# gnosisguild/stylus-zkvm-verifiers

Hardware: AMD Instinct MI355X
Metric: Groth16 proofs verified/sec (BN254) (higher is better)
Workload: dtype u32

## Files before the change

stylus_zkvm_verifiers_amd/csrc/bn254_constants.h:

```cpp
#pragma once
#include <stdint.h>
namespace zkv {
#define ZKV_FP_P_LIMBS {0xd87cfd47u, 0x3c208c16u, 0x6871ca8du, 0x97816a91u, 0x8181585du, 0xb85045b6u, 0xe131a029u, 0x30644e72u}
#define ZKV_FR_R_LIMBS {0xf0000001u, 0x43e1f593u, 0x79b97091u, 0x2833e848u, 0x8181585du, 0xb85045b6u, 0xe131a029u, 0x30644e72u}
#define ZKV_FP_INV32 0xe4866389u
#define ZKV_FP_P29_LIMBS {0x187cfd47u, 0x010460b6u, 0x1c72a34fu, 0x02d522d0u, 0x1585d978u, 0x02db40c0u, 0x00a6e141u, 0x0e5c2634u, 0x0030644eu}
#define ZKV_FP_INV29 0x04866389u
#define ZKV_FP_FAT4P_LIMBS {0x21f3f51cu, 0x241182dau, 0x31ca8d3bu, 0x2b548b42u, 0x361765dfu, 0x2b6d0301u, 0x229b8503u, 0x397098cfu, 0x00c19138u}
#define ZKV_FP_FAT8P_LIMBS {0x23e7ea38u, 0x282305b5u, 0x23951a77u, 0x36a91686u, 0x2c2ecbbfu, 0x36da0604u, 0x25370a07u, 0x32e1319fu, 0x01832272u}
#define ZKV_FP_2P_LIMBS {0xb0f9fa8eu, 0x7841182du, 0xd0e3951au, 0x2f02d522u, 0x0302b0bbu, 0x70a08b6du, 0xc2634053u, 0x60c89ce5u}
#define ZKV_FP_16P2_COLS {0x15d69b10ULL, 0xa2c5113ULL, 0xb0404edULL, 0xe5a13dULL, 0xadca602ULL, 0x4e36cb6ULL, 0x12129406ULL, 0xaf42485ULL, 0x104689e9ULL, 0x1a6359c6ULL, 0x1bb7e970ULL, 0x6eac0c4ULL, 0xb855116ULL, 0x690e580ULL, 0x1bdf00d2ULL, 0x1f38b334ULL, 0xb8763cbULL, 0x492e2ULL}
#define ZKV_FP_ONE {{0x157ccc21u, 0x4e8384ebu, 0x0ce148c3u, 0xfb90a602u, 0x819caa36u, 0x5301fa84u, 0x563d4475u, 0x0dc83629u}}
#define ZKV_FP_R2 {{0x659bac10u, 0xe1a2a074u, 0x5406005au, 0x63985586u, 0x2d3e2632u, 0xff54c580u, 0x34ea65a6u, 0x2a11a68cu}}
#define ZKV_FP_TWO_INV {{0xf6fce4b4u, 0x45520880u, 0xbaa989a8u, 0x49890849u, 0x818f014au, 0x85a9201du, 0x1bb7724fu, 0x1f16424eu}}
#define ZKV_FP_THREE {{0x40766463u, 0xeb8a8ec1u, 0x26a3da49u, 0xf2b1f206u, 0x84d5fea4u, 0xf905ef8du, 0x02b7cd5fu, 0x2958a27cu}}
#define ZKV_TWIST_B {{{0xab489658u, 0xdc19fa4au, 0xfbbf6e69u, 0x0d416744u, 0x0a8a033au, 0x8f7734edu, 0x53ee09bbu, 0x19316b83u}}, {{0x3b9fece0u, 0x1cfd999au, 0x79c1a7c7u, 0xbe166fb2u, 0x5580154cu, 0xe93a1ba4u, 0x4d11a9bau, 0x283739c9u}}}
#define ZKV_TWIST_3B {{{0x295cc5c1u, 0x582d62c9u, 0x8acc80b0u, 0x9042cb3du, 0x9e1cb150u, 0xf6155910u, 0x1a987d08u, 0x1b2ff417u}}, {{0x01e5cc12u, 0xdeb7b4a1u, 0x9c61623au, 0x0b4079f4u, 0xfd7d8f2bu, 0x4b0dc77fu, 0x24d1bcddu, 0x17dd1076u}}}
#define ZKV_FROB1 {{{{0x157ccc21u, 0x4e8384ebu, 0x0ce148c3u, 0xfb90a602u, 0x819caa36u, 0x5301fa84u, 0x563d4475u, 0x0dc83629u}}, {{0x00000000u, 0x00000000u, 0x00000000u, 0x00000000u, 0x00000000u, 0x00000000u, 0x00000000u, 0x00000000u}}}, {{{0x8a0c2399u, 0xb75446afu, 0x8d8526c8u, 0xb5e243dfu, 0x8fc2b89bu, 0x7f6d6627u, 0x62b5af58u, 0x2e056030u}}, {{0x3bc6cc33u, 0xaeefbf6eu, 0x4ed87762u, 0x7f50c04bu, 0xeb6a58d4u, 0x9a8b7572u, 0xc410c870u, 0x009b83e6u}}}, {{{0x24a59190u, 0xecdea09bu, 0xae2fe1c2u, 0x17db8ffeu, 0x6dabac4du, 0xbb09c97cu, 0x1d289af3u, 0x2492b3d4u}}, {{0xf1142ef1u, 0xf1663598u, 0x0bf56062u, 0x77ec057eu, 0xb677a631u, 0xdd0baaecu, 0xd284d463u, 0x135e4e31u}}}, {{{0xdb1f0678u, 0xf46e7f60u, 0x5bcc5c3eu, 0x31fc2ebau, 0x086a2411u, 0xedb3adc3u, 0x837817bcu, 0x1d46bd0fu}}, {{0x79a647d5u, 0x6b3fbdf5u, 0x2ff64974u, 0xcc568fb6u, 0xc4348ac6u, 0xc1bfbf4au, 0x3940b4d3u, 0x15871d4du}}}, {{{0xb081f85eu, 0x227346b0u, 0x30492bb5u, 0x6e51a671u, 0x52b19e16u, 0x7e20162eu, 0x2343bb4bu, 0x1677516fu}}, {{0x2f616a78u, 0x18b28085u, 0xbde06eceu, 0x25433712u, 0x6b9a0e66u, 0xb00a5825u, 0x11971bbdu, 0x06f9f8e1u}}}, {{{0x07461d8cu, 0x5c8694d6u, 0x07d3e2dau, 0x2df58554u, 0x667b18b9u, 0xb41988e2u, 0xc7bd8631u, 0x10a3f03eu}}, {{0xdeb54987u, 0x611aada3u, 0xc03203c7u, 0x4a7a9b79u, 0x9a786b4bu, 0x245c1057u, 0x754fe64du, 0x0817f6bdu}}}}
#define ZKV_FROB3 {{{{0x157ccc21u, 0x4e8384ebu, 0x0ce148c3u, 0xfb90a602u, 0x819caa36u, 0x5301fa84u, 0x563d4475u, 0x0dc83629u}}, {{0x00000000u, 0x00000000u, 0x00000000u, 0x00000000u, 0x00000000u, 0x00000000u, 0x00000000u, 0x00000000u}}}, {{{0x8e6a3d3du, 0x9dc00697u, 0x8ef4bf24u, 0x695b3f03u, 0xba7a7ccdu, 0x1a238968u, 0x0e49839cu, 0x103828f2u}}, {{0x4f4e6b31u, 0x5cbbb0bdu, 0x1b5b282bu, 0xe83ce8beu, 0xf03fbae3u, 0x646d437eu, 0x0031f0c0u, 0x133cf986u}}}, {{{0x136caecdu, 0x4738e103u, 0xc376b8c3u, 0xf491475bu, 0xa97cbee8u, 0x1f4034a3u, 0xef61ccd7u, 0x0cad5f8fu}}, {{0xe6e485d6u, 0x2f41c395u, 0x0242aa46u, 0x997230c7u, 0x84887ab5u, 0xeae16f21u, 0x3bcfc9b2u, 0x266696f7u}}}, {{{0xfd5df6cfu, 0x47b20cb5u, 0x0ca56e4eu, 0x65853bd7u, 0x7917344cu, 0xca9c97f3u, 0x5db9886cu, 0x131d9163u}}, {{0x5ed6b572u, 0xd0e0ce21u, 0x387b8118u, 0xcb2adadbu, 0xbd4ccd96u, 0xf690866bu, 0xa7f0eb55u, 0x1add3125u}}}, {{{0x0af866c4u, 0xa0d04454u, 0x7df631b3u, 0x9cc0145fu, 0xcd752de1u, 0x29dda327u, 0x0a170a74u, 0x14766fdbu}}, {{0xe9d402f7u, 0xdd532940u, 0xbfda559eu, 0x541490c5u, 0xc541b0b8u, 0xd9c9c659u, 0x69cbb3e4u, 0x0baf8cb5u}}}, {{{0xe314d9feu, 0xcdc1bb0eu, 0x7463ae42u, 0xfe0354c4u, 0x3e3cd6b9u, 0xf2cc84b7u, 0xabddad87u, 0x14445b76u}}, {{0x9b3b7638u, 0x0210d593u, 0x9015f128u, 0x2d0dc9e1u, 0xc52a22adu, 0xbe219959u, 0x44050889u, 0x12c9d777u}}}}
#define ZKV_FROB2 {{{0x157ccc21u, 0x4e8384ebu, 0x0ce148c3u, 0xfb90a602u, 0x819caa36u, 0x5301fa84u, 0x563d4475u, 0x0dc83629u}}, {{0x6e4983b2u, 0xd96ee872u, 0x458f581eu, 0xe9b7ed6au, 0x9ea5d262u, 0x5361c2c8u, 0x98a79c6eu, 0x24594fd1u}}, {{0x58ccb791u, 0x8aeb6387u, 0x38ae0f5bu, 0xee274768u, 0x1d09282bu, 0x005fc844u, 0x426a57f9u, 0x169119a8u}}, {{0xc3003126u, 0xed9d072bu, 0x5b9081c9u, 0x9bf0c48fu, 0xffe4ae26u, 0x654e4b31u, 0x8af45bb4u, 0x229c1849u}}, {{0x6a337995u, 0x62b1a3a4u, 0x22e2726eu, 0xadc97d27u, 0xe2db85fau, 0x64ee82edu, 0x488a03bbu, 0x0c0afea1u}}, {{0x7fb045b6u, 0xb135288fu, 0x2fc3bb31u, 0xa95a2329u, 0x64783031u, 0xb7f07d72u, 0x9ec74830u, 0x19d334cau}}}
#define ZKV_BN_U 0x44e992b44a6909f1ULL
#define ZKV_ATE_NAF_LEN 66
#define ZKV_ATE_NAF {0, 0, 0, 1, 0, 1, 0, -1, 0, 0, -1, 0, 0, 0, 1, 0, 0, -1, 0, -1, 0, 0, 0, 1, 0, -1, 0, 0, 0, 0, -1, 0, 0, 1, 0, -1, 0, 0, 1, 0, 0, 0, 0, 0, -1, 0, 0, -1, 0, 1, 0, -1, 0, 0, 0, -1, 0, -1, 0, 0, 0, 1, 0, -1, 0, 1}
#define ZKV_MILLER_STEPS 88
#define ZKV_MILLER_STEP_KIND {0, 0, 2, 0, 0, 1, 0, 0, 0, 0, 2, 0, 0, 2, 0, 0, 0, 0, 2, 0, 0, 1, 0, 0, 2, 0, 0, 0, 2, 0, 0, 0, 0, 0, 0, 1, 0, 0, 0, 2, 0, 0, 1, 0, 0, 0, 2, 0, 0, 0, 0, 0, 2, 0, 0, 1, 0, 0, 0, 0, 2, 0, 0, 2, 0, 0, 0, 1, 0, 0, 0, 0, 2, 0, 0, 0, 2, 0, 0, 1, 0, 0, 1, 0, 0, 0, 3, 4}
#define ZKV_U_NAF_LEN 63
#define ZKV_U_NAF {1, 0, 0, 0, -1, 0, 0, 0, 0, 1, 0, 1, 0, 0, 0, 0, 1, 0, 0, 1, 0, -1, 0, 1, 0, 1, 0, 1, 0, 0, 1, 0, 0, 0, 1, 0, -1, 0, -1, 0, -1, 0, 1, 0, 1, 0, 0, -1, 0, 1, 0, 1, 0, -1, 0, 0, 1, 0, 1, 0, 0, 0, 1}
#define ZKV_U_WNAF3_LEN 63
#define ZKV_U_WNAF3 {1, 0, 0, 0, -1, 0, 0, 0, 0, 5, 0, 0, 0, 0, 0, 0, -7, 0, 0, 0, 7, 0, 0, 0, 0, 5, 0, 0, 0, 0, 1, 0, 0, 0, -3, 0, 0, 0, -5, 0, 0, 0, 5, 0, 0, 0, 0, 3, 0, 0, 0, -3, 0, 0, 0, 0, 5, 0, 0, 0, 0, 0, 1}
#define ZKV_U_DIG_LEN 58
#define ZKV_U_DIG {17, 0, 0, 0, 0, -17, 0, 0, 0, 0, 35, 0, 0, 0, 0, 17, 0, 0, 0, 0, 0, 35, 0, 0, 0, 35, 0, 0, 0, 0, 0, 0, 0, 0, -35, 0, 0, 0, -35, 0, 0, 0, 35, 0, 17, 0, 0, 0, 0, 0, 0, -35, 0, 0, 0, 0, 0, 35}
#define ZKV_FE_PROG_LEN 268
#define ZKV_FE_PROG {0x10000u, 0x1u, 0x10102u, 0x1000003u, 0x800u, 0x2080105u, 0x800u, 0x8010203u, 0x20000u, 0x6u, 0x6u, 0x6u, 0x6u, 0x2000003u, 0x600u, 0x6u, 0x2000003u, 0x700u, 0x6u, 0x6u, 0x6u, 0x6u, 0x6u, 0x6u, 0x7000004u, 0x6u, 0x6u, 0x6u, 0x6u, 0x6u, 0x6u, 0x6u, 0x6000003u, 0x6u, 0x6u, 0x7000003u, 0x6u, 0x6u, 0x6u, 0x6u, 0x7000004u, 0x6u, 0x6u, 0x6u, 0x6u, 0x7000004u, 0x6u, 0x6u, 0x6u, 0x6u, 0x6u, 0x6u, 0x6u, 0x6u, 0x6u, 0x7000003u, 0x6u, 0x6u, 0x6u, 0x6u, 0x7000003u, 0x6u, 0x6u, 0x6u, 0x6u, 0x6u, 0x6u, 0x6000003u, 0x6u, 0x6u, 0x6u, 0x6u, 0x6u, 0x7000003u, 0x6u, 0x6u, 0x6u, 0x6u, 0x6u, 0x6000004u, 0x6u, 0x6u, 0x6u, 0x6u, 0x6u, 0x6000003u, 0x1u, 0x6u, 0x300u, 0x6u, 0x3000003u, 0x400u, 0x6u, 0x6u, 0x6u, 0x6u, 0x4000003u, 0x600u, 0x6u, 0x4000003u, 0x700u, 0x6u, 0x6u, 0x6u, 0x6u, 0x6u, 0x6u, 0x7000004u, 0x6u, 0x6u, 0x6u, 0x6u, 0x6u, 0x6u, 0x6u, 0x6000003u, 0x6u, 0x6u, 0x7000003u, 0x6u, 0x6u, 0x6u, 0x6u, 0x7000004u, 0x6u, 0x6u, 0x6u, 0x6u, 0x7000004u, 0x6u, 0x6u, 0x6u, 0x6u, 0x6u, 0x6u, 0x6u, 0x6u, 0x6u, 0x7000003u, 0x6u, 0x6u, 0x6u, 0x6u, 0x7000003u, 0x6u, 0x6u, 0x6u, 0x6u, 0x6u, 0x6u, 0x6000003u, 0x6u, 0x6u, 0x6u, 0x6u, 0x6u, 0x7000003u, 0x6u, 0x6u, 0x6u, 0x6u, 0x6u, 0x6000004u, 0x6u, 0x6u, 0x6u, 0x6u, 0x6u, 0x6000003u, 0x1u, 0x500u, 0x6u, 0x100u, 0x6u, 0x6u, 0x6u, 0x6u, 0x1000003u, 0x600u, 0x6u, 0x1000003u, 0x700u, 0x6u, 0x6u, 0x6u, 0x6u, 0x6u, 0x6u, 0x7000004u, 0x6u, 0x6u, 0x6u, 0x6u, 0x6u, 0x6u, 0x6u, 0x6000003u, 0x6u, 0x6u, 0x7000003u, 0x6u, 0x6u, 0x6u, 0x6u, 0x7000004u, 0x6u, 0x6u, 0x6u, 0x6u, 0x7000004u, 0x6u, 0x6u, 0x6u, 0x6u, 0x6u, 0x6u, 0x6u, 0x6u, 0x6u, 0x7000003u, 0x6u, 0x6u, 0x6u, 0x6u, 0x7000003u, 0x6u, 0x6u, 0x6u, 0x6u, 0x6u, 0x6u, 0x6000003u, 0x6u, 0x6u, 0x6u, 0x6u, 0x6u, 0x7000003u, 0x6u, 0x6u, 0x6u, 0x6u, 0x6u, 0x6000004u, 0x6u, 0x6u, 0x6u, 0x6u, 0x6u, 0x6000003u, 0x401u, 0x5000003u, 0x4000003u, 0x400u, 0x800u, 0x3080103u, 0x5000003u, 0x2000003u, 0x1010305u, 0x3000003u, 0x2040405u, 0x4000003u, 0x201u, 0x1020203u, 0x3020205u, 0x2000003u, 0x800u, 0x807u}
#define ZKV_FP_M30_LIMBS {0x187cfd47, 0x3082305b, 0x071ca8d3, 0x205aa45a, 0x01585d97, 0x0116da06, 0x1a029b85, 0x139cb84c, 0x00003064}
#define ZKV_FP_MINV30 0x1b799c77u
#define ZKV_FP_R3 {{0x4e2312b2u, 0x26d80b94u, 0x85af210eu, 0xfdde6f98u, 0xad1d1adau, 0xb923065cu, 0xa668ff5au, 0x26c2d286u}}
#define ZKV_FR_M30_LIMBS {0x30000001, 0x0f87d64f, 0x1b970914, 0x0cfa121e, 0x01585d28, 0x0116da06, 0x1a029b85, 0x139cb84c, 0x00003064}
#define ZKV_FR_MINV30 0x10000001u
#define ZKV_FR_R3 {{0x601fddb2u, 0xbafa616cu, 0x23e89803u, 0x29b4a83eu, 0x44d1496bu, 0x917ad601u, 0xfe59ed6du, 0x1baa96fcu}}
#define ZKV_GLV_BETA {{0x58ccb791u, 0x8aeb6387u, 0x38ae0f5bu, 0xee274768u, 0x1d09282bu, 0x005fc844u, 0x426a57f9u, 0x169119a8u}}
#define ZKV_GLV_LAMBDA {0x36636f23u, 0xb8ca0b2du, 0xec2bc5e9u, 0xcc37a73fu, 0x3fd84104u, 0x048b6e19u, 0xe131a029u, 0x30644e72u}
#define ZKV_GLV_G1 {0x00ff6565u, 0x5398fd03u, 0xa773d2d2u, 0x4ccef014u, 0x00000002u}
#define ZKV_GLV_G2 {0xc7e0b3d7u, 0xd91d232eu, 0x00000002u}
#define ZKV_GLV_A1 {0x7d4f1128u, 0x8211bbebu, 0xeeb859fcu, 0x6f4d8248u}
#define ZKV_GLV_N {0x94d213e3u, 0x89d32568u}
#define ZKV_GLV_B2 {0x1221250bu, 0x0be4e154u, 0xeeb859fdu, 0x6f4d8248u}
#define ZKV_FP_INV_SCHED_LEN 76
#define ZKV_FP_INV_SCHED {19, 59, 25, 33, 35, 9, 35, 9, 25, 27, 9, 41, 35, 43, 17, 65, 17, 35, 27, 9, 41, 17, 49, 33, 27, 27, 27, 17, 67, 57, 17, 27, 41, 27, 9, 27, 25, 27, 19, 57, 27, 17, 17, 17, 25, 33, 27, 17, 51, 9, 43, 9, 25, 17, 17, 43, 17, 35, 19, 41, 49, 43, 49, 27, 27, 27, 51, 19, 9, 35, 19, 19, 17, 17, 33, 17}
#define ZKV_FP_PM2_LIMBS {0xd87cfd45u, 0x3c208c16u, 0x6871ca8du, 0x97816a91u, 0x8181585du, 0xb85045b6u, 0xe131a029u, 0x30644e72u}
#define ZKV_FR_R29_LIMBS {0x10000001u, 0x1f0fac9fu, 0x0e5c2450u, 0x07d090f3u, 0x1585d283u, 0x02db40c0u, 0x00a6e141u, 0x0e5c2634u, 0x0030644eu}
#define ZKV_FR_INV29 0x0fffffffu
#define ZKV_FR_ONE {{0x8fffff57u, 0x2fd4e156u, 0xa494b01au, 0x75bba827u, 0x819caa80u, 0x5301fa84u, 0x563d4475u, 0x0dc83629u}}
#define ZKV_FR_R2 {{0x45b69bd4u, 0x38c2e14bu, 0x85883377u, 0x0ffedb18u, 0xabc6e54du, 0x7840f9f0u, 0x848b0f05u, 0x0a054a3eu}}
#define ZKV_FR_RM2_LIMBS {0xefffffffu, 0x43e1f593u, 0x79b97091u, 0x2833e848u, 0x8181585du, 0xb85045b6u, 0xe131a029u, 0x30644e72u}
}
```

stylus_zkvm_verifiers_amd/csrc/gen_constants.py:

```python
#!/usr/bin/env python3
import os

U = 4965661367192848881
P = 36 * U**4 + 36 * U**3 + 24 * U**2 + 6 * U + 1
R = 36 * U**4 + 36 * U**3 + 18 * U**2 + 6 * U + 1
MONT = 1 << 261


def f2mul(a, b): return ((a[0] * b[0] - a[1] * b[1]) % P, (a[0] * b[1] + a[1] * b[0]) % P)
def f2inv(a):
    d = pow(a[0] * a[0] + a[1] * a[1], -1, P)
    return (a[0] * d % P, -a[1] * d % P)
def f2pow(a, e):
    r = (1, 0)
    while e:
        if e & 1:
            r = f2mul(r, a)
        a = f2mul(a, a)
        e >>= 1
    return r


def limbs(x):
    return ', '.join('0x%08xu' % ((x >> (32 * i)) & 0xffffffff) for i in range(8))

def mont(x): return x * MONT % P
def fp(x): return '{{%s}}' % limbs(mont(x))
def fp2(a): return '{%s, %s}' % (fp(a[0]), fp(a[1]))


def naf(n):
    out = []
    while n:
        if n & 1:
            d = 2 - (n % 4)
            n -= d
        else:
            d = 0
        out.append(d)
        n >>= 1
    return out


def main():
    xi = (9, 1)
    twist_b = f2mul((3, 0), f2inv(xi))
    g = f2pow(xi, (P - 1) // 6)
    frob1 = [f2pow(g, k) for k in range(6)]
    g2 = f2pow(xi, (P * P - 1) // 6)
    frob2 = [f2pow(g2, k) for k in range(6)]
    assert all(c[1] == 0 for c in frob2)
    g3 = f2pow(xi, (P**3 - 1) // 6)
    frob3 = [f2pow(g3, k) for k in range(6)]
    ate = 6 * U + 2
    ate_naf = naf(ate)
    assert sum(d * (1 << i) for i, d in enumerate(ate_naf)) == ate
    inv32 = (-pow(P, -1, 1 << 32)) % (1 << 32)
    lines = []
    w = lines.append
    w('// GENERATED by gen_constants.py -- do not edit.  BN254 constants in Montgomery form (R = 2^261),')
    w('// 8 x 32-bit little-endian limbs.')
    w('#pragma once')
    w('#include <stdint.h>')
    w('namespace zkv {')
    w('#define ZKV_FP_P_LIMBS {%s}' % limbs(P))
    w('#define ZKV_FR_R_LIMBS {%s}' % limbs(R))
    w('#define ZKV_FP_INV32 0x%08xu' % inv32)
    w('#define ZKV_FP_P29_LIMBS {%s}' % ', '.join('0x%08xu' % ((P >> (29 * i)) & 0x1fffffff) for i in range(9)))
    w('#define ZKV_FP_INV29 0x%08xu' % ((-pow(P, -1, 1 << 29)) % (1 << 29)))
    d4 = [((4 * P) >> (29 * i)) & 0x1fffffff for i in range(9)]
    fat = [d4[0] + (1 << 29)] + [d4[i] + (1 << 29) - 1 for i in range(1, 8)] + [d4[8] - 1]
    assert sum(v << (29 * i) for i, v in enumerate(fat)) == 4 * P and all(v >= (1 << 29) - 1 for v in fat[:8])
    w('// 4p in borrow-free 29-bit limbs (limbs 0..7 >= 2^29-1): FAT - y is limb-wise non-negative for y < 2p')
    w('#define ZKV_FP_FAT4P_LIMBS {%s}' % ', '.join('0x%08xu' % v for v in fat))
    d8 = [((8 * P) >> (29 * i)) & 0x1fffffff for i in range(9)]
    fat8 = [d8[0] + (1 << 29)] + [d8[i] + (1 << 29) - 1 for i in range(1, 8)] + [d8[8] - 1]
    assert sum(v << (29 * i) for i, v in enumerate(fat8)) == 8 * P and all(v >= (1 << 29) - 1 for v in fat8[:8])
    assert fat8[8] >= ((4 * P) >> 232) and max(fat8) < (1 << 31)
    w('// 8p in borrow-free 29-bit limbs: FAT - y is limb-wise non-negative for every y < 4p (lazy sum of two values < 2p)')
    w('#define ZKV_FP_FAT8P_LIMBS {%s}' % ', '.join('0x%08xu' % v for v in fat8))
    w('#define ZKV_FP_2P_LIMBS {%s}' % limbs(2 * P))
    c16 = 16 * P * P
    w('// 16 p^2 in 29-bit digits (18 columns): offset that keeps T0 - T1 non-negative in the fused Fp2 product')
    w('#define ZKV_FP_16P2_COLS {%s}' % ', '.join('0x%xULL' % ((c16 >> (29 * i)) & 0x1fffffff) for i in range(18)))
    assert c16 >> (29 * 18) == 0
    w('#define ZKV_FP_ONE %s' % fp(1))
    w('#define ZKV_FP_R2 {{%s}}' % limbs(MONT * MONT % P))
    w('#define ZKV_FP_TWO_INV %s' % fp(pow(2, -1, P)))
    w('#define ZKV_FP_THREE %s' % fp(3))
    w('#define ZKV_TWIST_B %s' % fp2(twist_b))
    w('#define ZKV_TWIST_3B %s' % fp2((3 * twist_b[0] % P, 3 * twist_b[1] % P)))
    for name, arr in (('FROB1', frob1), ('FROB3', frob3)):
        w('#define ZKV_%s {%s}' % (name, ', '.join(fp2(c) for c in arr)))
    w('#define ZKV_FROB2 {%s}' % ', '.join(fp(c[0]) for c in frob2))
    w('#define ZKV_BN_U 0x%xULL' % U)
    w('#define ZKV_ATE_NAF_LEN %d' % len(ate_naf))
    w('// NAF digits of 6u+2, least significant first (top digit is 1)')
    w('#define ZKV_ATE_NAF {%s}' % ', '.join(str(d) for d in ate_naf))
    kinds = []
    for i in range(len(ate_naf) - 2, -1, -1):
        kinds.append(0)
        if ate_naf[i]:
            kinds.append(1 if ate_naf[i] > 0 else 2)
    kinds += [3, 4]
    assert len(kinds) == 88
    w('// Miller loop as a flat sequence of line steps: 0 doubling (preceded by f <- f^2 except at step 0), 1 add Q, 2 add -Q, 3 add pi(Q), 4 add -pi^2(Q)')
    w('#define ZKV_MILLER_STEPS %d' % len(kinds))
    w('#define ZKV_MILLER_STEP_KIND {%s}' % ', '.join(str(k) for k in kinds))
    u_naf = naf(U)
    assert sum(d * (1 << i) for i, d in enumerate(u_naf)) == U
    w('// NAF digits of u, least significant first (final exponentiation: x^u with conjugates for the -1 digits)')
    w('#define ZKV_U_NAF_LEN %d' % len(u_naf))
    w('#define ZKV_U_NAF {%s}' % ', '.join(str(d) for d in u_naf))
    def wnaf(n, width):
        out = []
        while n:
            if n & 1:
                d = n % (1 << (width + 1))
                if d >= (1 << width):
                    d -= 1 << (width + 1)
                n -= d
            else:
                d = 0
            out.append(d)
            n >>= 1
        return out
    u_w3 = wnaf(U, 3)
    assert sum(d * (1 << i) for i, d in enumerate(u_w3)) == U and u_w3[-1] == 1 and all(abs(d) in (0, 1, 3, 5, 7) for d in u_w3)
    w('// width-3 NAF digits of u (odd digits up to +-7), least significant first, top digit 1: %d non-zero digits' % sum(1 for d in u_w3 if d))
    w('#define ZKV_U_WNAF3_LEN %d' % len(u_w3))
    w('#define ZKV_U_WNAF3 {%s}' % ', '.join(str(d) for d in u_w3))
    OPS = dict(COPY=0, CONJ=1, INV=2, MUL=3, MULC=4, FROB=5, CSQR=6, ISONE=7)
    ACC, F_, E_, Y1, Y3, Y4, X3, X5, X7 = range(9)
    prog = []
    acc_is = [None]
    def op(name, d=0, a=0, b=0):
        if name == 'COPY' and d == ACC and acc_is[0] == a:
            return
        if name == 'COPY' and a == ACC: acc_is[0] = d
        elif name == 'COPY' and d == ACC: acc_is[0] = a
        elif d == ACC or d == acc_is[0]: acc_is[0] = None
        prog.append(OPS[name] | d << 8 | a << 16 | b << 24)
    import functools, sys
    sys.setrecursionlimit(10000)
    DIG = (1, 17, 35)
    @functools.lru_cache(None)
    def recode(n):
        if n == 0:
            return (0, ())
        if n % 2 == 0:
            c, t = recode(n // 2)
            return (c, (0,) + t)
        best = None
        for d in DIG:
            for sd in (d, -d):
                m = (n - sd) // 2
                if abs(m) < abs(n) or (abs(n) <= max(DIG) and m == 0):
                    c, t = recode(m)
                    if best is None or c + 1 < best[0]:
                        best = (c + 1, (sd,) + t)
        return best
    u_dig = recode(U)[1]
    assert sum(d << i for i, d in enumerate(u_dig)) == U and u_dig[-1] > 0 and sum(1 for d in u_dig if d) == 12
    w('// digits of u from {0, +-1, +-17, +-35}, least significant first, top digit positive: %d non-zero (final exponentiation, x^u)' % sum(1 for d in u_dig if d))
    w('#define ZKV_U_DIG_LEN %d' % len(u_dig))
    w('#define ZKV_U_DIG {%s}' % ', '.join(str(d) for d in u_dig))
    def expu(x):
        X17, X35 = X3, X5
        op('COPY', ACC, x)
        for _ in range(4): op('CSQR', ACC)
        op('MUL', ACC, ACC, x); op('COPY', X17, ACC)
        op('CSQR', ACC)
        op('MUL', ACC, ACC, x); op('COPY', X35, ACC)
        src = {1: x, 17: X17, 35: X35}
        op('COPY', ACC, src[u_dig[-1]])
        for i in range(len(u_dig) - 2, -1, -1):
            op('CSQR', ACC)
            d = u_dig[i]
            if d:
                op('MUL' if d > 0 else 'MULC', ACC, ACC, src[abs(d)])
    op('COPY', ACC, F_); op('CONJ', ACC); op('INV', F_, F_); op('MUL', ACC, ACC, F_)
    op('FROB', F_, ACC, 2); op('MUL', E_, F_, ACC)
    expu(E_); op('CONJ', ACC)
    op('CSQR', ACC); op('COPY', Y1, ACC)
    op('CSQR', ACC)
    op('MUL', ACC, ACC, Y1); op('COPY', Y3, ACC)
    expu(Y3); op('CONJ', ACC); op('COPY', Y4, ACC)
    op('CSQR', ACC); op('COPY', F_, ACC)
    expu(F_)
    op('CONJ', Y3)
    op('MUL', ACC, ACC, Y4)
    op('MUL', ACC, ACC, Y3); op('COPY', Y3, ACC)
    op('MUL', F_, ACC, Y1)
    op('MUL', ACC, ACC, Y4)
    op('MUL', ACC, ACC, E_)
    op('FROB', Y1, F_, 1); op('MUL', ACC, ACC, Y1)
    op('FROB', Y3, Y3, 2); op('MUL', ACC, ACC, Y3)
    op('CONJ', E_); op('MUL', E_, E_, F_); op('FROB', E_, E_, 3)
    op('MUL', ACC, ACC, E_)
    op('ISONE', ACC)
    TMP = 8
    out = []
    for e in prog:
        o, d, a, b = e & 255, (e >> 8) & 255, (e >> 16) & 255, e >> 24
        native = (o == OPS['CSQR'] or o == OPS['COPY'] or (o == OPS['CONJ'] and d == ACC)
                  or (o in (OPS['MUL'], OPS['MULC']) and d == ACC and a == ACC and b != ACC))
        if not native:
            assert d != ACC or o == OPS['ISONE']
            uses = (a == ACC and o in (OPS['INV'], OPS['MUL'], OPS['MULC'], OPS['FROB'])) or (b == ACC and o in (OPS['MUL'], OPS['MULC'])) or (o == OPS['ISONE'] and d == ACC)
            if uses:
                out.append(OPS['COPY'] | TMP << 8 | ACC << 16)
                if o == OPS['ISONE']: d = TMP
                if a == ACC and o != OPS['ISONE']: a = TMP
                if b == ACC and o in (OPS['MUL'], OPS['MULC']): b = TMP
                e = o | d << 8 | a << 16 | b << 24
        out.append(e)
    prog = out
    w('// final exponentiation (easy part, Fuentes-Castaneda hard part, x^u on the signed digit set {1, 17, 35}) as a flat program: op | dst << 8 | a << 16 | b << 24;')
    w('// ops 0 COPY d<-a, 1 CONJ d, 2 INV d<-a, 3 MUL d<-a*b, 4 MULC d<-a*conj(b), 5 FROB d<-pi^b(a), 6 CSQR d (cyclotomic), 7 ISONE; slots 0 ACC 1 F 2 E 3 Y1 4 Y3 5 Y4 6 X17 7 X35 8 TMP')
    w('#define ZKV_FE_PROG_LEN %d' % len(prog))
    w('#define ZKV_FE_PROG {%s}' % ', '.join('0x%xu' % v for v in prog))
    e = P - 2
    bits = bin(e)[2:]
    sched = []
    i = 0
    nsq = 0
    while i < len(bits):
        if bits[i] == '0':
            nsq += 1; i += 1
            continue
        l = min(2, len(bits) - i)
        while bits[i + l - 1] == '0':
            l -= 1
        v = int(bits[i:i + l], 2)
        sched.append((nsq + l, v))
        nsq = 0
        i += l
    if nsq:
        sched.append((nsq, 0))
    first = sched[0]
    acc = first[1]
    for n_, v in sched[1:]:
        acc = acc * (1 << n_) + v
    assert acc == e and first[0] == len(bin(first[1])) - 2
    assert all(n_ < 32 and v in (0, 1, 3) for n_, v in sched)
    w('// a^(p-2): sliding window (width 2) schedule, entries = squarings << 3 | odd power (0 = none); entry 0 = start power.')
    w('// %d squarings and %d multiplications instead of 253 and %d' % (sum(n_ for n_, v in sched[1:]), sum(1 for n_, v in sched[1:] if v) + 2, bin(e).count('1') - 1))
    def limbs30(x): return ', '.join('0x%08x' % ((x >> (30 * i)) & ((1 << 30) - 1)) for i in range(9))
    w('// safegcd inversion (zkv_modinv.h): the modulus as nine 30-bit limbs, its inverse mod 2^30, and R^3 mod p (Montgomery factor that')
    w('// turns (aR)^-1 into a^-1 R with one multiplication)')
    w('#define ZKV_FP_M30_LIMBS {%s}' % limbs30(P))
    w('#define ZKV_FP_MINV30 0x%08xu' % pow(P, -1, 1 << 30))
    w('#define ZKV_FP_R3 {{%s}}' % limbs(MONT ** 3 % P))
    w('#define ZKV_FR_M30_LIMBS {%s}' % limbs30(R))
    w('#define ZKV_FR_MINV30 0x%08xu' % pow(R, -1, 1 << 30))
    w('#define ZKV_FR_R3 {{%s}}' % limbs((1 << (3 * 261)) % R))
    lam = 0x30644e72e131a029048b6e193fd84104cc37a73fec2bc5e9b8ca0b2d36636f23
    beta = 0x30644e72e131a0295e6dd9e7e0acccb0c28f069fbb966e3de4bd44e5607cfd48
    assert (lam * lam + lam + 1) % R == 0 and pow(beta, 3, P) == 1 and beta != 1
    a1, nb1, a2, b2 = 6 * U * U + 2 * U, 2 * U + 1, 2 * U + 1, 6 * U * U + 4 * U + 1
    assert (a1 - nb1 * lam) % R == 0 and (a2 + b2 * lam) % R == 0
    def nl(x, n): return ', '.join('0x%08xu' % ((x >> (32 * i)) & 0xffffffff) for i in range(n))
    w('// GLV: beta (Montgomery form), lambda, floor(2^256 b2 / r) (5 words), floor(2^256 (2u+1) / r) (3 words), a1 = 6u^2+2u (4), 2u+1 (2), b2 = 6u^2+4u+1 (4)')
    w('#define ZKV_GLV_BETA %s' % fp(beta))
    w('#define ZKV_GLV_LAMBDA {%s}' % limbs(lam))
    w('#define ZKV_GLV_G1 {%s}' % nl((b2 << 256) // R, 5))
    w('#define ZKV_GLV_G2 {%s}' % nl((nb1 << 256) // R, 3))
    w('#define ZKV_GLV_A1 {%s}' % nl(a1, 4))
    w('#define ZKV_GLV_N {%s}' % nl(nb1, 2))
    w('#define ZKV_GLV_B2 {%s}' % nl(b2, 4))
    assert ((b2 << 256) // R).bit_length() <= 160 and ((nb1 << 256) // R).bit_length() <= 96
    w('#define ZKV_FP_INV_SCHED_LEN %d' % len(sched))
    w('#define ZKV_FP_INV_SCHED {%s}' % ', '.join(str((n_ << 3) | v) for n_, v in sched))
    w('// p-2 for Fermat inversion, little-endian 32-bit words')
    w('#define ZKV_FP_PM2_LIMBS {%s}' % limbs(P - 2))
    w('// scalar field: r as nine 29-bit limbs, -r^-1 mod 2^29, 2^261 mod r, 2^522 mod r, r - 2 (Fermat inversion)')
    w('#define ZKV_FR_R29_LIMBS {%s}' % ', '.join('0x%08xu' % ((R >> (29 * i)) & 0x1fffffff) for i in range(9)))
    w('#define ZKV_FR_INV29 0x%08xu' % ((-pow(R, -1, 1 << 29)) % (1 << 29)))
    w('#define ZKV_FR_ONE {{%s}}' % limbs((1 << 261) % R))
    w('#define ZKV_FR_R2 {{%s}}' % limbs((1 << 522) % R))
    w('#define ZKV_FR_RM2_LIMBS {%s}' % limbs(R - 2))
    w('}  // namespace zkv')
    out = os.path.join(os.path.dirname(os.path.abspath(__file__)), 'bn254_constants.h')
    with open(out, 'w') as f:
        f.write('\n'.join(lines) + '\n')
    print('wrote', out, 'naf len', len(ate_naf), 'weight', sum(1 for d in ate_naf if d))


if __name__ == '__main__':
    main()
```

stylus_zkvm_verifiers_amd/csrc/k_pair.hip:

```cpp
#define ZKV_PAIRED 1
#include "zkv_internal.h"
#include "zkv_agg.h"

namespace zkv {

#ifndef ZKV_PAIR_WAVES
#define ZKV_PAIR_WAVES 1
#endif
constexpr int PAIR_BLOCK = ZKV_BLOCK * ZKV_PAIR_WAVES;

__device__ __forceinline__ Fp2 ld_b(const Workspace& ws, int word0, size_t i) {
    Fp2 r; r.h = ws_ld(ws.prep, ws.cap, word0 + 8 * (int)(threadIdx.x & 1u), i);
    return r;
}

__global__ __launch_bounds__(ZKV_BLOCK, 2) void k_g2chk2(size_t n, Workspace ws, uint8_t* __restrict__ status) {
    size_t i = ((size_t)blockIdx.x * ZKV_BLOCK + threadIdx.x) >> 1;
    if (i >= n) return;
    uint32_t flags = ws.flags[i];
    if (!(flags & FL_ALIVE) || (flags & FL_B_INF)) return;
    Fp2 bx = ld_b(ws, 32, i), by = ld_b(ws, 48, i);
    bool ok = g2_in_subgroup(bx, by);
    if (!ok && !(threadIdx.x & 1u)) { ws.g2bad[i] = 1; status[i] = ST_VERIFICATION_FAILED; }
}

#if defined(ZKV_STAMPS)
__device__ unsigned long long* g_zkv_stamps = nullptr;
extern "C" __attribute__((visibility("default"))) int zkv_diag_set_stamps(void* dev_ptr) {
    return (int)hipMemcpyToSymbol(HIP_SYMBOL(g_zkv_stamps), &dev_ptr, sizeof(dev_ptr));
}
__device__ __forceinline__ void zkv_stamp(unsigned kernel, unsigned slot) {
    if ((threadIdx.x & 63u) != 0 || !g_zkv_stamps) return;
    unsigned long long* row = g_zkv_stamps + ((size_t)kernel * gridDim.x * (blockDim.x >> 6) + (size_t)blockIdx.x * (blockDim.x >> 6) + (threadIdx.x >> 6)) * 8;
    row[slot] = __builtin_amdgcn_s_memrealtime();
    row[4 + slot] = __builtin_amdgcn_s_memtime();
    if (slot == 0) { row[2] = __builtin_amdgcn_s_getreg((31 << 11) | 4); row[3] = __builtin_amdgcn_s_getreg((31 << 11) | 20); }
}
#define ZKV_STAMP(k, s) zkv_stamp(k, s)
#else
#define ZKV_STAMP(k, s) ((void)0)
#endif

__global__ __launch_bounds__(PAIR_BLOCK, 2) void k_miller2(size_t n, const VkTables* __restrict__ vk, Workspace ws, uint8_t* __restrict__ status) {
    __shared__ uint32_t lds[(48 + 24) * PAIR_BLOCK];
    ZKV_STAMP(0, 0);
    size_t i = ((size_t)blockIdx.x * PAIR_BLOCK + threadIdx.x) >> 1;
    if (i >= n) return;
    uint32_t flags = ws.flags[i];
    if (!(flags & FL_ALIVE)) return;
    const uint32_t par = threadIdx.x & 1u;
    uint32_t* wl = lds + (threadIdx.x >> 6) * ((48 + 24) * ZKV_BLOCK) + (threadIdx.x & 63u);
    LRef fm = l_ref(wl);
    LRef tm = l_ref(wl + 48 * ZKV_BLOCK);
    SoaRef norm = {ws.norm, ws.cap, (uint32_t)i * 4u};
    SoaRef bsrc = {ws.prep + 32 * ws.cap, ws.cap, (uint32_t)(8 * par * ws.cap + i) * 4u};
    if (!miller_loop_p(vk, flags, norm, bsrc, fm, tm, true)) {
        if (!par) { ws.g2bad[i] = 1; status[i] = ST_VERIFICATION_FAILED; }
        return;
    }
    MRef ab = m_ref((uint32_t*)(vk->f_alpha_beta) + 8 * par, 1, 16);
    MRef out = m_ref(ws.f + (size_t)(8 * par) * ws.cap + i, (uint32_t)ws.cap, 16);
    f12m_mul_body(out, fm, ab, false);
    ZKV_STAMP(0, 1);
}

__global__ __launch_bounds__(PAIR_BLOCK, 2) void k_finalexp2(size_t n, Workspace ws, uint8_t* __restrict__ status) {
    __shared__ uint32_t lds[54 * PAIR_BLOCK];
    ZKV_STAMP(1, 0);
    size_t i = ((size_t)blockIdx.x * PAIR_BLOCK + threadIdx.x) >> 1;
    if (i >= n) return;
    uint32_t flags = ws.flags[i];
    if (!(flags & FL_ALIVE) || ws.g2bad[i]) return;
    const uint32_t par = threadIdx.x & 1u;
    uint32_t* wl = lds + (threadIdx.x >> 6) * (54 * ZKV_BLOCK) + (threadIdx.x & 63u);
    L9Ref acc = l9_ref(wl);
    bool one = final_exp_prog_p(ws.f, ws.fe, ws.cap, (uint32_t)(8 * par * ws.cap + i) * 4u, acc);
    if (!par) status[i] = one ? ST_OK : ST_VERIFICATION_FAILED;
    ZKV_STAMP(1, 1);
}

ZKV_HD bool pair_all(bool mine) {
    uint32_t v = mine ? 0u : 1u;
    v |= zkv_partner_u32(v);
    return v == 0;
}
__global__ __launch_bounds__(ZKV_BLOCK, 2) void k_pairing_check(size_t n, uint32_t k, uint32_t j, size_t slot_off, const uint8_t* __restrict__ in, Workspace ws,
                                                                uint8_t* __restrict__ ok) {
    const size_t call = ((size_t)blockIdx.x * ZKV_BLOCK + threadIdx.x) >> 1;
    if (call >= n) return;
    const size_t i = call + slot_off;
    const uint32_t par = threadIdx.x & 1u;
    if (j == 0) {
        f12m_set_one(m_ref(ws.f + (size_t)(8 * par) * ws.cap + call, (uint32_t)ws.cap, 16));
        if (!par) ok[call] = 1;
    } else if (!ok[call]) { if (!par) ws.flags[i] = 0; return; }
    const uint8_t* p = in + (size_t)192 * ((size_t)k * call + j);
    uint32_t gx[8], gy[8], qxw[8], qyw[8];
    load_be256(gx, p); load_be256(gy, p + 32);
    load_be256(qxw, p + 64 + 32 * (1 - par));
    load_be256(qyw, p + 128 + 32 * (1 - par));
    bool okj = raw_lt_p(gx) && raw_lt_p(gy);
    okj = pair_all(okj && raw_lt_p(qxw) && raw_lt_p(qyw));
    const bool pinf = raw_is_zero(gx) && raw_is_zero(gy);
    const bool qinf = pair_all(raw_is_zero(qxw) && raw_is_zero(qyw));
    Fp px = fp_zero(), py = fp_zero();
    if (okj && !pinf) { px = fp_from_raw(gx); py = fp_from_raw(gy); okj = g1_on_curve(px, py); }
    uint32_t run = 0;
    if (okj && !qinf) {
        Fp2 qx, qy; qx.h = fp_from_raw(qxw); qy.h = fp_from_raw(qyw);
        okj = g2_on_twist(qx, qy);
        if (okj) {
            const Fp iy = pinf ? fp_zero() : fp_inv(py);
            ws_st(ws.norm, ws.cap, 0, i, fp_mul(px, iy)); ws_st(ws.norm, ws.cap, 8, i, iy);
            ws_st(ws.prep, ws.cap, 32 + 8 * (int)par, i, qx.h); ws_st(ws.prep, ws.cap, 48 + 8 * (int)par, i, qy.h);
            run = pinf ? 2u : 1u;
        }
    }
    if (!par) { ws.flags[i] = run; if (!okj) ok[call] = 0; }
}
template <int G>
__global__ __launch_bounds__(PAIR_BLOCK, 2) void k_pairing_miller_g(size_t n, uint32_t k, Workspace ws, uint8_t* __restrict__ ok) {
    __shared__ uint32_t lds[48 * PAIR_BLOCK];
    const size_t i = ((size_t)blockIdx.x * PAIR_BLOCK + threadIdx.x) >> 1;
    if (i >= n) return;
    if (!ok[i]) return;
    uint32_t mask = 0, abmask = 0;
#pragma unroll
    for (uint32_t p = 0; p < (uint32_t)G; p++) {
        const uint32_t run = p < k ? ws.flags[i + p * n] : 0u;
        if (run) { mask |= 1u << p; if (run == 1u) abmask |= 1u << p; }
    }
    const uint32_t par = threadIdx.x & 1u;
    MRef P = m_ref(ws.f + (size_t)(8 * par) * ws.cap + i, (uint32_t)ws.cap, 16);
    if (!mask) return;
    uint32_t* wl = lds + (threadIdx.x >> 6) * (48 * ZKV_BLOCK) + (threadIdx.x & 63u);
    LRef fm = l_ref(wl);
    SoaRef norm = {ws.norm, ws.cap, (uint32_t)i * 4u};
    SoaRef bsrc = {ws.prep + 32 * ws.cap, ws.cap, (uint32_t)(8 * par * ws.cap + i) * 4u};
    SoaRW tq = {ws.fe, ws.cap, (uint32_t)(8 * par * ws.cap + i) * 4u};
    const uint32_t fine = miller_loop_pg<G>(mask, abmask, norm, bsrc, tq, (uint32_t)n * 4u, fm);
    if ((fine & mask) != mask) { if (!par) ok[i] = 0; return; }
    f12m_copy(P, fm);
}
__global__ __launch_bounds__(ZKV_BLOCK, 2) void k_pairing_miller(size_t n, Workspace ws, uint8_t* __restrict__ ok) {
    __shared__ uint32_t lds[(48 + 24) * ZKV_BLOCK];
    size_t i = ((size_t)blockIdx.x * ZKV_BLOCK + threadIdx.x) >> 1;
    if (i >= n) return;
    const uint32_t run = ws.flags[i];
    if (!run) return;
    const uint32_t par = threadIdx.x & 1u;
    LRef fm = l_ref(lds + threadIdx.x);
    LRef tm = l_ref(lds + 48 * ZKV_BLOCK + threadIdx.x);
    MRef P = m_ref(ws.f + (size_t)(8 * par) * ws.cap + i, (uint32_t)ws.cap, 16);
    SoaRef norm = {ws.norm, ws.cap, (uint32_t)i * 4u};
    SoaRef bsrc = {ws.prep + 32 * ws.cap, ws.cap, (uint32_t)(8 * par * ws.cap + i) * 4u};
    const bool fine = miller_loop_p((const VkTables*)nullptr, run == 2 ? (uint32_t)FL_A_INF : 0u, norm, bsrc, fm, tm, true);
    if (fine && run == 1) f12m_mul(P, fm, P);
    if (!fine && !par) ok[i] = 0;
}
__global__ __launch_bounds__(ZKV_BLOCK, 2) void k_pairing_finalexp(size_t n, Workspace ws, const uint8_t* __restrict__ ok, uint8_t* __restrict__ result,
                                                                   uint32_t empty) {
    __shared__ uint32_t lds[54 * ZKV_BLOCK];
    size_t i = ((size_t)blockIdx.x * ZKV_BLOCK + threadIdx.x) >> 1;
    if (i >= n) return;
    const uint32_t par = threadIdx.x & 1u;
    uint8_t res = empty ? 1 : 0;
    if (ok[i] && !empty) {
        L9Ref acc = l9_ref(lds + threadIdx.x);
        res = final_exp_prog_p(ws.f, ws.fe, ws.cap, (uint32_t)(8 * par * ws.cap + i) * 4u, acc) ? 1 : 0;
    }
    if (!par) result[i] = res;
}
uint32_t pairing_group(uint32_t k) { return k < 2 ? 0u : k <= 2 ? 2u : k <= 4 ? 4u : k <= 8 ? 8u : 0u; }
void launch_pairing(size_t n, uint32_t k, const uint8_t* in, const Workspace& ws, uint8_t* result, uint8_t* ok, hipStream_t s) {
    if (!n) return;
    const unsigned grid = (unsigned)((2 * n + ZKV_BLOCK - 1) / ZKV_BLOCK);
    if (k == 0) (void)hipMemsetAsync(ok, 1, n, s);
    const uint32_t g = pairing_group(k);
    if (g && (size_t)k * n <= ws.cap) {
        for (uint32_t j = 0; j < k; j++) hipLaunchKernelGGL(k_pairing_check, dim3(grid), dim3(ZKV_BLOCK), 0, s, n, k, j, (size_t)j * n, in, ws, ok);
        const dim3 hg((unsigned)((2 * n + PAIR_BLOCK - 1) / PAIR_BLOCK)), hb(PAIR_BLOCK);
        if (g == 2) hipLaunchKernelGGL(k_pairing_miller_g<2>, hg, hb, 0, s, n, k, ws, ok);
        else if (g == 4) hipLaunchKernelGGL(k_pairing_miller_g<4>, hg, hb, 0, s, n, k, ws, ok);
        else hipLaunchKernelGGL(k_pairing_miller_g<8>, hg, hb, 0, s, n, k, ws, ok);
    } else for (uint32_t j = 0; j < k; j++) {
        hipLaunchKernelGGL(k_pairing_check, dim3(grid), dim3(ZKV_BLOCK), 0, s, n, k, j, (size_t)0, in, ws, ok);
        hipLaunchKernelGGL(k_pairing_miller, dim3(grid), dim3(ZKV_BLOCK), 0, s, n, ws, ok);
    }
    hipLaunchKernelGGL(k_pairing_finalexp, dim3(grid), dim3(ZKV_BLOCK), 0, s, n, ws, ok, result, k == 0 ? 1u : 0u);
}

template <int G>
__global__ __launch_bounds__(PAIR_BLOCK, 2) void k_agg_miller(size_t n, const VkTables* __restrict__ vk, Workspace ws, uint8_t* __restrict__ status) {
    __shared__ uint32_t lds[48 * PAIR_BLOCK];
    constexpr uint32_t L = 64u / G;
    const size_t gp = ((size_t)blockIdx.x * PAIR_BLOCK + threadIdx.x) >> 1;
    const size_t i0 = (gp / L) * 64 + (gp % L);
    if (i0 >= n) return;
    uint32_t alive = 0, mask = 0, abmask = 0;
#pragma unroll
    for (uint32_t p = 0; p < (uint32_t)G; p++) {
        const size_t i = i0 + p * L;
        const uint32_t f = i < n ? ws.flags[i] : 0u;
        if (f & FL_ALIVE) {
            alive |= 1u << p;
            if (!(f & FL_B_INF)) { mask |= 1u << p; if (!(f & FL_A_INF)) abmask |= 1u << p; }
        }
    }
    if (!alive) return;
    const uint32_t par = threadIdx.x & 1u;
    uint32_t* wl = lds + (threadIdx.x >> 6) * (48 * ZKV_BLOCK) + (threadIdx.x & 63u);
    LRef fm = l_ref(wl);
    SoaRef norm = {ws.norm, ws.cap, (uint32_t)i0 * 4u};
    SoaRef bsrc = {ws.prep + 32 * ws.cap, ws.cap, (uint32_t)(8 * par * ws.cap + i0) * 4u};
    SoaRW tq = {ws.fe, ws.cap, (uint32_t)(8 * par * ws.cap + i0) * 4u};
    const uint32_t fine = miller_loop_pg<G>(mask, abmask, norm, bsrc, tq, L * 4u, fm);
    if ((fine & mask) != mask) {
        if (!par) {
#pragma unroll 1
            for (uint32_t p = 0; p < (uint32_t)G; p++) {
                if (!((alive >> p) & 1u)) continue;
                const bool bad = ((mask & ~fine) >> p) & 1u;
                ws.g2bad[i0 + p * L] = bad ? 1u : 2u;
                if (bad) status[i0 + p * L] = ST_VERIFICATION_FAILED;
            }
        }
        return;
    }
    MRef ab = m_ref((uint32_t*)(vk->f_alpha_beta) + 8 * par, 1, 16);
    MRef out = m_ref(ws.f + (size_t)(8 * par) * ws.cap + i0, (uint32_t)ws.cap, 16);
    f12m_mul_body(out, fm, ab, false);
}
void launch_agg_miller(size_t n, uint32_t g, const VkTables* d_tab, const Workspace& ws, uint8_t* status, hipStream_t s) {
    if (!n) return;
    const size_t pairs = ((n + 63) / 64) * (64 / g);
    const dim3 grid((unsigned)((2 * pairs + PAIR_BLOCK - 1) / PAIR_BLOCK)), block(PAIR_BLOCK);
    if (g == 8) hipLaunchKernelGGL(k_agg_miller<8>, grid, block, 0, s, n, d_tab, ws, status);
    else if (g == 4) hipLaunchKernelGGL(k_agg_miller<4>, grid, block, 0, s, n, d_tab, ws, status);
    else hipLaunchKernelGGL(k_agg_miller<2>, grid, block, 0, s, n, d_tab, ws, status);
}
__global__ __launch_bounds__(ZKV_BLOCK, 2) void k_agg_fprod(size_t n, size_t n2, uint32_t sub, uint32_t g, Workspace ws, const uint32_t* __restrict__ agg, Workspace ws2) {
    __shared__ uint32_t lds[48 * ZKV_BLOCK];
    const size_t sb = ((size_t)blockIdx.x * ZKV_BLOCK + threadIdx.x) >> 1;
    if (sb >= n2) return;
    if (!(ws2.flags[sb] & FL_ALIVE)) return;
    const uint32_t par = threadIdx.x & 1u;
    LRef acc = l_ref(lds + threadIdx.x);
    MRef P2 = m_ref(ws2.f + (size_t)(8 * par) * ws2.cap + sb, (uint32_t)ws2.cap, 16);
    f12m_copy(acc, P2);
    const uint32_t L = 64u / g, w = (sub < 64u ? sub : 64u) / g, nblk = sub > 64u ? sub / 64u : 1u, per = sub > 64u ? 1u : 64u / sub;
#pragma unroll 1
    for (uint32_t b = 0; b < nblk; b++) {
        const size_t i0 = sub > 64u ? sb * sub + (size_t)b * 64 : (sb / per) * 64 + (sb % per) * w;
#pragma unroll 1
        for (uint32_t k = 0; k < w; k++) {
            bool in = false;
#pragma unroll 1
            for (uint32_t p = 0; p < g && !in; p++) {
                const size_t i = i0 + k + p * L;
                if (i < n) in = (agg[(size_t)AGG_W_FLAGS * ws.cap + i] & FL_ALIVE) && !ws.g2bad[i];
            }
            if (!in) continue;
            MRef Pi = m_ref(ws.f + (size_t)(8 * par) * ws.cap + i0 + k, (uint32_t)ws.cap, 16);
            f12m_mul(acc, acc, Pi);
        }
    }
    f12m_copy(P2, acc);
}
void launch_agg_fprod(size_t n, size_t n2, uint32_t sub, uint32_t g, const Workspace& ws, const uint32_t* agg, const Workspace& ws2, hipStream_t s) {
    if (!n2) return;
    hipLaunchKernelGGL(k_agg_fprod, dim3((unsigned)((2 * n2 + ZKV_BLOCK - 1) / ZKV_BLOCK)), dim3(ZKV_BLOCK), 0, s, n, n2, sub, g, ws, agg, ws2);
}

static inline unsigned pair_grid(size_t n) { return (unsigned)((2 * n + ZKV_BLOCK - 1) / ZKV_BLOCK); }
static inline unsigned hot_grid(size_t n) { return (unsigned)((2 * n + PAIR_BLOCK - 1) / PAIR_BLOCK); }

void launch_g2chk2(size_t n, const Workspace& ws, uint8_t* status, hipStream_t s) {
    if (!n) return;
    hipLaunchKernelGGL(k_g2chk2, dim3(pair_grid(n)), dim3(ZKV_BLOCK), 0, s, n, ws, status);
}
void launch_miller2(size_t n, const VkTables* d_tab, const Workspace& ws, uint8_t* status, hipStream_t s) {
    if (!n) return;
    hipLaunchKernelGGL(k_miller2, dim3(hot_grid(n)), dim3(PAIR_BLOCK), 0, s, n, d_tab, ws, status);
}
void launch_finalexp2(size_t n, const Workspace& ws, uint8_t* status, hipStream_t s) {
    if (!n) return;
    hipLaunchKernelGGL(k_finalexp2, dim3(hot_grid(n)), dim3(PAIR_BLOCK), 0, s, n, ws, status);
}

}
```

stylus_zkvm_verifiers_amd/csrc/zkv_field.h:

```cpp
#pragma once
#include <stdint.h>
#include "bn254_constants.h"

#if defined(__HIPCC__)
#define ZKV_HD __host__ __device__ __forceinline__
#define ZKV_HD_NI __host__ __device__ __noinline__ inline
#else
#define ZKV_HD inline
#define ZKV_HD_NI inline
#endif

#if defined(ZKV_COUNT_FP_MUL)
static thread_local unsigned long long zkv_fp_mul_counter = 0;
static thread_local unsigned long long zkv_mad_counter = 0;
#define ZKV_COUNT_MADS(n) (zkv_mad_counter += (n))
#else
#define ZKV_COUNT_MADS(n) ((void)0)
#endif

#if defined(__HIP_DEVICE_COMPILE__)
#define ZKV_TABLE static __device__ const
#else
#define ZKV_TABLE static const
#endif

#if defined(ZKV_ASM_MARKS) && defined(__HIP_DEVICE_COMPILE__)
#define ZKV_MARK(name) asm volatile("; ZKVMARK " name)
#else
#define ZKV_MARK(name) ((void)0)
#endif

#ifndef ZKV_FAIR_SLICE_SHIFT
#define ZKV_FAIR_SLICE_SHIFT 17
#endif
ZKV_HD uint32_t zkv_wave_slot_parity() {
#if defined(__HIP_DEVICE_COMPILE__) && !defined(ZKV_NO_FAIR_SHARE)
    return __builtin_amdgcn_s_getreg((3 << 11) | 4) & 1u;
#else
    return 0;
#endif
}
ZKV_HD void zkv_fair_share(uint32_t slot_parity) {
#if defined(__HIP_DEVICE_COMPILE__) && !defined(ZKV_NO_FAIR_SHARE)
    const uint32_t t = (uint32_t)(__builtin_amdgcn_s_memrealtime() >> ZKV_FAIR_SLICE_SHIFT);
    if ((t ^ slot_parity) & 1u) __builtin_amdgcn_s_setprio(1);
    else __builtin_amdgcn_s_setprio(0);
#else
    (void)slot_parity;
#endif
}

#include "zkv_modinv.h"

namespace zkv {

struct Fp { uint32_t v[8]; };
struct Fp2C { Fp c0, c1; };
#if defined(ZKV_PAIRED)
struct Fp2 { Fp h; };
#else
struct Fp2 { Fp c0, c1; };
#endif
struct Fp6 { Fp2 c0, c1, c2; };

#if defined(__has_builtin)
#if __has_builtin(__builtin_addc) && __has_builtin(__builtin_subc)
#define ZKV_HAVE_CARRY_BUILTINS 1
#endif
#endif
ZKV_HD uint32_t addc(uint32_t a, uint32_t b, uint32_t& carry) {
#if defined(ZKV_HAVE_CARRY_BUILTINS)
    unsigned co; uint32_t r = __builtin_addc(a, b, carry, &co); carry = co; return r;
#else
    uint64_t t = (uint64_t)a + b + carry;
    carry = (uint32_t)(t >> 32);
    return (uint32_t)t;
#endif
}
ZKV_HD uint32_t subb(uint32_t a, uint32_t b, uint32_t& borrow) {
#if defined(ZKV_HAVE_CARRY_BUILTINS)
    unsigned bo; uint32_t r = __builtin_subc(a, b, borrow, &bo); borrow = bo; return r;
#else
    uint64_t t = (uint64_t)a - b - borrow;
    borrow = (uint32_t)(t >> 32) & 1u;
    return (uint32_t)t;
#endif
}

ZKV_HD Fp fp_zero() { Fp r; for (int i = 0; i < 8; i++) r.v[i] = 0; return r; }
ZKV_HD Fp fp_one() { Fp r = ZKV_FP_ONE; return r; }
ZKV_HD bool fp_is_zero(const Fp& a) {
    const uint32_t P[8] = ZKV_FP_P_LIMBS;
    uint32_t o = 0, q = 0;
    for (int i = 0; i < 8; i++) { o |= a.v[i]; q |= a.v[i] ^ P[i]; }
    return o == 0 || q == 0;
}
ZKV_HD bool u256_geq(const uint32_t* a, const uint32_t* m) {
    uint32_t br = 0;
    for (int i = 0; i < 8; i++) (void)subb(a[i], m[i], br);
    return br == 0;
}
ZKV_HD Fp fp_add(const Fp& a, const Fp& b) {
    const uint32_t P[8] = ZKV_FP_2P_LIMBS;
    Fp t, s; uint32_t c = 0, br = 0;
#pragma unroll
    for (int i = 0; i < 8; i++) t.v[i] = addc(a.v[i], b.v[i], c);
#pragma unroll
    for (int i = 0; i < 8; i++) s.v[i] = subb(t.v[i], P[i], br);
#pragma unroll
    for (int i = 0; i < 8; i++) t.v[i] = br ? t.v[i] : s.v[i];
    return t;
}
ZKV_HD Fp fp_sub(const Fp& a, const Fp& b) {
    const uint32_t P[8] = ZKV_FP_2P_LIMBS;
    Fp t; uint32_t br = 0, c = 0;
#pragma unroll
    for (int i = 0; i < 8; i++) t.v[i] = subb(a.v[i], b.v[i], br);
    uint32_t mask = 0u - br;
#pragma unroll
    for (int i = 0; i < 8; i++) t.v[i] = addc(t.v[i], P[i] & mask, c);
    return t;
}
ZKV_HD bool fp_eq(const Fp& a, const Fp& b) { return fp_is_zero(fp_sub(a, b)); }
ZKV_HD Fp fp_neg(const Fp& a) { return fp_sub(fp_zero(), a); }
ZKV_HD Fp fp_dbl(const Fp& a) { return fp_add(a, a); }
ZKV_HD Fp fp_half(const Fp& a) {
    const uint32_t P[8] = ZKV_FP_P_LIMBS;
    const uint32_t m = 0u - (a.v[0] & 1u);
    Fp t; uint32_t c = 0;
#pragma unroll
    for (int i = 0; i < 8; i++) t.v[i] = addc(a.v[i], P[i] & m, c);
    Fp r;
#pragma unroll
    for (int i = 0; i < 7; i++) r.v[i] = (t.v[i] >> 1) | (t.v[i + 1] << 31);
    r.v[7] = t.v[7] >> 1;
    return r;
}
ZKV_HD Fp fp_add_nr(const Fp& a, const Fp& b) {
    Fp t; uint32_t c = 0;
#pragma unroll
    for (int i = 0; i < 8; i++) t.v[i] = addc(a.v[i], b.v[i], c);
    return t;
}
ZKV_HD void fp_add_x2(const Fp& a0, const Fp& b0, const Fp& a1, const Fp& b1, Fp& r0, Fp& r1) {
    const uint32_t P[8] = ZKV_FP_2P_LIMBS;
    Fp t0, t1, s0, s1; uint32_t c0 = 0, c1 = 0, w0 = 0, w1 = 0;
#pragma unroll
    for (int i = 0; i < 8; i++) { t0.v[i] = addc(a0.v[i], b0.v[i], c0); t1.v[i] = addc(a1.v[i], b1.v[i], c1); }
#pragma unroll
    for (int i = 0; i < 8; i++) { s0.v[i] = subb(t0.v[i], P[i], w0); s1.v[i] = subb(t1.v[i], P[i], w1); }
#pragma unroll
    for (int i = 0; i < 8; i++) { r0.v[i] = w0 ? t0.v[i] : s0.v[i]; r1.v[i] = w1 ? t1.v[i] : s1.v[i]; }
}
ZKV_HD void fp_sub_x2(const Fp& a0, const Fp& b0, const Fp& a1, const Fp& b1, Fp& r0, Fp& r1) {
    const uint32_t P[8] = ZKV_FP_2P_LIMBS;
    Fp t0, t1; uint32_t w0 = 0, w1 = 0, c0 = 0, c1 = 0;
#pragma unroll
    for (int i = 0; i < 8; i++) { t0.v[i] = subb(a0.v[i], b0.v[i], w0); t1.v[i] = subb(a1.v[i], b1.v[i], w1); }
    uint32_t m0 = 0u - w0, m1 = 0u - w1;
#pragma unroll
    for (int i = 0; i < 8; i++) { r0.v[i] = addc(t0.v[i], P[i] & m0, c0); r1.v[i] = addc(t1.v[i], P[i] & m1, c1); }
}

ZKV_HD void fp_unpack29(const Fp& a, uint32_t x[9]) {
#pragma unroll
    for (int k = 0; k < 9; k++) {
        const int bit = 29 * k, w = bit >> 5, s = bit & 31;
        uint32_t v = a.v[w] >> s;
        if (s > 3 && w < 7) v |= a.v[w + 1] << (32 - s);
        x[k] = v & 0x1fffffffu;
    }
}
template <typename COL>
ZKV_HD void fp_mac81(COL col[18], const uint32_t x[9], const uint32_t y[9]) {
    ZKV_COUNT_MADS(81);
#pragma unroll
    for (int i = 0; i < 9; i++) {
#pragma unroll
        for (int j = 0; j < 9; j++) col[i + j] = (COL)((uint64_t)col[i + j] + (uint64_t)x[i] * y[j]);
    }
}
template <typename COL>
ZKV_HD void fp_reduce_cols_limbs(COL col[18], uint32_t (&r)[9]) {
    ZKV_COUNT_MADS(81);
    const uint32_t P29[9] = ZKV_FP_P29_LIMBS;
    const uint32_t M29 = 0x1fffffffu;
#pragma unroll
    for (int i = 0; i < 9; i++) {
        uint32_t m = ((uint32_t)col[i] * ZKV_FP_INV29) & M29;
#pragma unroll
        for (int j = 0; j < 9; j++) col[i + j] = (COL)((uint64_t)col[i + j] + (uint64_t)m * P29[j]);
        col[i + 1] += col[i] >> 29;
    }
#pragma unroll
    for (int k = 9; k < 17; k++) {
        r[k - 9] = (uint32_t)col[k] & M29;
        col[k + 1] += col[k] >> 29;
    }
    r[8] = (uint32_t)col[17];
}
ZKV_HD Fp fp_pack29(const uint32_t (&r)[9]) {
    Fp o;
#pragma unroll
    for (int w = 0; w < 8; w++) {
        const int bit = 32 * w, k = bit / 29, s = bit - 29 * k, got = 29 - s;
        uint32_t v = r[k] >> s;
        if (k + 1 < 9) v |= r[k + 1] << got;
        if (got + 29 < 32 && k + 2 < 9) v |= r[k + 2] << (got + 29);
        o.v[w] = v;
    }
    return o;
}
template <typename COL>
ZKV_HD Fp fp_reduce_cols(COL col[18]) {
    uint32_t r[9];
    fp_reduce_cols_limbs(col, r);
    return fp_pack29(r);
}
#if defined(ZKV_FP_MUL_NOINLINE)
ZKV_HD_NI
#else
ZKV_HD
#endif
Fp fp_mul(Fp a, Fp b) {
#if defined(ZKV_COUNT_FP_MUL)
    zkv_fp_mul_counter++;
#endif
    uint32_t x[9], y[9];
    fp_unpack29(a, x); fp_unpack29(b, y);
    int64_t col[18];
#pragma unroll
    for (int k = 0; k < 18; k++) col[k] = 0;
    fp_mac81(col, x, y);
    return fp_reduce_cols(col);
}
#if defined(ZKV_FP_MUL_NOINLINE)
ZKV_HD_NI
#else
ZKV_HD
#endif
Fp fp_sqr(Fp a) {
#if defined(ZKV_COUNT_FP_MUL)
    zkv_fp_mul_counter++;
#endif
    uint32_t x[9], d[9];
    fp_unpack29(a, x);
#pragma unroll
    for (int i = 0; i < 9; i++) d[i] = x[i] << 1;
    uint64_t col[18];
    ZKV_COUNT_MADS(45);
#pragma unroll
    for (int k = 0; k < 18; k++) col[k] = 0;
#pragma unroll
    for (int i = 0; i < 9; i++) {
        col[2 * i] += (uint64_t)x[i] * x[i];
#pragma unroll
        for (int j = i + 1; j < 9; j++) col[i + j] += (uint64_t)d[i] * x[j];
    }
    return fp_reduce_cols(col);
}

ZKV_HD Fp fp_from_raw(const uint32_t* limbs) {
    Fp t, r2 = ZKV_FP_R2;
    for (int i = 0; i < 8; i++) t.v[i] = limbs[i];
    return fp_mul(t, r2);
}
ZKV_HD void fp_to_raw(uint32_t* limbs, const Fp& a) {
    const uint32_t P[8] = ZKV_FP_P_LIMBS;
    Fp one = fp_zero(); one.v[0] = 1;
    Fp t = fp_mul(a, one), s; uint32_t br = 0;
    for (int i = 0; i < 8; i++) s.v[i] = subb(t.v[i], P[i], br);
    for (int i = 0; i < 8; i++) limbs[i] = br ? t.v[i] : s.v[i];
}
ZKV_HD Fp fp_inv_fermat(const Fp& a) {
    const uint8_t S[ZKV_FP_INV_SCHED_LEN] = ZKV_FP_INV_SCHED;
    const Fp a3 = fp_mul(fp_sqr(a), a);
    Fp acc = (S[0] & 7) == 3 ? a3 : a;
#pragma unroll 1
    for (int i = 1; i < ZKV_FP_INV_SCHED_LEN; i++) {
        const int nsq = S[i] >> 3, v = S[i] & 7;
#pragma unroll 1
        for (int k = 0; k < nsq; k++) acc = fp_sqr(acc);
        if (v) {
            Fp m;
#pragma unroll
            for (int k = 0; k < 8; k++) m.v[k] = v == 3 ? a3.v[k] : a.v[k];
            acc = fp_mul(acc, m);
        }
    }
    return acc;
}

ZKV_HD Fp fp_inv(const Fp& a) {
    const int32_t M[9] = ZKV_FP_M30_LIMBS;
    const Fp r3 = ZKV_FP_R3;
    Fp t = a;
    modinv30(t.v, M, ZKV_FP_MINV30);
    return fp_mul(t, r3);
}

template <int N>
ZKV_HD void fp_add_n(const Fp (&a)[N], const Fp (&b)[N], Fp (&r)[N]) {
    const uint32_t P[8] = ZKV_FP_2P_LIMBS;
    Fp t[N], s[N]; uint32_t c[N], w[N];
#pragma unroll
    for (int k = 0; k < N; k++) { c[k] = 0; w[k] = 0; }
#pragma unroll
    for (int i = 0; i < 8; i++) {
#pragma unroll
        for (int k = 0; k < N; k++) t[k].v[i] = addc(a[k].v[i], b[k].v[i], c[k]);
    }
#pragma unroll
    for (int i = 0; i < 8; i++) {
#pragma unroll
        for (int k = 0; k < N; k++) s[k].v[i] = subb(t[k].v[i], P[i], w[k]);
    }
#pragma unroll
    for (int i = 0; i < 8; i++) {
#pragma unroll
        for (int k = 0; k < N; k++) r[k].v[i] = w[k] ? t[k].v[i] : s[k].v[i];
    }
}
template <int N>
ZKV_HD void fp_sub_n(const Fp (&a)[N], const Fp (&b)[N], Fp (&r)[N]) {
    const uint32_t P[8] = ZKV_FP_2P_LIMBS;
    Fp t[N]; uint32_t w[N], c[N], m[N];
#pragma unroll
    for (int k = 0; k < N; k++) { c[k] = 0; w[k] = 0; }
#pragma unroll
    for (int i = 0; i < 8; i++) {
#pragma unroll
        for (int k = 0; k < N; k++) t[k].v[i] = subb(a[k].v[i], b[k].v[i], w[k]);
    }
#pragma unroll
    for (int k = 0; k < N; k++) m[k] = 0u - w[k];
#pragma unroll
    for (int i = 0; i < 8; i++) {
#pragma unroll
        for (int k = 0; k < N; k++) r[k].v[i] = addc(t[k].v[i], P[i] & m[k], c[k]);
    }
}

#if !defined(ZKV_PAIRED)
ZKV_HD Fp2 f2_const(const Fp2C& c) { Fp2 r; r.c0 = c.c0; r.c1 = c.c1; return r; }
ZKV_HD Fp2 f2_zero() { Fp2 r; r.c0 = fp_zero(); r.c1 = fp_zero(); return r; }
ZKV_HD Fp2 f2_one() { Fp2 r; r.c0 = fp_one(); r.c1 = fp_zero(); return r; }
ZKV_HD bool f2_is_zero(const Fp2& a) { return fp_is_zero(a.c0) && fp_is_zero(a.c1); }
ZKV_HD bool f2_eq(const Fp2& a, const Fp2& b) { return fp_eq(a.c0, b.c0) && fp_eq(a.c1, b.c1); }
ZKV_HD Fp2 f2_add(const Fp2& a, const Fp2& b) { Fp2 r; fp_add_x2(a.c0, b.c0, a.c1, b.c1, r.c0, r.c1); return r; }
ZKV_HD Fp2 f2_sub(const Fp2& a, const Fp2& b) { Fp2 r; fp_sub_x2(a.c0, b.c0, a.c1, b.c1, r.c0, r.c1); return r; }
ZKV_HD Fp2 f2_neg(const Fp2& a) { Fp2 r; Fp z = fp_zero(); fp_sub_x2(z, a.c0, z, a.c1, r.c0, r.c1); return r; }
ZKV_HD Fp2 f2_add_nr(const Fp2& a, const Fp2& b) { Fp2 r; r.c0 = fp_add_nr(a.c0, b.c0); r.c1 = fp_add_nr(a.c1, b.c1); return r; }
ZKV_HD Fp2 f2_dbl(const Fp2& a) { return f2_add(a, a); }
ZKV_HD Fp2 f2_half(const Fp2& a) { Fp2 r; r.c0 = fp_half(a.c0); r.c1 = fp_half(a.c1); return r; }
ZKV_HD Fp2 f2_conj(const Fp2& a) { Fp2 r; r.c0 = a.c0; r.c1 = fp_neg(a.c1); return r; }
ZKV_HD void f2_mul_core(const Fp& a0, const Fp& a1, const Fp& b0, const Fp& b1, Fp& c0, Fp& c1) {
#if defined(ZKV_COUNT_FP_MUL)
    zkv_fp_mul_counter += 3;
#endif
    const uint64_t C16P2[18] = ZKV_FP_16P2_COLS;
    uint32_t x0[9], x1[9], y0[9], y1[9], sx[9], sy[9];
    fp_unpack29(a0, x0); fp_unpack29(a1, x1); fp_unpack29(b0, y0); fp_unpack29(b1, y1);
#pragma unroll
    for (int i = 0; i < 9; i++) { sx[i] = x0[i] + x1[i]; sy[i] = y0[i] + y1[i]; }
    int64_t t0[18], t1[18], m[18];
#pragma unroll
    for (int k = 0; k < 18; k++) { t0[k] = 0; t1[k] = 0; m[k] = 0; }
    fp_mac81(t0, x0, y0); fp_mac81(t1, x1, y1); fp_mac81(m, sx, sy);
#pragma unroll
    for (int k = 0; k < 18; k++) {
        m[k] = (int64_t)((uint64_t)m[k] - (uint64_t)t0[k] - (uint64_t)t1[k]);
        t0[k] = (int64_t)((uint64_t)t0[k] - (uint64_t)t1[k] + C16P2[k]);
    }
    c0 = fp_reduce_cols(t0);
    c1 = fp_reduce_cols(m);
}
#if defined(__HIP_DEVICE_COMPILE__) && defined(ZKV_FP_MUL_NOINLINE)
#define ZKV_L8(p) uint32_t p##0, uint32_t p##1, uint32_t p##2, uint32_t p##3, uint32_t p##4, uint32_t p##5, uint32_t p##6, uint32_t p##7
#define ZKV_A8(f) f.v[0], f.v[1], f.v[2], f.v[3], f.v[4], f.v[5], f.v[6], f.v[7]
#define ZKV_MK(f, p) Fp f; f.v[0] = p##0; f.v[1] = p##1; f.v[2] = p##2; f.v[3] = p##3; f.v[4] = p##4; f.v[5] = p##5; f.v[6] = p##6; f.v[7] = p##7
__device__ __noinline__ inline Fp2 f2_mul_ni(ZKV_L8(pa), ZKV_L8(pb), ZKV_L8(pc), ZKV_L8(pd)) {
    ZKV_MK(a0, pa); ZKV_MK(a1, pb); ZKV_MK(b0, pc); ZKV_MK(b1, pd);
    Fp2 r; f2_mul_core(a0, a1, b0, b1, r.c0, r.c1);
    return r;
}
ZKV_HD Fp2 f2_mul(const Fp2& a, const Fp2& b) { return f2_mul_ni(ZKV_A8(a.c0), ZKV_A8(a.c1), ZKV_A8(b.c0), ZKV_A8(b.c1)); }
#else
ZKV_HD Fp2 f2_mul(const Fp2& a, const Fp2& b) { Fp2 r; f2_mul_core(a.c0, a.c1, b.c0, b.c1, r.c0, r.c1); return r; }
#endif
ZKV_HD Fp2 f2_sqr(const Fp2& a) {
    Fp2 r;
    r.c0 = fp_mul(fp_add_nr(a.c0, a.c1), fp_sub(a.c0, a.c1));
    r.c1 = fp_mul(fp_add_nr(a.c0, a.c0), a.c1);
    return r;
}
ZKV_HD Fp2 f2_mul_fp(const Fp2& a, const Fp& k) { Fp2 r; r.c0 = fp_mul(a.c0, k); r.c1 = fp_mul(a.c1, k); return r; }
ZKV_HD Fp2 f2_mul_xi(const Fp2& a) {
    Fp t0 = fp_dbl(fp_dbl(fp_dbl(a.c0))), t1 = fp_dbl(fp_dbl(fp_dbl(a.c1)));
    Fp2 r; r.c0 = fp_sub(fp_add(t0, a.c0), a.c1); r.c1 = fp_add(fp_add(t1, a.c1), a.c0);
    return r;
}
ZKV_HD Fp2 f2_inv(const Fp2& a) {
    Fp n = fp_add(fp_sqr(a.c0), fp_sqr(a.c1));
    Fp i = fp_inv(n);
    Fp2 r; r.c0 = fp_mul(a.c0, i); r.c1 = fp_neg(fp_mul(a.c1, i));
    return r;
}

#else
#if defined(__HIP_DEVICE_COMPILE__)
ZKV_HD uint32_t zkv_parity() { return __builtin_amdgcn_mbcnt_hi(~0u, __builtin_amdgcn_mbcnt_lo(~0u, 0u)) & 1u; }
ZKV_HD uint32_t zkv_partner_u32(uint32_t x) { return (uint32_t)__builtin_amdgcn_mov_dpp((int)x, 0xB1, 0xF, 0xF, true); }
ZKV_HD uint32_t zkv_pair_even_u32(uint32_t x) { return (uint32_t)__builtin_amdgcn_mov_dpp((int)x, 0xA0, 0xF, 0xF, true); }
ZKV_HD uint32_t zkv_pair_odd_u32(uint32_t x) { return (uint32_t)__builtin_amdgcn_mov_dpp((int)x, 0xF5, 0xF, 0xF, true); }
#else
uint32_t zkv_parity();
uint32_t zkv_partner_u32(uint32_t x);
inline uint32_t zkv_pair_even_u32(uint32_t x) { const uint32_t o = zkv_partner_u32(x); return zkv_parity() ? o : x; }
inline uint32_t zkv_pair_odd_u32(uint32_t x) { const uint32_t o = zkv_partner_u32(x); return zkv_parity() ? x : o; }
#endif
ZKV_HD Fp zkv_partner(const Fp& a) {
    Fp r;
#pragma unroll
    for (int i = 0; i < 8; i++) r.v[i] = zkv_partner_u32(a.v[i]);
    return r;
}
ZKV_HD Fp fp_sel(bool odd, const Fp& if_odd, const Fp& if_even) {
    Fp r;
#pragma unroll
    for (int i = 0; i < 8; i++) r.v[i] = odd ? if_odd.v[i] : if_even.v[i];
    return r;
}
ZKV_HD Fp2 f2_const(const Fp2C& c) { Fp2 r; r.h = fp_sel(zkv_parity() != 0, c.c1, c.c0); return r; }
ZKV_HD Fp2 f2_zero() { Fp2 r; r.h = fp_zero(); return r; }
ZKV_HD Fp2 f2_one() { Fp2 r; r.h = fp_sel(zkv_parity() != 0, fp_zero(), fp_one()); return r; }
ZKV_HD bool f2_is_zero(const Fp2& a) {
    uint32_t o = fp_is_zero(a.h) ? 0u : 1u;
    o |= zkv_partner_u32(o);
    return o == 0;
}
ZKV_HD bool f2_eq(const Fp2& a, const Fp2& b) {
    uint32_t o = fp_eq(a.h, b.h) ? 0u : 1u;
    o |= zkv_partner_u32(o);
    return o == 0;
}
ZKV_HD Fp2 f2_add(const Fp2& a, const Fp2& b) { Fp2 r; r.h = fp_add(a.h, b.h); return r; }
ZKV_HD Fp2 f2_sub(const Fp2& a, const Fp2& b) { Fp2 r; r.h = fp_sub(a.h, b.h); return r; }
ZKV_HD Fp2 f2_neg(const Fp2& a) { Fp2 r; r.h = fp_neg(a.h); return r; }
ZKV_HD Fp2 f2_add_nr(const Fp2& a, const Fp2& b) { Fp2 r; r.h = fp_add_nr(a.h, b.h); return r; }
ZKV_HD Fp2 f2_dbl(const Fp2& a) { return f2_add(a, a); }
ZKV_HD Fp2 f2_half(const Fp2& a) { Fp2 r; r.h = fp_half(a.h); return r; }
ZKV_HD Fp2 f2_conj(const Fp2& a) { Fp2 r; r.h = fp_sel(zkv_parity() != 0, fp_neg(a.h), a.h); return r; }
#if defined(ZKV_FP_MUL_NOINLINE)
ZKV_HD_NI
#else
ZKV_HD
#endif
Fp f2_mul_lane(Fp my_a, Fp my_b) {
#if defined(ZKV_COUNT_FP_MUL)
    zkv_fp_mul_counter += 2;
#endif
    const uint32_t FAT[9] = ZKV_FP_FAT8P_LIMBS;
    const bool odd = zkv_parity() != 0;
    uint32_t xa[9], xo[9], yb[9], U[9], V[9];
    fp_unpack29(my_a, xa); fp_unpack29(my_b, yb);
#pragma unroll
    for (int i = 0; i < 9; i++) { xo[i] = zkv_partner_u32(xa[i]); U[i] = zkv_pair_even_u32(yb[i]); V[i] = zkv_pair_odd_u32(yb[i]); }
    if (!odd) {
#pragma unroll
        for (int i = 0; i < 9; i++) V[i] = FAT[i] - V[i];
    }
    uint64_t col[18];
#pragma unroll
    for (int k = 0; k < 18; k++) col[k] = 0;
    fp_mac81(col, xa, U); fp_mac81(col, xo, V);
    return fp_reduce_cols(col);
}
ZKV_HD Fp2 f2_mul(const Fp2& a, const Fp2& b) { Fp2 r; r.h = f2_mul_lane(a.h, b.h); return r; }
ZKV_HD void f2_limbs_x(const Fp& v, uint32_t (&own)[9], uint32_t (&par)[9]) {
    fp_unpack29(v, own);
#pragma unroll
    for (int i = 0; i < 9; i++) par[i] = zkv_partner_u32(own[i]);
}
ZKV_HD void f2_limbs_y(const Fp& v, uint32_t (&U)[9], uint32_t (&V)[9]) {
    const uint32_t FAT[9] = ZKV_FP_FAT8P_LIMBS;
    uint32_t y[9];
    fp_unpack29(v, y);
#pragma unroll
    for (int i = 0; i < 9; i++) { U[i] = zkv_pair_even_u32(y[i]); V[i] = zkv_pair_odd_u32(y[i]); }
    if (zkv_parity() == 0) {
#pragma unroll
        for (int i = 0; i < 9; i++) V[i] = FAT[i] - V[i];
    }
}
ZKV_HD Fp f2_dot2_limbs(const uint32_t (&ao)[9], const uint32_t (&ap)[9], const uint32_t (&bU)[9], const uint32_t (&bV)[9],
                        const uint32_t (&co)[9], const uint32_t (&cp)[9], const uint32_t (&dU)[9], const uint32_t (&dV)[9]) {
#if defined(ZKV_COUNT_FP_MUL)
    zkv_fp_mul_counter += 4;
#endif
    uint64_t col[18];
#pragma unroll
    for (int k = 0; k < 18; k++) col[k] = 0;
    fp_mac81(col, ao, bU); fp_mac81(col, ap, bV); fp_mac81(col, co, dU); fp_mac81(col, cp, dV);
    return fp_reduce_cols(col);
}
ZKV_HD Fp f2_mul_limbs(const uint32_t (&ao)[9], const uint32_t (&ap)[9], const uint32_t (&bU)[9], const uint32_t (&bV)[9]) {
#if defined(ZKV_COUNT_FP_MUL)
    zkv_fp_mul_counter += 2;
#endif
    uint64_t col[18];
#pragma unroll
    for (int k = 0; k < 18; k++) col[k] = 0;
    fp_mac81(col, ao, bU); fp_mac81(col, ap, bV);
    return fp_reduce_cols(col);
}
struct L9 { uint32_t l[9]; };
ZKV_HD L9 l9_from_fp(const Fp& a) { L9 r; fp_unpack29(a, r.l); return r; }
ZKV_HD Fp l9_to_fp(const L9& a) { return fp_pack29(a.l); }
ZKV_HD L9 l9_partner(const L9& a) {
    L9 r;
#pragma unroll
    for (int i = 0; i < 9; i++) r.l[i] = zkv_partner_u32(a.l[i]);
    return r;
}
ZKV_HD L9 l9_mul_core(const L9& a, const L9& b) {
#if defined(ZKV_COUNT_FP_MUL)
    zkv_fp_mul_counter += 2;
#endif
    const uint32_t FAT[9] = ZKV_FP_FAT8P_LIMBS;
    uint32_t xo[9], U[9], V[9];
    uint64_t col[18];
#pragma unroll
    for (int k = 0; k < 18; k++) col[k] = 0;
#pragma unroll
    for (int i = 0; i < 9; i++) U[i] = zkv_pair_even_u32(b.l[i]);
    fp_mac81(col, a.l, U);
#pragma unroll
    for (int i = 0; i < 9; i++) { xo[i] = zkv_partner_u32(a.l[i]); V[i] = zkv_pair_odd_u32(b.l[i]); }
    if (zkv_parity() == 0) {
#pragma unroll
        for (int i = 0; i < 9; i++) V[i] = FAT[i] - V[i];
    }
    fp_mac81(col, xo, V);
    L9 r; fp_reduce_cols_limbs(col, r.l);
    return r;
}
#if defined(__HIP_DEVICE_COMPILE__) && defined(ZKV_FP_MUL_NOINLINE)
#define ZKV_L9P(p) uint32_t p##0, uint32_t p##1, uint32_t p##2, uint32_t p##3, uint32_t p##4, uint32_t p##5, uint32_t p##6, uint32_t p##7, uint32_t p##8
#define ZKV_L9A(f) f.l[0], f.l[1], f.l[2], f.l[3], f.l[4], f.l[5], f.l[6], f.l[7], f.l[8]
#define ZKV_L9MK(f, p) L9 f; f.l[0] = p##0; f.l[1] = p##1; f.l[2] = p##2; f.l[3] = p##3; f.l[4] = p##4; f.l[5] = p##5; f.l[6] = p##6; f.l[7] = p##7; f.l[8] = p##8
__device__ __noinline__ inline L9 l9_mul_ni(ZKV_L9P(pa), ZKV_L9P(pb)) {
    ZKV_L9MK(a, pa); ZKV_L9MK(b, pb);
    return l9_mul_core(a, b);
}
ZKV_HD L9 l9_mul(const L9& a, const L9& b) { return l9_mul_ni(ZKV_L9A(a), ZKV_L9A(b)); }
#else
ZKV_HD L9 l9_mul(const L9& a, const L9& b) { return l9_mul_core(a, b); }
#endif
struct LTerm { const uint32_t* x; int32_t k; };
#define ZKV_L9_G 256
template <int N> ZKV_HD L9 l9_lincomb(const LTerm (&t)[N], const int c) {
    const uint32_t P29[9] = ZKV_FP_P29_LIMBS;
    const int32_t D = (int32_t)P29[8] + 1;
    const uint32_t M = (uint32_t)(((1ull << 53) + (uint64_t)D - 1) / (uint64_t)D);
    int32_t top = 0;
#pragma unroll
    for (int j = 0; j < N; j++) top += t[j].k * (int32_t)t[j].x[8];
    const uint32_t tt = (uint32_t)(top + c * D - c - ZKV_L9_G);
    const int32_t nq = c - (int32_t)(uint32_t)(((uint64_t)tt * M) >> 53);
    L9 y; int64_t carry = 0;
#pragma unroll
    for (int i = 0; i < 9; i++) {
        int64_t s = carry;
#pragma unroll
        for (int j = 0; j < N; j++) s += (int64_t)t[j].k * (int64_t)(int32_t)t[j].x[i];
        s += (int64_t)nq * (int64_t)(int32_t)P29[i];
        if (i < 8) { y.l[i] = (uint32_t)s & 0x1fffffffu; carry = s >> 29; }
        else y.l[i] = (uint32_t)s;
    }
    return y;
}
ZKV_HD Fp2 f2_sqr(const Fp2& a) {
    const bool odd = zkv_parity() != 0;
    Fp o = zkv_partner(a.h);
    Fp x = fp_add_nr(a.h, fp_sel(odd, a.h, o));
    Fp y = fp_sel(odd, o, fp_sub(a.h, o));
    Fp2 r; r.h = fp_mul(x, y);
    return r;
}
ZKV_HD Fp2 f2_mul_fp(const Fp2& a, const Fp& k) { Fp2 r; r.h = fp_mul(a.h, k); return r; }
ZKV_HD Fp2 f2_mul_xi(const Fp2& a) {
    const uint32_t P2[8] = ZKV_FP_2P_LIMBS;
    const bool odd = zkv_parity() != 0;
    Fp n; uint32_t br = 0;
#pragma unroll
    for (int i = 0; i < 8; i++) n.v[i] = subb(P2[i], a.h.v[i], br);
    const Fp o = zkv_partner(fp_sel(odd, n, a.h));
    uint32_t t[9], c = 0;
#pragma unroll
    for (int i = 0; i < 8; i++) t[i] = addc(a.h.v[i], o.v[i], c);
    t[8] = c;
    uint32_t sh[9];
    sh[0] = a.h.v[0] << 3;
#pragma unroll
    for (int i = 1; i < 8; i++) sh[i] = (a.h.v[i] << 3) | (a.h.v[i - 1] >> 29);
    sh[8] = a.h.v[7] >> 29;
    c = 0;
#pragma unroll
    for (int i = 0; i < 9; i++) t[i] = addc(t[i], sh[i], c);
    const uint32_t x = (t[8] << 12) | (t[7] >> 20);
    const uint32_t q = (uint32_t)(((uint64_t)x * 0x2a4effu) >> 32);
    uint64_t carry = 0;
    Fp r, s2; br = 0;
#pragma unroll
    for (int i = 0; i < 8; i++) { carry += (uint64_t)q * P2[i]; r.v[i] = subb(t[i], (uint32_t)carry, br); carry >>= 32; }
    br = 0;
#pragma unroll
    for (int i = 0; i < 8; i++) s2.v[i] = subb(r.v[i], P2[i], br);
    Fp2 out;
#pragma unroll
    for (int i = 0; i < 8; i++) out.h.v[i] = br ? r.v[i] : s2.v[i];
    return out;
}
ZKV_HD Fp2 f2_inv(const Fp2& a) {
    Fp sq = fp_sqr(a.h);
    Fp n = fp_add(sq, zkv_partner(sq));
    Fp i = fp_inv(n);
    Fp m = fp_mul(a.h, i);
    Fp2 r; r.h = fp_sel(zkv_parity() != 0, fp_neg(m), m);
    return r;
}
#endif

ZKV_HD Fp6 f6_zero() { Fp6 r; r.c0 = f2_zero(); r.c1 = f2_zero(); r.c2 = f2_zero(); return r; }
#if defined(ZKV_PAIRED)
constexpr int F6N = 3;
ZKV_HD void f6_flat(const Fp6& a, Fp (&o)[3]) { o[0] = a.c0.h; o[1] = a.c1.h; o[2] = a.c2.h; }
ZKV_HD Fp6 f6_unflat(const Fp (&o)[3]) { Fp6 r; r.c0.h = o[0]; r.c1.h = o[1]; r.c2.h = o[2]; return r; }
#else
constexpr int F6N = 6;
ZKV_HD void f6_flat(const Fp6& a, Fp (&o)[6]) { o[0] = a.c0.c0; o[1] = a.c0.c1; o[2] = a.c1.c0; o[3] = a.c1.c1; o[4] = a.c2.c0; o[5] = a.c2.c1; }
ZKV_HD Fp6 f6_unflat(const Fp (&o)[6]) { Fp6 r; r.c0.c0 = o[0]; r.c0.c1 = o[1]; r.c1.c0 = o[2]; r.c1.c1 = o[3]; r.c2.c0 = o[4]; r.c2.c1 = o[5]; return r; }
#endif
ZKV_HD Fp6 f6_add(const Fp6& a, const Fp6& b) { Fp x[F6N], y[F6N], r[F6N]; f6_flat(a, x); f6_flat(b, y); fp_add_n<F6N>(x, y, r); return f6_unflat(r); }
ZKV_HD Fp6 f6_sub(const Fp6& a, const Fp6& b) { Fp x[F6N], y[F6N], r[F6N]; f6_flat(a, x); f6_flat(b, y); fp_sub_n<F6N>(x, y, r); return f6_unflat(r); }
ZKV_HD Fp6 f6_neg(const Fp6& a) { Fp x[F6N], z[F6N], r[F6N]; f6_flat(a, x); for (int k = 0; k < F6N; k++) z[k] = fp_zero(); fp_sub_n<F6N>(z, x, r); return f6_unflat(r); }
ZKV_HD Fp6 f6_mul_v(const Fp6& a) { Fp6 r; r.c0 = f2_mul_xi(a.c2); r.c1 = a.c0; r.c2 = a.c1; return r; }
ZKV_HD Fp6 f6_mul(const Fp6& a, const Fp6& b) {
    Fp2 v0 = f2_mul(a.c0, b.c0), v1 = f2_mul(a.c1, b.c1), v2 = f2_mul(a.c2, b.c2);
    Fp6 t, u, w;
    t.c0 = f2_mul(f2_add_nr(a.c1, a.c2), f2_add_nr(b.c1, b.c2));
    t.c1 = f2_mul(f2_add_nr(a.c0, a.c1), f2_add_nr(b.c0, b.c1));
    t.c2 = f2_mul(f2_add_nr(a.c0, a.c2), f2_add_nr(b.c0, b.c2));
    u.c0 = v1; u.c1 = v0; u.c2 = v0;
    w.c0 = v2; w.c1 = v1; w.c2 = v2;
    t = f6_sub(f6_sub(t, u), w);
    u.c0 = v0; u.c1 = t.c1; u.c2 = t.c2;
    w.c0 = f2_mul_xi(t.c0); w.c1 = f2_mul_xi(v2); w.c2 = v1;
    return f6_add(u, w);
}
ZKV_HD Fp6 f6_mul_by_01(const Fp6& a, const Fp2& b0, const Fp2& b1) {
    Fp2 v0 = f2_mul(a.c0, b0), v1 = f2_mul(a.c1, b1);
    Fp6 r;
    r.c1 = f2_sub(f2_sub(f2_mul(f2_add_nr(a.c0, a.c1), f2_add_nr(b0, b1)), v0), v1);
    r.c0 = f2_add(v0, f2_mul_xi(f2_mul(a.c2, b1)));
    r.c2 = f2_add(v1, f2_mul(a.c2, b0));
    return r;
}
ZKV_HD Fp6 f6_mul_fp2(const Fp6& a, const Fp2& k) { Fp6 r; r.c0 = f2_mul(a.c0, k); r.c1 = f2_mul(a.c1, k); r.c2 = f2_mul(a.c2, k); return r; }
ZKV_HD Fp6 f6_inv(const Fp6& a) {
    Fp2 A = f2_sub(f2_sqr(a.c0), f2_mul_xi(f2_mul(a.c1, a.c2)));
    Fp2 B = f2_sub(f2_mul_xi(f2_sqr(a.c2)), f2_mul(a.c0, a.c1));
    Fp2 C = f2_sub(f2_sqr(a.c1), f2_mul(a.c0, a.c2));
    Fp2 F = f2_add(f2_mul_xi(f2_add(f2_mul(a.c2, B), f2_mul(a.c1, C))), f2_mul(a.c0, A));
    F = f2_inv(F);
    Fp6 r; r.c0 = f2_mul(A, F); r.c1 = f2_mul(B, F); r.c2 = f2_mul(C, F);
    return r;
}

}
```

stylus_zkvm_verifiers_amd/csrc/zkv_internal.h:

```cpp
#pragma once
#include <hip/hip_runtime.h>
#include "zkv_verify.h"

namespace zkv {

constexpr int WS_PREP_WORDS = 64 + 8 * MAX_VAR;
constexpr int WS_NORM_WORDS = 48;
constexpr int WS_F_WORDS = 96;
constexpr int WS_FE_WORDS = 7 * 96;
struct Workspace {
    uint32_t* prep; uint32_t* norm; uint32_t* f; uint32_t* fe; uint32_t* flags;
    uint32_t* g2bad;
    size_t cap;
};

constexpr int ZKV_BLOCK = 64;

__device__ __forceinline__ Fp ws_ld(const uint32_t* base, size_t cap, int word0, size_t i) {
    Fp r;
#pragma unroll
    for (int k = 0; k < 8; k++) r.v[k] = base[(size_t)(word0 + k) * cap + i];
    return r;
}
__device__ __forceinline__ void ws_st(uint32_t* base, size_t cap, int word0, size_t i, const Fp& a) {
#pragma unroll
    for (int k = 0; k < 8; k++) base[(size_t)(word0 + k) * cap + i] = a.v[k];
}

struct PrepArgs {
    size_t n;
    const uint8_t* blob;
    const uint64_t* off;
    uint32_t stride;
    const uint8_t* in32_a;
    const uint8_t* in32_b;
    const uint8_t* pv_blob;
    const uint64_t* pv_off;
    uint32_t pv_stride;
    uint32_t selector_be;
    uint32_t force_fail;
    uint32_t n_sig;
    uint32_t negate_a;
    const uint32_t* len;
    const uint8_t* kind;
    const uint32_t* pv_len;
    const uint32_t* inst; const InstTab* inst_tab; uint32_t n_inst;
    uint32_t* plonk_tab;
    uint32_t not_initialized;
    uint8_t* status; uint8_t* recv;
};

struct WireArgs {
    size_t n;
    const uint8_t* cd;
    const uint64_t* off;
    uint64_t cd_bytes;
    uint32_t sel_a_be, sel_b_be;
    uint8_t* seals;
    uint32_t* seal_len;
    uint8_t* in_a; uint8_t* in_b;
    uint8_t* kind;
    uint8_t* pv; uint64_t* pv_off; uint32_t* pv_len;
};
void launch_wire_risc0(const WireArgs& a, hipStream_t s);
void launch_wire_sp1(const WireArgs& a, hipStream_t s);

void launch_setup(const VkRaw* d_raw, VkTables* d_tab, hipStream_t s);
void launch_prep_risc0(const PrepArgs& a, const Risc0Consts& k, const Workspace& ws, hipStream_t s);
void launch_prep_sp1(const PrepArgs& a, const Workspace& ws, hipStream_t s);
void launch_prep_groth16(const PrepArgs& a, const Workspace& ws, hipStream_t s);
void launch_setup_msm16(const VkTables* d_tab, const Msm16& m, G1A* tab, uint32_t rows, hipStream_t s);
void launch_msm(size_t n, const VkTables* d_tab, const Msm16& m16, const InstTab* inst_tab, const Workspace& ws, hipStream_t s);
void launch_msm_w(size_t n, const VkTables* d_tab, const InstTab* inst_tab, const Workspace& ws, hipStream_t s);
void launch_setup_long(const uint32_t* d_ic, uint32_t n_sig, VkTables* d_tab, G1A* tab, uint32_t* win, hipStream_t s);
void launch_prep_groth16_long(const PrepArgs& a, const Workspace& ws, uint32_t* sig, size_t stride, hipStream_t s);
void launch_msm_long(size_t n, uint32_t lanes, const VkTables* d_tab, const LongKey& lk, const Workspace& ws, hipStream_t s);
void launch_vk_x_long(size_t n, uint32_t lanes, const VkTables* d_tab, const LongKey& lk, const uint8_t* sig, uint8_t* out, hipStream_t s);
void launch_status_to_bool(size_t n, uint8_t* status, hipStream_t s);
void launch_setup_instances(const VkRaw* d_raw, const InstConsts& k, const InstRaw* d_in, InstTab* d_out, uint32_t n_inst, hipStream_t s);
void launch_vk_x(size_t n, const VkTables* d_tab, const Msm16& m16, const InstTab* inst_tab, const uint32_t* inst, const uint8_t* sig, uint8_t* out, hipStream_t s);
void launch_g2chk2(size_t n, const Workspace& ws, uint8_t* status, hipStream_t s);
void launch_miller2(size_t n, const VkTables* d_tab, const Workspace& ws, uint8_t* status, hipStream_t s);
void launch_finalexp2(size_t n, const Workspace& ws, uint8_t* status, hipStream_t s);
void launch_miller_w(size_t n, const VkTables* d_tab, const Workspace& ws, hipStream_t s);
void launch_finalexp_w(size_t n, const Workspace& ws, uint8_t* status, hipStream_t s);
void launch_miller_w64(size_t n, const VkTables* d_tab, const Workspace& ws, hipStream_t s);
void launch_finalexp_w64(size_t n, const Workspace& ws, uint8_t* status, hipStream_t s);
void launch_miller_w64d(size_t n, const VkTables* d_tab, const Workspace& ws, uint8_t* status, hipStream_t s);

struct MixedArgs {
    size_t n;
    const uint8_t* vm;
    const uint8_t* method;
    const uint8_t* seals; const uint64_t* seal_off; uint32_t seal_stride;
    const uint8_t* in_a;
    const uint8_t* in_b; const uint64_t* b_off; uint32_t b_stride, pv_len;
    const uint32_t* cnt; const uint32_t* totals;
    uint32_t* pos; uint32_t* idx;
    uint8_t* c_seals; uint32_t* c_len; uint8_t* c_a; uint8_t* c_b; uint64_t* c_pvoff; uint32_t* c_pvlen;
    uint8_t* c_kind;
    uint8_t* status; uint8_t* recv;
};
void launch_mixed_partition(const MixedArgs& a, uint32_t* cnt, uint32_t* totals, hipStream_t s);
void launch_mixed_return(size_t m, const uint32_t* idx, const uint8_t* c_status, const uint8_t* c_recv, uint8_t* status, uint8_t* recv, hipStream_t s);

constexpr int GW_MAX_ROUTES = 8, GW_COL_NOT_FOUND = 8, GW_COL_SHORT = 9, GW_COLS = 10;
constexpr uint32_t GW_NONE = 0xFFFFFFFFu;
struct GatewayArgs {
    size_t n;
    const uint8_t* proofs; const uint64_t* proof_off; uint64_t proof_bytes;
    const uint8_t* vkeys;
    const uint64_t* pv_off; uint64_t pv_stride;
    uint32_t n_routes;
    uint32_t sel[GW_MAX_ROUTES];
    uint32_t rec[GW_MAX_ROUTES];
    uint32_t start[GW_MAX_ROUTES]; uint64_t base[GW_MAX_ROUTES];
    uint32_t* cnt; uint32_t* totals;
    uint32_t* pos; uint32_t* idx;
    uint8_t* c_proofs; uint32_t* c_len; uint8_t* c_a; uint64_t* c_pvoff; uint32_t* c_pvlen;
    uint8_t* status; uint8_t* recv;
};
void launch_gateway_count(const GatewayArgs& a, hipStream_t s);
void launch_gateway_place(const GatewayArgs& a, hipStream_t s);

struct GsetKey { const VkTables* tab; uint32_t sig0, n_sig, negate, pad; };
constexpr uint32_t GSET_NONE = 0xFFFFFFFFu;
struct GsetPart {
    size_t n; uint32_t n_keys, blocks, per_block;
    const uint32_t* key;
    uint32_t* cnt;
    uint32_t* totals;
    uint32_t* off;
    uint32_t* idx; uint32_t* skey;
    uint32_t* pos;
};
struct GsetChunk {
    size_t m, slot0;
    const uint32_t* idx; const uint32_t* skey;
    const GsetKey* keys; const G1A* rows; const uint32_t* win;
    const uint8_t* proofs; const uint8_t* signals; uint32_t sig_stride;
    uint32_t* sig; size_t sig_cap;
    uint8_t* status;
};
void launch_gset_setup(uint32_t n_keys, const VkRaw* d_raw, VkTables* d_tabs, uint32_t n_sig_all, const uint32_t* d_ic, const uint32_t* d_sig_key,
                       G1A* rows, uint32_t* win, hipStream_t s);
void launch_gset_count(const GsetPart& p, hipStream_t s);
void launch_gset_place(const GsetPart& p, const uint64_t* d_start, hipStream_t s);
void launch_gset_prep(const GsetChunk& c, const Workspace& ws, hipStream_t s);
void launch_gset_msm(const GsetChunk& c, uint32_t lanes, const Workspace& ws, hipStream_t s);
void launch_gset_vk_x(size_t n, uint32_t lanes, const uint32_t* key, const GsetKey* keys, const G1A* rows, const uint32_t* win, const uint8_t* sig,
                      uint32_t sig_stride, uint8_t* out, hipStream_t s);
void launch_gset_return(size_t n, const uint32_t* pos, const uint8_t* status, uint8_t* verified, hipStream_t s);
void launch_gset_miller(int lanes, size_t m, const uint32_t* skey, const GsetKey* keys, const Workspace& ws, uint8_t* status, hipStream_t s);
int read_gset_wait_faults(unsigned long long* out);
struct AggTables;
void launch_gset_setup_agg(uint32_t n_keys, const VkRaw* d_raw, const VkTables* d_tabs, AggTables* d_agg, hipStream_t s);
__global__ void k_gset_scan(GsetPart p, const uint64_t* __restrict__ start);
void launch_gset_agg_place(const GsetPart& p, const uint64_t* d_zero, const uint64_t* d_map, hipStream_t s);
void launch_gset_agg_miller(size_t n, uint32_t g, const uint32_t* skey, const GsetKey* keys, const Workspace& ws, uint8_t* status, hipStream_t s);
void launch_gset_agg_reduce(const GsetChunk& c, uint32_t sub, uint32_t g, const Workspace& ws, const uint32_t* agg, const AggTables* tabs,
                            const Workspace& ws2, uint8_t* status2, const uint32_t* psl, bool park, hipStream_t s);
void launch_gset_agg_combine(const GsetChunk& c, size_t n2, uint32_t wide, const AggTables* tabs, const Workspace& ws2, uint8_t* status2, const uint32_t* psl,
                             hipStream_t s);
void launch_gset_agg_fprod(size_t n, size_t n2, uint32_t sub, uint32_t g, const Workspace& ws, const uint32_t* agg, const Workspace& ws2, const uint32_t* psl,
                           hipStream_t s);
void launch_gset_agg_mark(size_t n, uint32_t sub, uint32_t g, const Workspace& ws, const uint32_t* agg, const uint8_t* status2, const uint32_t* psl,
                          uint8_t* status, unsigned long long* counters, hipStream_t s);

#ifndef ZKV_PLONK_PROOF_BYTES
#define ZKV_PLONK_PROOF_BYTES 868
#endif
struct PlonkKeyRaw; struct PlonkKey;
void launch_plonk_setup(const PlonkKeyRaw* d_raw, PlonkKey* d_key, hipStream_t s);
void launch_plonk_setup_keys(const PlonkKeyRaw* d_raw, PlonkKey* d_key, hipStream_t s);
void launch_plonk_prep(const PrepArgs& a, const PlonkKey* d_key, const Workspace& ws, hipStream_t s);
void launch_plonk_prep_keys(const PrepArgs& a, const PlonkKey* d_key, const Workspace& ws, hipStream_t s);
struct PsetChunk {
    size_t m, slot0;
    const uint32_t* idx; const uint32_t* skey;
    const PlonkKey* keys; const uint32_t* ok;
    const uint8_t* proofs; uint32_t proof_stride;
    const uint8_t* inputs; uint32_t input_stride;
    uint32_t* plonk_tab;
    uint8_t* status;
};
void launch_pset_setup(uint32_t n_keys, const PlonkKeyRaw* d_raw, PlonkKey* d_keys, const VkTables* d_tabs, uint32_t* d_ok, hipStream_t s);
void launch_pset_prep(const PsetChunk& c, const Workspace& ws, hipStream_t s);
void launch_pset_agg_reduce(size_t m, uint32_t sub, const Workspace& ws, const uint32_t* agg, const Workspace& ws2, uint8_t* status2, const uint32_t* psl,
                            bool park, hipStream_t s);
void launch_pset_agg_combine(size_t n2, uint32_t wide, const Workspace& ws2, uint8_t* status2, const uint32_t* psl, hipStream_t s);

int read_wait_faults(unsigned long long* out);
void launch_diag_mulmod(int kind, unsigned blocks, uint32_t iters, uint32_t* out, unsigned long long* clk, hipStream_t s);
void launch_diag_issue(int kind, unsigned blocks, uint32_t iters, uint32_t* out, unsigned long long* clk, hipStream_t s);
void launch_selftest_lane(int op, unsigned waves, const uint32_t* in, uint32_t* out, hipStream_t s);
void launch_selftest_pair(int mapping, int op, unsigned waves, const uint32_t* in, uint32_t* out, hipStream_t s);

struct AggTables; struct AggSeed;
void launch_setup_agg(const VkRaw* d_raw, const VkTables* d_tab, AggTables* d_agg, hipStream_t s);
void launch_agg_g1(size_t n, const VkTables* d_tab, const InstTab* inst_tab, const Workspace& ws, uint32_t* agg, const AggSeed& seed, bool sums, hipStream_t s);
void launch_agg_reduce(size_t n, uint32_t sub, bool sums, uint32_t g, const VkTables* d_tab, const Workspace& ws, const uint32_t* agg, const AggTables* tab,
                       const Workspace& ws2, uint8_t* status2, bool park, hipStream_t s);
void launch_agg_combine(size_t n64, size_t n2, uint32_t wide, const AggTables* tab, const Workspace& ws2, uint8_t* status2, hipStream_t s);
void launch_agg_miller(size_t n, uint32_t g, const VkTables* d_tab, const Workspace& ws, uint8_t* status, hipStream_t s);
void launch_agg_fprod(size_t n, size_t n2, uint32_t sub, uint32_t g, const Workspace& ws, const uint32_t* agg, const Workspace& ws2, hipStream_t s);
void launch_agg_mark(size_t n, uint32_t sub, uint32_t g, const Workspace& ws, const uint32_t* agg, const uint8_t* status2, uint8_t* status, unsigned long long* counters,
                     uint32_t* idx, hipStream_t s);
void launch_agg_gather(size_t n, const Workspace& ws, const uint32_t* agg, const unsigned long long* counters, const uint32_t* idx, const Workspace& ws3,
                       uint8_t* status3, hipStream_t s);
void launch_agg_plonk_g1(size_t n, const Workspace& ws, uint32_t* agg, const AggSeed& seed, hipStream_t s);
void launch_agg_plonk_norm(size_t n, const Workspace& ws, const uint32_t* agg, const unsigned long long* counters, const uint32_t* idx, const Workspace& ws3,
                           uint8_t* status3, hipStream_t s);
void launch_agg_scatter(size_t n, const unsigned long long* counters, const uint32_t* idx, const uint8_t* status3, uint8_t* status, hipStream_t s);

void launch_ecadd(size_t n, const uint8_t* in, uint8_t* out, uint8_t* ok, hipStream_t s);
void launch_ecmul(size_t n, const uint8_t* in, uint8_t* out, uint8_t* ok, hipStream_t s);
void launch_pairing(size_t n, uint32_t k, const uint8_t* in, const Workspace& ws, uint8_t* result, uint8_t* ok, hipStream_t s);
uint32_t pairing_group(uint32_t k);
void launch_pairing_w(size_t n, uint32_t k, const uint8_t* in, const Workspace& ws, uint8_t* result, uint8_t* ok, hipStream_t s);

}
```

stylus_zkvm_verifiers_amd/csrc/zkv_tower_mem.h:

```cpp
#pragma once
#include "zkv_curve.h"

namespace zkv {

struct MRef {
    uint32_t* p; uint32_t stride; uint32_t f2w;
    ZKV_HD uint32_t ld(int k) const { return p[(size_t)k * stride]; }
    ZKV_HD void st(int k, uint32_t v) const { p[(size_t)k * stride] = v; }
    ZKV_HD int fw() const { return (int)f2w; }
};
ZKV_HD MRef m_ref(uint32_t* p, uint32_t stride, uint32_t f2w = 16) { MRef r; r.p = p; r.stride = stride; r.f2w = f2w; return r; }
ZKV_HD MRef m_off(MRef m, int words) { MRef r = m; r.p = m.p + (size_t)words * m.stride; return r; }

struct SoaRW {
    uint32_t* p; size_t stride; uint32_t off;
    ZKV_HD uint32_t ld(int k) const { return *(const uint32_t*)((const char*)(p + (size_t)k * stride) + off); }
    ZKV_HD void st(int k, uint32_t v) const { *(uint32_t*)((char*)(p + (size_t)k * stride) + off) = v; }
    ZKV_HD int fw() const { return 16; }
};
template <class R> ZKV_HD R m_fresh(R r) { return r; }
ZKV_HD SoaRW m_fresh(SoaRW r) {
#if defined(__HIP_DEVICE_COMPILE__)
    asm volatile("" : "+v"(r.off));
#endif
    return r;
}

#if defined(__HIP_DEVICE_COMPILE__)
typedef __attribute__((address_space(3))) uint32_t zkv_lds_u32;
#else
typedef uint32_t zkv_lds_u32;
#endif
struct LRef {
    zkv_lds_u32* p;
    ZKV_HD uint32_t ld(int k) const { return p[k * 64]; }
    ZKV_HD void st(int k, uint32_t v) const { p[k * 64] = v; }
#if defined(ZKV_PAIRED)
    ZKV_HD int fw() const { return 8; }
#else
    ZKV_HD int fw() const { return 16; }
#endif
};
ZKV_HD LRef l_ref(uint32_t* lds_base_plus_lane) { LRef r; r.p = (zkv_lds_u32*)lds_base_plus_lane; return r; }

template <class R> ZKV_HD Fp m_ld_fp(R m, int word0) {
    Fp r;
#pragma unroll
    for (int k = 0; k < 8; k++) r.v[k] = m.ld(word0 + k);
    return r;
}
template <class R> ZKV_HD void m_st_fp(R m, int word0, const Fp& a) {
#pragma unroll
    for (int k = 0; k < 8; k++) m.st(word0 + k, a.v[k]);
}
#if defined(ZKV_PAIRED)
template <class R> ZKV_HD Fp2 m_ld_f2(R m, int idx) { Fp2 r; r.h = m_ld_fp(m, m.fw() * idx); return r; }
template <class R> ZKV_HD void m_st_f2(R m, int idx, const Fp2& a) { m_st_fp(m, m.fw() * idx, a.h); }
#else
template <class R> ZKV_HD Fp2 m_ld_f2(R m, int idx) { Fp2 r; r.c0 = m_ld_fp(m, 16 * idx); r.c1 = m_ld_fp(m, 16 * idx + 8); return r; }
template <class R> ZKV_HD void m_st_f2(R m, int idx, const Fp2& a) { m_st_fp(m, 16 * idx, a.c0); m_st_fp(m, 16 * idx + 8, a.c1); }
#endif
template <class R> ZKV_HD Fp6 m_ld_f6(R m, int idx) { Fp6 r; r.c0 = m_ld_f2(m, idx); r.c1 = m_ld_f2(m, idx + 1); r.c2 = m_ld_f2(m, idx + 2); return r; }
template <class R> ZKV_HD void m_st_f6(R m, int idx, const Fp6& a) { m_st_f2(m, idx, a.c0); m_st_f2(m, idx + 1, a.c1); m_st_f2(m, idx + 2, a.c2); }
template <class RD, class RA> ZKV_HD void f12m_copy(RD d, RA a) {
#pragma unroll 1
    for (int k = 0; k < 6; k++) m_st_f2(d, k, m_ld_f2(a, k));
}
template <class RD> ZKV_HD void f12m_set_one(RD d) {
    m_st_f2(d, 0, f2_one());
#pragma unroll 1
    for (int k = 1; k < 6; k++) m_st_f2(d, k, f2_zero());
}
template <class RD> ZKV_HD void f12m_conj(RD d) {
#pragma unroll 1
    for (int k = 3; k < 6; k++) m_st_f2(d, k, f2_neg(m_ld_f2(d, k)));
}
template <class RA> ZKV_HD bool f12m_is_one(RA a) {
    bool ok = f2_eq(m_ld_f2(a, 0), f2_one());
#pragma unroll 1
    for (int k = 1; k < 6; k++) ok = f2_is_zero(m_ld_f2(a, k)) && ok;
    return ok;
}

template <class RF> ZKV_HD void f12m_sqr_body(RF f) {
    Fp6 g = m_ld_f6(f, 0), h = m_ld_f6(f, 3);
    Fp6 t = f6_mul(g, h);
    Fp6 s = f6_mul(f6_add(g, h), f6_add(g, f6_mul_v(h)));
    m_st_f6(f, 0, f6_sub(f6_sub(s, t), f6_mul_v(t)));
    m_st_f6(f, 3, f6_add(t, t));
}
template <class RF> ZKV_HD_NI void f12m_sqr(RF f) { f12m_sqr_body(f); }
ZKV_HD void fp4_sqr(const Fp2& a, const Fp2& b, Fp2& t0, Fp2& t1) {
    Fp2 tmp = f2_mul(a, b);
    t0 = f2_sub(f2_sub(f2_mul(f2_add(a, b), f2_add(f2_mul_xi(b), a)), tmp), f2_mul_xi(tmp));
    t1 = f2_dbl(tmp);
}
template <class RF> ZKV_HD void f12m_cyclo_sqr_body(RF f) {
    Fp2 z0 = m_ld_f2(f, 0), z1 = m_ld_f2(f, 4), t0, t1;
    fp4_sqr(z0, z1, t0, t1);
    z0 = f2_sub(t0, z0); z0 = f2_add(f2_dbl(z0), t0);
    z1 = f2_add(t1, z1); z1 = f2_add(f2_dbl(z1), t1);
    m_st_f2(f, 0, z0); m_st_f2(f, 4, z1);
    Fp2 z2 = m_ld_f2(f, 3), z3 = m_ld_f2(f, 2), t2, t3;
    fp4_sqr(z2, z3, t2, t3);
    Fp2 z4 = m_ld_f2(f, 1), z5 = m_ld_f2(f, 5), t4, t5;
    fp4_sqr(z4, z5, t4, t5);
    Fp2 x = f2_mul_xi(t5);
    z2 = f2_add(x, z2); z2 = f2_add(f2_dbl(z2), x);
    z3 = f2_sub(t4, z3); z3 = f2_add(f2_dbl(z3), t4);
    z4 = f2_sub(t2, z4); z4 = f2_add(f2_dbl(z4), t2);
    z5 = f2_add(t3, z5); z5 = f2_add(f2_dbl(z5), t3);
    m_st_f2(f, 3, z2); m_st_f2(f, 2, z3); m_st_f2(f, 1, z4); m_st_f2(f, 5, z5);
}
template <class RF> ZKV_HD_NI void f12m_cyclo_sqr(RF f) { f12m_cyclo_sqr_body(f); }
#if defined(ZKV_PAIRED)
struct L9Ref {
    zkv_lds_u32* p;
    ZKV_HD int fw() const { return 8; }
};
ZKV_HD L9Ref l9_ref(uint32_t* lds_base_plus_lane) { L9Ref r; r.p = (zkv_lds_u32*)lds_base_plus_lane; return r; }
ZKV_HD L9 l9_ld(L9Ref m, int idx) {
    L9 r;
#pragma unroll
    for (int k = 0; k < 9; k++) r.l[k] = m.p[(9 * idx + k) * 64];
    return r;
}
ZKV_HD void l9_st(L9Ref m, int idx, const L9& a) {
#pragma unroll
    for (int k = 0; k < 9; k++) m.p[(9 * idx + k) * 64] = a.l[k];
}
ZKV_HD Fp m_ld_fp(L9Ref m, int word0) { return l9_to_fp(l9_ld(m, word0 >> 3)); }
ZKV_HD void m_st_fp(L9Ref m, int word0, const Fp& a) { l9_st(m, word0 >> 3, l9_from_fp(a)); }

ZKV_HD void l9_fp4_sqr_update(const L9& a, const L9& b, const L9& za, const L9& zb, const bool xi_t1, L9& o0, L9& o1) {
    const bool odd = zkv_parity() != 0;
    const int32_t k1 = odd ? 1 : -1, k3 = odd ? -3 : 3;
    const L9 tmp = l9_mul(a, b);
    L9 s1, s2;
#pragma unroll
    for (int i = 0; i < 9; i++) s1.l[i] = a.l[i] + b.l[i];
    {
        const L9 pb = l9_partner(b);
        const LTerm t[3] = {{a.l, 1}, {b.l, 9}, {pb.l, k1}};
        s2 = l9_lincomb(t, 4);
    }
    const L9 S = l9_mul(s1, s2);
    const L9 tp = l9_partner(tmp);
    {
        const LTerm t[4] = {{S.l, 3}, {tmp.l, -30}, {tp.l, k3}, {za.l, -2}};
        o0 = l9_lincomb(t, 72);
    }
    if (!xi_t1) {
        const LTerm t[2] = {{tmp.l, 6}, {zb.l, 2}};
        o1 = l9_lincomb(t, 1);
    } else {
        const LTerm t[3] = {{tmp.l, 54}, {tp.l, -2 * k3}, {zb.l, 2}};
        o1 = l9_lincomb(t, 14);
    }
}
ZKV_HD void f12l9_cyclo_sqr(L9Ref f) {
    {
        const L9 a = l9_ld(f, 0), b = l9_ld(f, 4);
        L9 o0, o1;
        l9_fp4_sqr_update(a, b, a, b, false, o0, o1);
        l9_st(f, 0, o0); l9_st(f, 4, o1);
    }
    L9 n1, n5;
    {
        const L9 a = l9_ld(f, 3), b = l9_ld(f, 2), za = l9_ld(f, 1), zb = l9_ld(f, 5);
        l9_fp4_sqr_update(a, b, za, zb, false, n1, n5);
    }
    {
        const L9 a = l9_ld(f, 1), b = l9_ld(f, 5), za = l9_ld(f, 2), zb = l9_ld(f, 3);
        L9 o0, o1;
        l9_fp4_sqr_update(a, b, za, zb, true, o0, o1);
        l9_st(f, 2, o0); l9_st(f, 3, o1);
    }
    l9_st(f, 1, n1); l9_st(f, 5, n5);
}
ZKV_HD void l9_carry(uint32_t (&x)[9]) {
#pragma unroll
    for (int k = 0; k < 8; k++) { x[k + 1] += x[k] >> 29; x[k] &= 0x1fffffffu; }
}
struct L9F6Raw { L9 v0, v2; int32_t wa[9], wb[9], wc[9]; };
template <class LDA, class LDB> ZKV_HD void l9_f6_mul_raw(LDA lda, LDB ldb, L9F6Raw& r) {
    const L9 b0 = ldb(0), b1 = ldb(1), b2 = ldb(2);
    r.v0 = l9_mul(lda(0), b0);
    const L9 v1 = l9_mul(lda(1), b1);
    r.v2 = l9_mul(lda(2), b2);
    L9 sa, sb, m;
    { const L9 a1 = lda(1), a2 = lda(2);
#pragma unroll
      for (int i = 0; i < 9; i++) { sa.l[i] = a1.l[i] + a2.l[i]; sb.l[i] = b1.l[i] + b2.l[i]; } }
    l9_carry(sb.l); m = l9_mul(sa, sb);
#pragma unroll
    for (int i = 0; i < 9; i++) r.wa[i] = (int32_t)m.l[i] - (int32_t)v1.l[i] - (int32_t)r.v2.l[i];
    { const L9 a0 = lda(0), a1 = lda(1);
#pragma unroll
      for (int i = 0; i < 9; i++) { sa.l[i] = a0.l[i] + a1.l[i]; sb.l[i] = b0.l[i] + b1.l[i]; } }
    l9_carry(sb.l); m = l9_mul(sa, sb);
#pragma unroll
    for (int i = 0; i < 9; i++) r.wb[i] = (int32_t)m.l[i] - (int32_t)r.v0.l[i] - (int32_t)v1.l[i];
    { const L9 a0 = lda(0), a2 = lda(2);
#pragma unroll
      for (int i = 0; i < 9; i++) { sa.l[i] = a0.l[i] + a2.l[i]; sb.l[i] = b0.l[i] + b2.l[i]; } }
    l9_carry(sb.l); m = l9_mul(sa, sb);
#pragma unroll
    for (int i = 0; i < 9; i++) r.wc[i] = (int32_t)m.l[i] - (int32_t)r.v0.l[i] - (int32_t)r.v2.l[i] + (int32_t)v1.l[i];
}
ZKV_HD void l9_partner_i32(const int32_t (&a)[9], int32_t (&o)[9]) {
#pragma unroll
    for (int i = 0; i < 9; i++) o[i] = (int32_t)zkv_partner_u32((uint32_t)a[i]);
}
template <class RB> ZKV_HD void f12l9_mul(L9Ref acc, RB S0, const bool conj_b) {
    const int32_t k1 = zkv_parity() != 0 ? 1 : -1;
    L9F6Raw raw;
    int32_t pw[9];
    L9 xc0, xc1, xc2;
    {
        const RB S = m_fresh(S0);
        l9_f6_mul_raw([&](int i) { return l9_ld(acc, i); }, [&](int i) { return l9_from_fp(m_ld_f2(S, i).h); }, raw);
        l9_partner_i32(raw.wa, pw);
        { const LTerm t[3] = {{raw.v0.l, 1}, {(const uint32_t*)raw.wa, 9}, {(const uint32_t*)pw, k1}}; xc0 = l9_lincomb(t, 48); }
        const L9 pv2 = l9_partner(raw.v2);
        { const LTerm t[3] = {{(const uint32_t*)raw.wb, 1}, {raw.v2.l, 9}, {pv2.l, k1}}; xc1 = l9_lincomb(t, 8); }
        { const LTerm t[1] = {{(const uint32_t*)raw.wc, 1}}; xc2 = l9_lincomb(t, 8); }
    }
    uint32_t xy0[9], xy1[9], xy2[9];
    {
        L9 g0, g1, g2;
        const RB S = m_fresh(S0);
        l9_f6_mul_raw([&](int i) { return l9_ld(acc, 3 + i); }, [&](int i) {
            Fp2 b = m_ld_f2(S, 3 + i);
            if (conj_b) b = f2_neg(b);
            return l9_from_fp(b.h);
        }, raw);
        L9 yc0, yc1, yc2;
        l9_partner_i32(raw.wa, pw);
        { const LTerm t[3] = {{raw.v0.l, 1}, {(const uint32_t*)raw.wa, 9}, {(const uint32_t*)pw, k1}}; yc0 = l9_lincomb(t, 48); }
        const L9 pv2 = l9_partner(raw.v2);
        { const LTerm t[3] = {{(const uint32_t*)raw.wb, 1}, {raw.v2.l, 9}, {pv2.l, k1}}; yc1 = l9_lincomb(t, 8); }
        { const LTerm t[1] = {{(const uint32_t*)raw.wc, 1}}; yc2 = l9_lincomb(t, 8); }
        const L9 pyc2 = l9_partner(yc2);
        { const LTerm t[3] = {{xc0.l, 1}, {yc2.l, 9}, {pyc2.l, k1}}; g0 = l9_lincomb(t, 4); }
        { const LTerm t[2] = {{xc1.l, 1}, {yc0.l, 1}}; g1 = l9_lincomb(t, 1); }
        { const LTerm t[2] = {{xc2.l, 1}, {yc1.l, 1}}; g2 = l9_lincomb(t, 1); }
#pragma unroll
        for (int i = 0; i < 9; i++) { xy0[i] = xc0.l[i] + yc0.l[i]; xy1[i] = xc1.l[i] + yc1.l[i]; xy2[i] = xc2.l[i] + yc2.l[i]; }
#pragma unroll
        for (int i = 0; i < 3; i++) {
            const L9 g = l9_ld(acc, i), h = l9_ld(acc, 3 + i);
            L9 sum;
#pragma unroll
            for (int k = 0; k < 9; k++) sum.l[k] = g.l[k] + h.l[k];
            l9_carry(sum.l);
            l9_st(acc, 3 + i, sum);
        }
        l9_st(acc, 0, g0); l9_st(acc, 1, g1); l9_st(acc, 2, g2);
    }
    L9 h0, h1, h2;
    {
        const RB S = m_fresh(S0);
        l9_f6_mul_raw([&](int i) { return l9_ld(acc, 3 + i); }, [&](int i) {
            Fp2 b = m_ld_f2(S, 3 + i);
            if (conj_b) b = f2_neg(b);
            return l9_from_fp(f2_add(m_ld_f2(S, i), b).h);
        }, raw);
        l9_partner_i32(raw.wa, pw);
        { const LTerm t[4] = {{raw.v0.l, 1}, {(const uint32_t*)raw.wa, 9}, {(const uint32_t*)pw, k1}, {xy0, -1}}; h0 = l9_lincomb(t, 52); }
        const L9 pv2 = l9_partner(raw.v2);
        { const LTerm t[4] = {{(const uint32_t*)raw.wb, 1}, {raw.v2.l, 9}, {pv2.l, k1}, {xy1, -1}}; h1 = l9_lincomb(t, 12); }
        { const LTerm t[2] = {{(const uint32_t*)raw.wc, 1}, {xy2, -1}}; h2 = l9_lincomb(t, 12); }
    }
    l9_st(acc, 3, h0); l9_st(acc, 4, h1); l9_st(acc, 5, h2);
}
#endif

template <class RD, class RA, class RB> ZKV_HD void f12m_mul_body(RD d, RA a, RB b, bool conj_b) {
    Fp6 ag = m_ld_f6(a, 0), bg = m_ld_f6(b, 0);
    Fp6 t0 = f6_mul(ag, bg);
    Fp6 ah = m_ld_f6(a, 3), bh = m_ld_f6(b, 3);
    if (conj_b) bh = f6_neg(bh);
    Fp6 t1 = f6_mul(ah, bh);
    Fp6 m = f6_mul(f6_add(ag, ah), f6_add(bg, bh));
    d = m_fresh(d);
    m_st_f6(d, 3, f6_sub(f6_sub(m, t0), t1));
    m_st_f6(d, 0, f6_add(t0, f6_mul_v(t1)));
}
template <class RD, class RA, class RB> ZKV_HD_NI void f12m_mul(RD d, RA a, RB b) { f12m_mul_body(d, a, b, false); }
template <class RD, class RA, class RB> ZKV_HD_NI void f12m_mul_conj(RD d, RA a, RB b) { f12m_mul_body(d, a, b, true); }
#if defined(ZKV_PAIRED)
template <class RF> ZKV_HD void f12m_mul_by_034_body(RF f, const Fp2& c0, const Fp2& c3, const Fp2& c4) {
    uint32_t c0U[9], c0V[9], c4U[9], c4V[9], tU[9], tV[9], xo[9], xp[9];
    f2_limbs_y(c0.h, c0U, c0V); f2_limbs_y(c4.h, c4U, c4V);
    Fp2 t0c0, t0c1, t0c2, t1c0, t1c1, t1c2;
    {
        const Fp2 h0 = m_ld_f2(f, 3), h1 = m_ld_f2(f, 4), h2 = m_ld_f2(f, 5);
        Fp2 p4, p5, p6, p7, p8;
        f2_limbs_y(c3.h, tU, tV);
        f2_limbs_x(h0.h, xo, xp); p4.h = f2_mul_limbs(xo, xp, tU, tV);
        f2_limbs_x(h2.h, xo, xp); p8.h = f2_mul_limbs(xo, xp, tU, tV); p7.h = f2_mul_limbs(xo, xp, c4U, c4V);
        f2_limbs_x(h1.h, xo, xp); p5.h = f2_mul_limbs(xo, xp, c4U, c4V);
        f2_limbs_y(f2_add_nr(c3, c4).h, tU, tV);
        f2_limbs_x(f2_add_nr(h0, h1).h, xo, xp); p6.h = f2_mul_limbs(xo, xp, tU, tV);
        t1c0 = f2_add(p4, f2_mul_xi(p7)); t1c1 = f2_sub(f2_sub(p6, p4), p5); t1c2 = f2_add(p5, p8);
    }
    Fp2 s0, s1, s2;
    {
        const Fp2 g0 = m_ld_f2(f, 0), g1 = m_ld_f2(f, 1), g2 = m_ld_f2(f, 2);
        f2_limbs_x(g0.h, xo, xp); t0c0.h = f2_mul_limbs(xo, xp, c0U, c0V);
        f2_limbs_x(g1.h, xo, xp); t0c1.h = f2_mul_limbs(xo, xp, c0U, c0V);
        f2_limbs_x(g2.h, xo, xp); t0c2.h = f2_mul_limbs(xo, xp, c0U, c0V);
        s0 = f2_add(g0, m_ld_f2(f, 3)); s1 = f2_add(g1, m_ld_f2(f, 4)); s2 = f2_add(g2, m_ld_f2(f, 5));
    }
    m_st_f2(f, 0, f2_add(t0c0, f2_mul_xi(t1c2))); m_st_f2(f, 1, f2_add(t0c1, t1c0)); m_st_f2(f, 2, f2_add(t0c2, t1c1));
    const Fp2 b0 = f2_add(c0, c3);
    Fp2 w0, w1, n, q;
    f2_limbs_y(b0.h, tU, tV);
    f2_limbs_x(s0.h, xo, xp); w0.h = f2_mul_limbs(xo, xp, tU, tV);
    f2_limbs_x(s2.h, xo, xp); q.h = f2_mul_limbs(xo, xp, tU, tV);
    Fp2 q2; q2.h = f2_mul_limbs(xo, xp, c4U, c4V);
    f2_limbs_x(s1.h, xo, xp); w1.h = f2_mul_limbs(xo, xp, c4U, c4V);
    f2_limbs_y(f2_add_nr(b0, c4).h, tU, tV);
    f2_limbs_x(f2_add_nr(s0, s1).h, xo, xp); n.h = f2_mul_limbs(xo, xp, tU, tV);
    m_st_f2(f, 3, f2_sub(f2_sub(f2_add(w0, f2_mul_xi(q2)), t0c0), t1c0));
    m_st_f2(f, 4, f2_sub(f2_sub(f2_sub(f2_sub(n, w0), w1), t0c1), t1c1));
    m_st_f2(f, 5, f2_sub(f2_sub(f2_add(w1, q), t0c2), t1c2));
}
#else
template <class RF> ZKV_HD void f12m_mul_by_034_body(RF f, const Fp2& c0, const Fp2& c3, const Fp2& c4) {
    Fp6 g = m_ld_f6(f, 0), h = m_ld_f6(f, 3);
    Fp6 t0 = f6_mul_fp2(g, c0);
    Fp6 t1 = f6_mul_by_01(h, c3, c4);
    Fp6 t2 = f6_mul_by_01(f6_add(g, h), f2_add(c0, c3), c4);
    m_st_f6(f, 3, f6_sub(f6_sub(t2, t0), t1));
    m_st_f6(f, 0, f6_add(t0, f6_mul_v(t1)));
}
#endif
template <class RF> ZKV_HD_NI void f12m_mul_by_034(RF f, const Fp2* c0, const Fp2* c3, const Fp2* c4) { f12m_mul_by_034_body(f, *c0, *c3, *c4); }
#if defined(ZKV_PAIRED)
template <class RF> ZKV_HD void f12m_mul_by_134_body(RF f, const Fp2& c3, const Fp2& c4) {
    uint32_t c3U[9], c3V[9], c4U[9], c4V[9], x3U[9], x3V[9], x4U[9], x4V[9];
    f2_limbs_y(c3.h, c3U, c3V); f2_limbs_y(c4.h, c4U, c4V);
    { const Fp2 x3 = f2_mul_xi(c3), x4 = f2_mul_xi(c4); f2_limbs_y(x3.h, x3U, x3V); f2_limbs_y(x4.h, x4U, x4V); }
    Fp ng0, ng1, ng2, nh0, nh1, nh2;
    {
        uint32_t h0o[9], h0p[9], h1o[9], h1p[9], h2o[9], h2p[9];
        f2_limbs_x(m_ld_f2(f, 3).h, h0o, h0p); f2_limbs_x(m_ld_f2(f, 4).h, h1o, h1p); f2_limbs_x(m_ld_f2(f, 5).h, h2o, h2p);
        ng0 = fp_add(m_ld_f2(f, 0).h, f2_dot2_limbs(h1o, h1p, x4U, x4V, h2o, h2p, x3U, x3V));
        ng1 = fp_add(m_ld_f2(f, 1).h, f2_dot2_limbs(h0o, h0p, c3U, c3V, h2o, h2p, x4U, x4V));
        ng2 = fp_add(m_ld_f2(f, 2).h, f2_dot2_limbs(h0o, h0p, c4U, c4V, h1o, h1p, c3U, c3V));
    }
    {
        uint32_t g0o[9], g0p[9], g1o[9], g1p[9], g2o[9], g2p[9];
        f2_limbs_x(m_ld_f2(f, 0).h, g0o, g0p); f2_limbs_x(m_ld_f2(f, 1).h, g1o, g1p); f2_limbs_x(m_ld_f2(f, 2).h, g2o, g2p);
        nh0 = fp_add(m_ld_f2(f, 3).h, f2_dot2_limbs(g0o, g0p, c3U, c3V, g2o, g2p, x4U, x4V));
        nh1 = fp_add(m_ld_f2(f, 4).h, f2_dot2_limbs(g0o, g0p, c4U, c4V, g1o, g1p, c3U, c3V));
        nh2 = fp_add(m_ld_f2(f, 5).h, f2_dot2_limbs(g1o, g1p, c4U, c4V, g2o, g2p, c3U, c3V));
    }
    Fp2 o;
    o.h = ng0; m_st_f2(f, 0, o); o.h = ng1; m_st_f2(f, 1, o); o.h = ng2; m_st_f2(f, 2, o);
    o.h = nh0; m_st_f2(f, 3, o); o.h = nh1; m_st_f2(f, 4, o); o.h = nh2; m_st_f2(f, 5, o);
}
#else
template <class RF> ZKV_HD void f12m_mul_by_134_body(RF f, const Fp2& c3, const Fp2& c4) {
    Fp6 g = m_ld_f6(f, 0), h = m_ld_f6(f, 3);
    Fp6 hs = f6_mul_by_01(h, c3, c4);
    Fp6 gs = f6_mul_by_01(g, c3, c4);
    m_st_f6(f, 0, f6_add(g, f6_mul_v(hs)));
    m_st_f6(f, 3, f6_add(h, gs));
}
#endif
template <class RF> ZKV_HD_NI void f12m_mul_by_134(RF f, const Fp2* c3, const Fp2* c4) { f12m_mul_by_134_body(f, *c3, *c4); }
template <class RD, class RA> ZKV_HD void f12m_inv_body(RD d, RA a) {
    Fp6 g = m_ld_f6(a, 0), h = m_ld_f6(a, 3);
    Fp6 t = f6_sub(f6_mul(g, g), f6_mul_v(f6_mul(h, h)));
    t = f6_inv(t);
    d = m_fresh(d);
    m_st_f6(d, 0, f6_mul(g, t));
    m_st_f6(d, 3, f6_neg(f6_mul(h, t)));
}
template <class RD, class RA> ZKV_HD_NI void f12m_inv(RD d, RA a) { f12m_inv_body(d, a); }
ZKV_TABLE Fp2C ZKV_FROB1_TAB[6] = ZKV_FROB1;
ZKV_TABLE Fp ZKV_FROB2_TAB[6] = ZKV_FROB2;
ZKV_TABLE Fp2C ZKV_FROB3_TAB[6] = ZKV_FROB3;
template <class RD, class RA> ZKV_HD void f12m_frob_body(RD d, RA a, int k) {
    const Fp2C* G1 = ZKV_FROB1_TAB; const Fp* G2 = ZKV_FROB2_TAB; const Fp2C* G3 = ZKV_FROB3_TAB;
    const int wp[6] = {0, 2, 4, 1, 3, 5};
#pragma unroll 1
    for (int i = 0; i < 6; i++) {
        Fp2 c = m_ld_f2(a, i);
        int e = wp[i];
        if (k == 2) c = f2_mul_fp(c, G2[e]);
        else {
            c = f2_conj(c);
            if (e) c = f2_mul(c, f2_const(k == 1 ? G1[e] : G3[e]));
        }
        m_st_f2(d, i, c);
    }
}
template <class RD, class RA> ZKV_HD_NI void f12m_frob(RD d, RA a, int k) { f12m_frob_body(d, a, k); }

template <class RT> ZKV_HD_NI void g2m_line_dbl(RT Tm, Fp2* l0, Fp2* l1, Fp2* l3) {
    G2H T; T.x = m_ld_f2(Tm, 0); T.y = m_ld_f2(Tm, 1); T.z = m_ld_f2(Tm, 2);
    line_dbl(T, *l0, *l1, *l3);
    m_st_f2(Tm, 0, T.x); m_st_f2(Tm, 1, T.y); m_st_f2(Tm, 2, T.z);
}
template <class RT> ZKV_HD_NI void g2m_line_add(RT Tm, const Fp2* qx, const Fp2* qy, Fp2* l0, Fp2* l1, Fp2* l3) {
    G2H T; T.x = m_ld_f2(Tm, 0); T.y = m_ld_f2(Tm, 1); T.z = m_ld_f2(Tm, 2);
    line_add(T, *qx, *qy, *l0, *l1, *l3);
    m_st_f2(Tm, 0, T.x); m_st_f2(Tm, 1, T.y); m_st_f2(Tm, 2, T.z);
}

}
```

stylus_zkvm_verifiers_amd/csrc/zkv_verify.h:

```cpp
#pragma once
#include "zkv_tower_mem.h"
#include "zkv_sha256.h"

namespace zkv {

enum : uint8_t {
    ST_OK = 0, ST_VERIFICATION_FAILED = 1, ST_INVALID_INITIALIZATION = 2, ST_ALREADY_INITIALIZED = 3,
    ST_INVALID_PROOF_DATA = 4, ST_SELECTOR_MISMATCH = 5,
    ST_BAD_CALLDATA = 6
};
enum : uint32_t { FL_ALIVE = 1u, FL_A_INF = 2u, FL_B_INF = 4u, FL_C_INF = 8u, FL_L_INF = 16u };

constexpr int N_LINES = 88;
constexpr int MSM_MAX_WINDOWS = 32;
constexpr int MSM_DIGITS = 256;
constexpr int MAX_IC = 6;
constexpr int MAX_VAR = 5;

struct VkRaw {
    uint32_t alpha[2][8];
    uint32_t beta[4][8], gamma[4][8], delta[4][8];
    uint32_t ic[MAX_IC][2][8];
    uint32_t n_ic;
    uint32_t fixed_scalar[MAX_IC][8];
    uint32_t is_fixed[MAX_IC];
    uint32_t n_var;
    uint32_t var_ic[MAX_VAR];
    uint32_t var_windows[MAX_VAR];
};

struct VkTables {
    G1A base; uint32_t base_inf; uint32_t n_var; uint32_t var_windows[MAX_VAR];
    uint32_t vk_valid;
    uint32_t skip_fixed[2];
    G1A msm[MAX_VAR][MSM_MAX_WINDOWS][MSM_DIGITS];
    LineAffC lines[2][N_LINES];
    uint32_t f_alpha_beta[96];
};

constexpr uint32_t MSM16_MAX_ROWS = 32;
struct Msm16 { const G1A* tab; uint32_t row0[MAX_VAR]; };
struct LongKey {
    const G1A* tab; const uint32_t* win;
    const uint32_t* sig; size_t stride;
    uint32_t n_sig;
};
constexpr uint32_t LONG_ROW_ENTRIES = MSM_MAX_WINDOWS * MSM_DIGITS;

struct InstRaw { uint8_t control_root[32]; uint8_t control_id[32]; };
struct InstConsts { uint8_t tag[32]; uint8_t vk_digest[32]; };
struct InstTab { G1A base; uint32_t base_inf, selector_be, fail, pad; };

struct PrepOut {
    Fp ax, ay, cx, cy; Fp2 bx, by;
    uint32_t s[MAX_VAR][8];
    uint32_t flags;
};
struct G1Norm { Fp axs, ays, lxs, lys, cxs, cys; };

ZKV_HD int8_t ate_naf(int i) {
    const int8_t NAF[ZKV_ATE_NAF_LEN] = ZKV_ATE_NAF;
    return NAF[i];
}

ZKV_HD void load_be256(uint32_t limbs[8], const uint8_t* p) {
#pragma unroll 1
    for (int i = 0; i < 8; i++) limbs[7 - i] = load_be32(p + 4 * i);
}
ZKV_HD bool raw_is_zero(const uint32_t* a) {
    uint32_t o = 0;
    for (int i = 0; i < 8; i++) o |= a[i];
    return o == 0;
}
ZKV_HD bool raw_lt_p(const uint32_t* a) { const uint32_t P[8] = ZKV_FP_P_LIMBS; return !u256_geq(a, P); }
ZKV_HD bool raw_lt_r(const uint32_t* a) { const uint32_t R[8] = ZKV_FR_R_LIMBS; return !u256_geq(a, R); }

struct Risc0Consts { uint32_t tag_output[8]; uint32_t claim_mid[8]; uint32_t post[8]; };

#if !defined(ZKV_PAIRED)
ZKV_HD bool prep_points(uint32_t w[8][8], bool negate_a, PrepOut& o) {
    const uint32_t P[8] = ZKV_FP_P_LIMBS;
    if (negate_a && !(raw_is_zero(w[0]) && raw_is_zero(w[1]))) {
        uint32_t br = 0;
        for (int i = 0; i < 8; i++) w[1][i] = subb(P[i], w[1][i], br);
    }
    bool ok = true;
    for (int k = 0; k < 8; k++) ok = ok && raw_lt_p(w[k]);
    if (!ok) return false;
    uint32_t fl = 0;
    if (raw_is_zero(w[0]) && raw_is_zero(w[1])) {
        fl |= FL_A_INF; o.ax = fp_zero(); o.ay = fp_zero();
    } else {
        o.ax = fp_from_raw(w[0]); o.ay = fp_from_raw(w[1]);
        if (!g1_on_curve(o.ax, o.ay)) return false;
    }
    if (raw_is_zero(w[6]) && raw_is_zero(w[7])) {
        fl |= FL_C_INF; o.cx = fp_zero(); o.cy = fp_zero();
    } else {
        o.cx = fp_from_raw(w[6]); o.cy = fp_from_raw(w[7]);
        if (!g1_on_curve(o.cx, o.cy)) return false;
    }
    if (raw_is_zero(w[2]) && raw_is_zero(w[3]) && raw_is_zero(w[4]) && raw_is_zero(w[5])) {
        fl |= FL_B_INF; o.bx = f2_zero(); o.by = f2_zero();
    } else {
        o.bx.c1 = fp_from_raw(w[2]); o.bx.c0 = fp_from_raw(w[3]);
        o.by.c1 = fp_from_raw(w[4]); o.by.c0 = fp_from_raw(w[5]);
        if (!g2_on_twist(o.bx, o.by)) return false;
    }
    o.flags = fl | FL_ALIVE;
    return true;
}


ZKV_HD void risc0_claim_digest(const Risc0Consts& k, const uint8_t* image_id, const uint8_t* journal, uint32_t h[8]) {
    uint32_t w[16], out[8];
    sha256_init(out);
    for (int i = 0; i < 8; i++) { w[i] = k.tag_output[i]; w[8 + i] = load_be32(journal + 4 * i); }
    sha256_compress(out, w);
    for (int i = 0; i < 8; i++) w[i] = 0;
    w[8] = 0x02008000u;
    for (int i = 9; i < 15; i++) w[i] = 0;
    w[15] = 98u * 8u;
    sha256_compress(out, w);
    for (int i = 0; i < 8; i++) h[i] = k.claim_mid[i];
    for (int i = 0; i < 8; i++) { w[i] = load_be32(image_id + 4 * i); w[8 + i] = k.post[i]; }
    sha256_compress(h, w);
    for (int i = 0; i < 8; i++) w[i] = out[i];
    w[8] = 0; w[9] = 0;
    w[10] = 0x04008000u;
    for (int i = 11; i < 15; i++) w[i] = 0;
    w[15] = 170u * 8u;
    sha256_compress(h, w);
}
ZKV_HD void risc0_split_digest(const uint32_t h[8], uint32_t lo[8], uint32_t hi[8]) {
    for (int i = 0; i < 4; i++) {
        lo[i] = __builtin_bswap32(h[i]); hi[i] = __builtin_bswap32(h[4 + i]);
        lo[4 + i] = 0; hi[4 + i] = 0;
    }
}

template <class WORD> ZKV_HD G1J msm_accumulate_w(const VkTables& vk, WORD word, const G1A& base, uint32_t base_inf) {
    G1J acc;
    if (base_inf) acc = g1j_infinity();
    else { acc.x = base.x; acc.y = base.y; acc.z = fp_one(); }
#pragma unroll 1
    for (uint32_t b = 0; b < vk.n_var; b++) {
#pragma unroll 1
        for (uint32_t w = 0; w < vk.var_windows[b]; w++) {
            uint32_t d = (word(b, w >> 2) >> ((w & 3) * 8)) & 255u;
            if (d) {
                const G1A& e = vk.msm[b][w][d];
                acc = g1j_add_affine(acc, e.x, e.y);
            }
        }
    }
    return acc;
}
template <class WORD> ZKV_HD G1J msm_accumulate_w16(const VkTables& vk, const Msm16& m, WORD word, const G1A& base, uint32_t base_inf) {
    G1J acc;
    if (base_inf) acc = g1j_infinity();
    else { acc.x = base.x; acc.y = base.y; acc.z = fp_one(); }
#pragma unroll 1
    for (uint32_t b = 0; b < vk.n_var; b++) {
        const uint32_t nw = vk.var_windows[b];
#pragma unroll 1
        for (uint32_t w = 0; 2 * w < nw; w++) {
            uint32_t d = (word(b, w >> 1) >> ((w & 1) * 16)) & 0xffffu;
            if (2 * w + 1 >= nw) d &= 0xffu;
            if (d) {
                const G1A e = m.tab[((size_t)(m.row0[b] + w) << 16) + d];
                acc = g1j_add_affine(acc, e.x, e.y);
            }
        }
    }
    return acc;
}
ZKV_HD G1J msm_accumulate(const VkTables& vk, const PrepOut& in, const G1A& base, uint32_t base_inf) {
    return msm_accumulate_w(vk, [&](uint32_t b, uint32_t k) { return in.s[b][k]; }, base, base_inf);
}
ZKV_HD G1J msm_accumulate(const VkTables& vk, const PrepOut& in) { return msm_accumulate(vk, in, vk.base, vk.base_inf); }
ZKV_HD void msm_normalize_acc(const G1J& acc, const PrepOut& in, uint32_t& flags, G1Norm& out);
ZKV_HD void msm_normalize(const VkTables& vk, const PrepOut& in, uint32_t& flags, G1Norm& out, const G1A& base, uint32_t base_inf) {
    msm_normalize_acc(msm_accumulate(vk, in, base, base_inf), in, flags, out);
}
ZKV_HD void msm_normalize_acc(const G1J& acc, const PrepOut& in, uint32_t& flags, G1Norm& out) {
    Fp one = fp_one();
    bool linf = fp_is_zero(acc.z), ainf = (flags & FL_A_INF) != 0, cinf = (flags & FL_C_INF) != 0;
    if (linf) flags |= FL_L_INF;
    Fp ya = ainf ? one : in.ay, yl = linf ? one : acc.y, yc = cinf ? one : in.cy;
    Fp t = fp_mul(ya, yl);
    Fp inv = fp_inv(fp_mul(t, yc));
    Fp iyc = fp_mul(inv, t);
    Fp u = fp_mul(inv, yc);
    Fp iyl = fp_mul(u, ya), iya = fp_mul(u, yl);
    out.axs = fp_mul(in.ax, iya); out.ays = iya;
    out.cxs = fp_mul(in.cx, iyc); out.cys = iyc;
    Fp z2 = fp_sqr(acc.z);
    out.lxs = fp_mul(fp_mul(acc.x, acc.z), iyl);
    out.lys = fp_mul(fp_mul(z2, acc.z), iyl);
}
ZKV_HD void msm_normalize(const VkTables& vk, const PrepOut& in, uint32_t& flags, G1Norm& out) { msm_normalize(vk, in, flags, out, vk.base, vk.base_inf); }

template <class DIGIT> ZKV_HD G1J long_msm_slice(uint32_t n_sig, const uint32_t* win, const G1A* tab, DIGIT digit, uint32_t lane, uint32_t lanes) {
    G1J acc = g1j_infinity();
#pragma unroll 1
    for (uint32_t q = lane; q < (uint32_t)MSM_MAX_WINDOWS * n_sig; q += lanes) {
        const uint32_t b = q / MSM_MAX_WINDOWS, w = q % MSM_MAX_WINDOWS;
        if (w >= win[b]) continue;
        const uint32_t d = digit(b, w);
        if (d) { const G1A e = tab[(size_t)q * MSM_DIGITS + d]; acc = g1j_add_affine(acc, e.x, e.y); }
    }
    return acc;
}

#endif

template <class RF> ZKV_HD void fixed_line_mul(RF fm, const LineAffC& L, const Fp& xs, const Fp& ys) {
    Fp2 c3 = f2_mul_fp(f2_const(L.nl), xs), c4 = f2_mul_fp(f2_const(L.c), ys);
    f12m_mul_by_134(fm, &c3, &c4);
}
template <class RF> ZKV_HD void var_line_mul(RF fm, const Fp2& l0, const Fp2& l1, const Fp2& l3, const Fp& xs, const Fp& ys) {
    Fp2 c3 = f2_mul_fp(l1, xs), c4 = f2_mul_fp(l3, ys);
    f12m_mul_by_034(fm, &l0, &c3, &c4);
}
template <class RT> ZKV_HD bool miller_point_closes(RT tm, const Fp2& bx, const Fp2& by) {
    const Fp2C G3[6] = ZKV_FROB3;
    const Fp2 tz = m_ld_f2(tm, 2);
    const Fp2 x3 = f2_mul(f2_mul(f2_conj(bx), f2_const(G3[2])), tz);
    const Fp2 y3 = f2_mul(f2_mul(f2_conj(by), f2_const(G3[3])), tz);
    return !f2_is_zero(tz) && f2_eq(m_ld_f2(tm, 0), x3) && f2_is_zero(f2_add(m_ld_f2(tm, 1), y3));
}
template <class RF, class RT>
ZKV_HD bool miller_loop_m(const VkTables* vkp, uint32_t flags, const G1Norm& n, const Fp2& bx, const Fp2& by, RF fm, RT tm, bool check_b = false) {
    const bool with_fixed = vkp != nullptr;
    const VkTables* vkq = with_fixed ? vkp : nullptr;
    const bool do_ab = !(flags & (FL_A_INF | FL_B_INF));
    const bool do_t = do_ab || (check_b && !(flags & FL_B_INF));
    bool do_l = with_fixed && !(flags & FL_L_INF) && !vkq->skip_fixed[0], do_c = with_fixed && !(flags & FL_C_INF) && !vkq->skip_fixed[1];
    const LineAffC* lines0 = with_fixed ? vkq->lines[0] : nullptr;
    const LineAffC* lines1 = with_fixed ? vkq->lines[1] : nullptr;
    f12m_set_one(fm);
    m_st_f2(tm, 0, bx); m_st_f2(tm, 1, by); m_st_f2(tm, 2, f2_one());
    Fp2 nby = f2_neg(by);
    Fp2 l0, l1, l3;
    int li = 0;
#pragma unroll 1
    for (int i = ZKV_ATE_NAF_LEN - 2; i >= 0; i--) {
        if (i != ZKV_ATE_NAF_LEN - 2) f12m_sqr(fm);
        if (do_t) {
            g2m_line_dbl(tm, &l0, &l1, &l3);
            if (do_ab) var_line_mul(fm, l0, l1, l3, n.axs, n.ays);
        }
        if (do_l) fixed_line_mul(fm, lines0[li], n.lxs, n.lys);
        if (do_c) fixed_line_mul(fm, lines1[li], n.cxs, n.cys);
        li++;
        int d = ate_naf(i);
        if (d != 0) {
            if (do_t) {
                Fp2 qy = d > 0 ? by : nby;
                g2m_line_add(tm, &bx, &qy, &l0, &l1, &l3);
                if (do_ab) var_line_mul(fm, l0, l1, l3, n.axs, n.ays);
            }
            if (do_l) fixed_line_mul(fm, lines0[li], n.lxs, n.lys);
            if (do_c) fixed_line_mul(fm, lines1[li], n.cxs, n.cys);
            li++;
        }
    }
    Fp2 qx[2], qy[2];
    g2_frob_affine(qx[0], qy[0], bx, by);
    g2_frob2_affine(qx[1], qy[1], bx, by);
    qy[1] = f2_neg(qy[1]);
#pragma unroll 1
    for (int s = 0; s < 2; s++) {
        if (do_t) {
            g2m_line_add(tm, &qx[s], &qy[s], &l0, &l1, &l3);
            if (do_ab) var_line_mul(fm, l0, l1, l3, n.axs, n.ays);
        }
        if (do_l) fixed_line_mul(fm, lines0[li], n.lxs, n.lys);
        if (do_c) fixed_line_mul(fm, lines1[li], n.cxs, n.cys);
        li++;
    }
    return !(check_b && do_t) || miller_point_closes(tm, bx, by);
}

#if defined(ZKV_PAIRED)
struct SoaRef {
    const uint32_t* p; size_t stride; uint32_t off;
    ZKV_HD Fp fp(int word0) const {
        Fp r;
#pragma unroll
        for (int k = 0; k < 8; k++) r.v[k] = *(const uint32_t*)((const char*)(p + (size_t)(word0 + k) * stride) + off);
        return r;
    }
};
template <class RF, class RT>
ZKV_HD bool miller_loop_p(const VkTables* vkp, uint32_t flags, SoaRef norm, SoaRef bsrc, RF fm, RT tm, bool check_b = false) {
    const uint8_t KIND[ZKV_MILLER_STEPS] = ZKV_MILLER_STEP_KIND;
    const bool with_fixed = vkp != nullptr;
    const bool do_ab = !(flags & (FL_A_INF | FL_B_INF));
    const bool do_t = do_ab || (check_b && !(flags & FL_B_INF));
    const bool do_l = with_fixed && !(flags & FL_L_INF) && !vkp->skip_fixed[0], do_c = with_fixed && !(flags & FL_C_INF) && !vkp->skip_fixed[1];
    f12m_set_one(fm);
    { Fp2 bx, by; bx.h = bsrc.fp(0); by.h = bsrc.fp(16); m_st_f2(tm, 0, bx); m_st_f2(tm, 1, by); m_st_f2(tm, 2, f2_one()); }
    const uint32_t slot = zkv_wave_slot_parity();
#pragma unroll 1
    for (int li = 0; li < ZKV_MILLER_STEPS; li++) {
        const int kind = KIND[li];
        zkv_fair_share(slot);
#if defined(__HIP_DEVICE_COMPILE__)
        asm volatile("" : "+v"(norm.off), "+v"(bsrc.off));
#endif
        if (kind == 0 && li != 0) { ZKV_MARK("begin sqr"); f12m_sqr_body(fm); ZKV_MARK("end sqr"); }
        if (do_t) {
            Fp2 l0, l1, l3;
            G2H T; T.x = m_ld_f2(tm, 0); T.y = m_ld_f2(tm, 1); T.z = m_ld_f2(tm, 2);
            if (kind == 0) { ZKV_MARK("begin linedbl"); line_dbl(T, l0, l1, l3); ZKV_MARK("end linedbl"); }
            else {
                Fp2 qx, qy; qx.h = bsrc.fp(0); qy.h = bsrc.fp(16);
                if (kind == 2) qy = f2_neg(qy);
                else if (kind == 3) { Fp2 x, y; g2_frob_affine(x, y, qx, qy); qx = x; qy = y; }
                else if (kind == 4) { Fp2 x, y; g2_frob2_affine(x, y, qx, qy); qx = x; qy = f2_neg(y); }
                ZKV_MARK("begin lineadd"); line_add(T, qx, qy, l0, l1, l3); ZKV_MARK("end lineadd");
            }
            m_st_f2(tm, 0, T.x); m_st_f2(tm, 1, T.y); m_st_f2(tm, 2, T.z);
            if (do_ab) {
                ZKV_MARK("begin mul034");
                const Fp2 c3 = f2_mul_fp(l1, norm.fp(0)), c4 = f2_mul_fp(l3, norm.fp(8));
                f12m_mul_by_034_body(fm, l0, c3, c4);
                ZKV_MARK("end mul034");
            }
        }
#pragma unroll 1
        for (int j = 0; j < 2; j++) {
            if (j == 0 ? !do_l : !do_c) continue;
            ZKV_MARK("begin mul134");
            const LineAffC& L = vkp->lines[j][li];
            const Fp2 c3 = f2_mul_fp(f2_const(L.nl), norm.fp(16 + 16 * j)), c4 = f2_mul_fp(f2_const(L.c), norm.fp(24 + 16 * j));
            f12m_mul_by_134_body(fm, c3, c4);
            ZKV_MARK("end mul134");
        }
    }
    if (!check_b || !do_t) return true;
    Fp2 qx, qy; qx.h = bsrc.fp(0); qy.h = bsrc.fp(16);
    return miller_point_closes(tm, qx, qy);
}
template <int G, class RF>
ZKV_HD uint32_t miller_loop_pg(uint32_t mask, uint32_t abmask, SoaRef norm, SoaRef bsrc, SoaRW tq, uint32_t step, RF fm) {
    const uint8_t KIND[ZKV_MILLER_STEPS] = ZKV_MILLER_STEP_KIND;
    f12m_set_one(fm);
#pragma unroll 1
    for (uint32_t p = 0; p < (uint32_t)G; p++) {
        if (!((mask >> p) & 1u)) continue;
        SoaRef b = bsrc; b.off += p * step;
        SoaRW t = tq; t.off += p * step;
        Fp2 bx, by; bx.h = b.fp(0); by.h = b.fp(16);
        m_st_f2(t, 0, bx); m_st_f2(t, 1, by); m_st_f2(t, 2, f2_one());
    }
#pragma unroll 1
    for (int li = 0; li < ZKV_MILLER_STEPS; li++) {
        const int kind = KIND[li];
#if defined(__HIP_DEVICE_COMPILE__)
        asm volatile("" : "+v"(norm.off), "+v"(bsrc.off), "+v"(tq.off));
#endif
        if (kind == 0 && li != 0) f12m_sqr_body(fm);
#pragma unroll 1
        for (uint32_t p = 0; p < (uint32_t)G; p++) {
            if (!((mask >> p) & 1u)) continue;
            SoaRef n = norm; n.off += p * step;
            SoaRef b = bsrc; b.off += p * step;
            SoaRW t = tq; t.off += p * step;
            Fp2 l0, l1, l3;
            G2H T; T.x = m_ld_f2(t, 0); T.y = m_ld_f2(t, 1); T.z = m_ld_f2(t, 2);
            if (kind == 0) line_dbl(T, l0, l1, l3);
            else {
                Fp2 qx, qy; qx.h = b.fp(0); qy.h = b.fp(16);
                if (kind == 2) qy = f2_neg(qy);
                else if (kind == 3) { Fp2 x, y; g2_frob_affine(x, y, qx, qy); qx = x; qy = y; }
                else if (kind == 4) { Fp2 x, y; g2_frob2_affine(x, y, qx, qy); qx = x; qy = f2_neg(y); }
                line_add(T, qx, qy, l0, l1, l3);
            }
            m_st_f2(t, 0, T.x); m_st_f2(t, 1, T.y); m_st_f2(t, 2, T.z);
            if ((abmask >> p) & 1u) {
                const Fp2 c3 = f2_mul_fp(l1, n.fp(0)), c4 = f2_mul_fp(l3, n.fp(8));
                f12m_mul_by_034_body(fm, l0, c3, c4);
            }
        }
    }
    uint32_t fine = (1u << G) - 1u;
#pragma unroll 1
    for (uint32_t p = 0; p < (uint32_t)G; p++) {
        if (!((mask >> p) & 1u)) continue;
        SoaRef b = bsrc; b.off += p * step;
        SoaRW t = tq; t.off += p * step;
        Fp2 qx, qy; qx.h = b.fp(0); qy.h = b.fp(16);
        if (!miller_point_closes(t, qx, qy)) fine &= ~(1u << p);
    }
    return fine;
}
#endif

ZKV_HD int8_t u_digit(int i) {
    const int8_t D[ZKV_U_DIG_LEN] = ZKV_U_DIG;
    return D[i];
}
template <class RA> ZKV_HD void exp_u_m(RA acc, MRef x, MRef W) {
    const MRef X17 = W, X35 = m_off(W, 96);
    f12m_copy(acc, x);
#pragma unroll 1
    for (int k = 0; k < 4; k++) f12m_cyclo_sqr(acc);
    f12m_mul(X17, acc, x);
    f12m_copy(acc, X17); f12m_cyclo_sqr(acc);
    f12m_mul(X35, acc, x);
    { const int t = u_digit(ZKV_U_DIG_LEN - 1); f12m_copy(acc, t == 1 ? x : t == 17 ? X17 : X35); }
#pragma unroll 1
    for (int i = ZKV_U_DIG_LEN - 2; i >= 0; i--) {
        f12m_cyclo_sqr(acc);
        const int d = u_digit(i);
        if (d == 0) continue;
        const int m = d < 0 ? -d : d;
        const MRef S = m == 1 ? x : m == 17 ? X17 : X35;
        if (d > 0) f12m_mul(acc, acc, S);
        else f12m_mul_conj(acc, acc, S);
    }
}
template <class RA> ZKV_HD bool final_exp_is_one_m(MRef F, MRef E, MRef Y1, MRef Y3, MRef Y4, MRef W, RA acc) {
    f12m_copy(acc, F); f12m_conj(acc);
    f12m_inv(F, F);
    f12m_mul(acc, acc, F);
    f12m_frob(F, acc, 2);
    f12m_mul(E, F, acc);
    exp_u_m(acc, E, W); f12m_conj(acc);
    f12m_cyclo_sqr(acc); f12m_copy(Y1, acc);
    f12m_cyclo_sqr(acc);
    f12m_mul(acc, acc, Y1); f12m_copy(Y3, acc);
    exp_u_m(acc, Y3, W); f12m_conj(acc); f12m_copy(Y4, acc);
    f12m_cyclo_sqr(acc); f12m_copy(F, acc);
    exp_u_m(acc, F, W);
    f12m_conj(Y3);
    f12m_mul(acc, acc, Y4);
    f12m_mul(acc, acc, Y3); f12m_copy(Y3, acc);
    f12m_mul(F, acc, Y1);
    f12m_mul(acc, acc, Y4);
    f12m_mul(acc, acc, E);
    f12m_frob(Y1, F, 1);
    f12m_mul(acc, Y1, acc);
    f12m_frob(Y3, Y3, 2);
    f12m_mul(acc, Y3, acc);
    f12m_conj(E);
    f12m_mul(E, E, F);
    f12m_frob(E, E, 3);
    f12m_mul(acc, E, acc);
    return f12m_is_one(acc);
}

#if defined(ZKV_PAIRED)
ZKV_HD SoaRW fe_slot(int s, uint32_t* fbase, uint32_t* ebase, size_t cap, uint32_t off) {
    SoaRW r; r.p = s == 1 ? fbase : ebase + (size_t)(96 * (s - 2)) * cap; r.stride = cap; r.off = off;
    return r;
}
ZKV_HD bool final_exp_prog_p(uint32_t* fbase, uint32_t* ebase, size_t cap, uint32_t off, L9Ref acc) {
    const uint32_t PROG[ZKV_FE_PROG_LEN] = ZKV_FE_PROG;
    bool one = false;
    const uint32_t slot = zkv_wave_slot_parity();
#pragma unroll 1
    for (int pc = 0; pc < ZKV_FE_PROG_LEN; pc++) {
        const uint32_t e = PROG[pc];
        const int op = (int)(e & 255u), d = (int)((e >> 8) & 255u), a = (int)((e >> 16) & 255u), b = (int)(e >> 24);
        if ((pc & 3) == 0) zkv_fair_share(slot);
#if defined(__HIP_DEVICE_COMPILE__)
        asm volatile("" : "+v"(off));
#endif
        if (op == 6) { ZKV_MARK("begin cyclo"); f12l9_cyclo_sqr(acc); ZKV_MARK("end cyclo"); }
        else if ((op == 3 || op == 4) && d == 0) { ZKV_MARK("begin accmul");  f12l9_mul(acc, fe_slot(b, fbase, ebase, cap, off), op == 4); ZKV_MARK("end accmul"); }
        else if (op == 0 && d == 0) f12m_copy(acc, fe_slot(a, fbase, ebase, cap, off));
        else if (op == 0 && a == 0) f12m_copy(fe_slot(d, fbase, ebase, cap, off), acc);
        else if (op == 1 && d == 0) f12m_conj(acc);
        else {
            const SoaRW D = fe_slot(d, fbase, ebase, cap, off), A = fe_slot(a, fbase, ebase, cap, off);
            if (op == 3 || op == 4) { ZKV_MARK("begin genmul"); f12m_mul_body(D, A, fe_slot(b, fbase, ebase, cap, off), op == 4); ZKV_MARK("end genmul"); }
            else if (op == 0) f12m_copy(D, A);
            else if (op == 1) f12m_conj(D);
            else if (op == 2) { ZKV_MARK("begin geninv"); f12m_inv_body(D, A); ZKV_MARK("end geninv"); }
            else if (op == 5) { ZKV_MARK("begin genfrob"); f12m_frob_body(D, A, b); ZKV_MARK("end genfrob"); }
            else one = f12m_is_one(D);
        }
    }
    return one;
}
#endif

#if !defined(ZKV_PAIRED)
ZKV_HD bool raw_g1_is_inf(const uint32_t p[2][8]) { return raw_is_zero(p[0]) && raw_is_zero(p[1]); }
ZKV_HD bool raw_g1_valid(const uint32_t p[2][8]) {
    if (!raw_lt_p(p[0]) || !raw_lt_p(p[1])) return false;
    if (raw_g1_is_inf(p)) return true;
    return g1_on_curve(fp_from_raw(p[0]), fp_from_raw(p[1]));
}
ZKV_HD bool raw_g2_is_inf(const uint32_t q[4][8]) { return raw_is_zero(q[0]) && raw_is_zero(q[1]) && raw_is_zero(q[2]) && raw_is_zero(q[3]); }
ZKV_HD bool raw_g2_valid(const uint32_t q[4][8]) {
    for (int k = 0; k < 4; k++) if (!raw_lt_p(q[k])) return false;
    if (raw_g2_is_inf(q)) return true;
    Fp2 x, y; x.c0 = fp_from_raw(q[0]); x.c1 = fp_from_raw(q[1]); y.c0 = fp_from_raw(q[2]); y.c1 = fp_from_raw(q[3]);
    return g2_on_twist(x, y) && g2_in_subgroup(x, y);
}
ZKV_HD void setup_validate(const VkRaw& vk, VkTables& t) {
    bool ok = raw_g1_valid(vk.alpha) && raw_g2_valid(vk.beta) && raw_g2_valid(vk.gamma) && raw_g2_valid(vk.delta);
    for (uint32_t i = 0; i < vk.n_ic; i++) ok = ok && raw_g1_valid(vk.ic[i]);
    t.vk_valid = ok ? 1u : 0u;
    t.skip_fixed[0] = raw_g2_is_inf(vk.gamma) ? 1u : 0u;
    t.skip_fixed[1] = raw_g2_is_inf(vk.delta) ? 1u : 0u;
}
ZKV_HD LineAffC line_to_table(const LineAff& l) {
    LineAffC r; r.nl.c0 = l.nl.c0; r.nl.c1 = l.nl.c1; r.c.c0 = l.c.c0; r.c.c1 = l.c.c1; return r;
}
ZKV_HD void setup_lines(const uint32_t q[4][8], LineAffC* out) {
    if (raw_g2_is_inf(q)) return;
    G2A Q, T;
    Q.x.c0 = fp_from_raw(q[0]); Q.x.c1 = fp_from_raw(q[1]); Q.y.c0 = fp_from_raw(q[2]); Q.y.c1 = fp_from_raw(q[3]);
    T = Q;
    Fp2 nqy = f2_neg(Q.y);
    int li = 0;
#pragma unroll 1
    for (int i = ZKV_ATE_NAF_LEN - 2; i >= 0; i--) {
        out[li++] = line_to_table(aff_dbl(T));
        int d = ate_naf(i);
        if (d != 0) out[li++] = line_to_table(aff_add(T, Q.x, d > 0 ? Q.y : nqy));
    }
    Fp2 q1x, q1y, q2x, q2y;
    g2_frob_affine(q1x, q1y, Q.x, Q.y);
    g2_frob2_affine(q2x, q2y, Q.x, Q.y);
    out[li++] = line_to_table(aff_add(T, q1x, q1y));
    out[li++] = line_to_table(aff_add(T, q2x, f2_neg(q2y)));
}
ZKV_HD G1J g1_mul_raw(const Fp& x, const Fp& y, const uint32_t k[8]) {
    G1J acc = g1j_infinity();
#pragma unroll 1
    for (int i = 255; i >= 0; i--) {
        acc = g1j_dbl(acc);
        if ((k[i >> 5] >> (i & 31)) & 1u) acc = g1j_add_affine(acc, x, y);
    }
    return acc;
}
ZKV_HD void g1j_to_affine(const G1J& p, G1A& out, uint32_t& inf) {
    if (fp_is_zero(p.z)) { inf = 1; out.x = fp_zero(); out.y = fp_zero(); return; }
    Fp zi = fp_inv(p.z), zi2 = fp_sqr(zi);
    out.x = fp_mul(p.x, zi2); out.y = fp_mul(p.y, fp_mul(zi2, zi)); inf = 0;
}
ZKV_HD void fixed_signal_base(const VkRaw& vk, const uint32_t scalar[MAX_IC][8], G1A& base, uint32_t& base_inf) {
    G1J acc;
    if (raw_g1_is_inf(vk.ic[0])) acc = g1j_infinity();
    else { acc.x = fp_from_raw(vk.ic[0][0]); acc.y = fp_from_raw(vk.ic[0][1]); acc.z = fp_one(); }
#pragma unroll 1
    for (uint32_t i = 1; i < vk.n_ic; i++) {
        if (!vk.is_fixed[i] || raw_g1_is_inf(vk.ic[i])) continue;
        G1J m = g1_mul_raw(fp_from_raw(vk.ic[i][0]), fp_from_raw(vk.ic[i][1]), scalar[i]);
        G1A ma; uint32_t inf;
        g1j_to_affine(m, ma, inf);
        if (!inf) acc = g1j_add_affine(acc, ma.x, ma.y);
    }
    g1j_to_affine(acc, base, base_inf);
}
ZKV_HD void setup_base(const VkRaw& vk, VkTables& t) {
    fixed_signal_base(vk, vk.fixed_scalar, t.base, t.base_inf);
    t.n_var = vk.n_var;
    for (int b = 0; b < MAX_VAR; b++) t.var_windows[b] = vk.var_windows[b];
}
ZKV_HD void setup_window_row(const Fp& x, const Fp& y, int w, G1A* row) {
    G1J p; p.x = x; p.y = y; p.z = fp_one();
#pragma unroll 1
    for (int i = 0; i < 8 * w; i++) p = g1j_dbl(p);
    Fp zi = fp_inv(p.z), zi2 = fp_sqr(zi);
    row[0].x = fp_zero(); row[0].y = fp_zero();
    row[1].x = fp_mul(p.x, zi2); row[1].y = fp_mul(p.y, fp_mul(zi2, zi));
#pragma unroll 1
    for (int m = 1; m < MSM_DIGITS; m *= 2) {
        const Fp xm = row[m].x, ym = row[m].y;
        const int cnt = (2 * m < MSM_DIGITS) ? m : m - 1;
        Fp prod = fp_one();
#pragma unroll 1
        for (int j = 1; j <= cnt; j++) {
            Fp den = (j < m) ? fp_sub(row[j].x, xm) : fp_dbl(ym);
            row[m + j].y = prod;
            prod = fp_mul(prod, den);
        }
        Fp inv = fp_inv(prod);
#pragma unroll 1
        for (int j = cnt; j >= 1; j--) {
            Fp den = (j < m) ? fp_sub(row[j].x, xm) : fp_dbl(ym);
            Fp dinv = fp_mul(inv, row[m + j].y);
            inv = fp_mul(inv, den);
            Fp xj = (j < m) ? row[j].x : xm;
            Fp num = (j < m) ? fp_sub(row[j].y, ym) : fp_add(fp_dbl(fp_sqr(xm)), fp_sqr(xm));
            Fp lam = fp_mul(num, dinv);
            Fp x3 = fp_sub(fp_sub(fp_sqr(lam), xm), xj);
            row[m + j].x = x3;
            row[m + j].y = fp_sub(fp_mul(lam, fp_sub(xm, x3)), ym);
        }
    }
}
ZKV_HD void setup_msm_row(const VkRaw& vk, VkTables& t, int b, int w) {
    uint32_t ici = vk.var_ic[b];
    if (raw_g1_is_inf(vk.ic[ici])) {
        if (w == 0) t.var_windows[b] = 0;
        return;
    }
    setup_window_row(fp_from_raw(vk.ic[ici][0]), fp_from_raw(vk.ic[ici][1]), w, t.msm[b][w]);
}
ZKV_HD void setup_msm16_chunk(const VkTables& t, G1A* row, uint32_t b, uint32_t w, uint32_t hi, uint32_t lo0) {
    const uint32_t nw = t.var_windows[b];
    if (2 * w >= nw) return;
    const G1A* L = t.msm[b][2 * w];
    G1A* out = row + hi * 256 + lo0;
    if (hi == 0) {
#pragma unroll 1
        for (uint32_t j = 0; j < 64; j++) out[j] = L[lo0 + j];
        return;
    }
    if (2 * w + 1 >= nw) return;
    const G1A H = t.msm[b][2 * w + 1][hi];
    Fp prod = fp_one();
#pragma unroll 1
    for (uint32_t j = 0; j < 64; j++) {
        if (lo0 + j == 0) continue;
        out[j].y = prod;
        prod = fp_mul(prod, fp_sub(L[lo0 + j].x, H.x));
    }
    Fp inv = fp_inv(prod);
#pragma unroll 1
    for (int j = 63; j >= 0; j--) {
        if (lo0 + j == 0) { out[j] = H; continue; }
        const G1A P = L[lo0 + j];
        const Fp dinv = fp_mul(inv, out[j].y);
        inv = fp_mul(inv, fp_sub(P.x, H.x));
        const Fp lam = fp_mul(fp_sub(P.y, H.y), dinv);
        const Fp x3 = fp_sub(fp_sub(fp_sqr(lam), H.x), P.x);
        out[j].x = x3;
        out[j].y = fp_sub(fp_mul(lam, fp_sub(H.x, x3)), H.y);
    }
}
ZKV_HD void setup_long_row(const uint32_t ic[2][8], uint32_t w, G1A* row, uint32_t* win) {
    const bool inf = raw_g1_is_inf(ic);
    if (w == 0) *win = inf ? 0u : (uint32_t)MSM_MAX_WINDOWS;
    if (!inf) setup_window_row(fp_from_raw(ic[0]), fp_from_raw(ic[1]), (int)w, row);
}
ZKV_HD bool long_ic_valid(const uint32_t* ic, uint32_t first, uint32_t n_sig, uint32_t step) {
    bool ok = true;
#pragma unroll 1
    for (uint32_t b = first; b < n_sig; b += step) ok = raw_g1_valid((const uint32_t(*)[8])(ic + 16 * (size_t)b)) && ok;
    return ok;
}
ZKV_HD void setup_instance(const VkRaw& vk, const InstConsts& k, const InstRaw& in, InstTab& out) {
    uint8_t buf[130];
    for (int i = 0; i < 32; i++) { buf[i] = k.tag[i]; buf[32 + i] = in.control_root[i]; buf[64 + i] = in.control_id[31 - i]; buf[96 + i] = k.vk_digest[i]; }
    buf[128] = 3; buf[129] = 0;
    uint32_t h[8];
    sha256_bytes(buf, 130, h);
    out.selector_be = h[0];
    uint32_t sc[MAX_IC][8];
    for (int i = 0; i < MAX_IC; i++) for (int j = 0; j < 8; j++) sc[i][j] = 0;
    for (int j = 0; j < 4; j++) {
        sc[1][j] = __builtin_bswap32(load_be32(in.control_root + 4 * j));
        sc[2][j] = __builtin_bswap32(load_be32(in.control_root + 16 + 4 * j));
    }
    load_be256(sc[5], in.control_id);
    out.fail = raw_lt_r(sc[5]) ? 0u : 1u;
    if (out.fail) for (int j = 0; j < 8; j++) sc[5][j] = 0;
    fixed_signal_base(vk, sc, out.base, out.base_inf);
    out.pad = 0;
}
ZKV_HD void setup_alpha_beta(const VkRaw& vk, VkTables& t, MRef fm, MRef tm) {
    if (raw_g1_is_inf(vk.alpha) || raw_g2_is_inf(vk.beta)) {
        f12m_set_one(fm);
        for (int k = 0; k < 96; k++) t.f_alpha_beta[k] = fm.p[(size_t)k * fm.stride];
        return;
    }
    Fp ax = fp_from_raw(vk.alpha[0]), ay = fp_from_raw(vk.alpha[1]);
    Fp iy = fp_inv(ay);
    G1Norm n; n.axs = fp_mul(ax, iy); n.ays = iy;
    n.lxs = n.lys = n.cxs = n.cys = fp_zero();
    Fp2 bx, by;
    bx.c0 = fp_from_raw(vk.beta[0]); bx.c1 = fp_from_raw(vk.beta[1]);
    by.c0 = fp_from_raw(vk.beta[2]); by.c1 = fp_from_raw(vk.beta[3]);
    miller_loop_m((const VkTables*)nullptr, 0, n, bx, by, fm, tm);
    for (int k = 0; k < 96; k++) t.f_alpha_beta[k] = fm.p[(size_t)k * fm.stride];
}

#endif

}
```

Baseline: 6.120 million.

## Use prepared multiplier tables for x^u multiplications in final exponentiation

Adds a second final-exponentiation program whose x^u tables (x, x^17, x^35) are stored once in a prepared form: Karatsuba-style pair sums are precomputed in limb form. Those multiplications (39 of them) then use a dedicated f12l9_mul_p that reads the precomputed sums instead of recomputing operand additions. New PREP/MULP/MULPC/COPYP opcodes and extra workspace for three prepared entries support this, and the paired kernel switches to the prepared program. The cost is extra memory traffic and storage for the prepared entries, which may offset the saved arithmetic.

After: 5.932 million. 0.969x the previous value.

```diff
diff --git a/stylus_zkvm_verifiers_amd/csrc/bn254_constants.h b/stylus_zkvm_verifiers_amd/csrc/bn254_constants.h
--- a/stylus_zkvm_verifiers_amd/csrc/bn254_constants.h
+++ b/stylus_zkvm_verifiers_amd/csrc/bn254_constants.h
@@ -32,6 +32,8 @@
 #define ZKV_U_DIG {17, 0, 0, 0, 0, -17, 0, 0, 0, 0, 35, 0, 0, 0, 0, 17, 0, 0, 0, 0, 0, 35, 0, 0, 0, 35, 0, 0, 0, 0, 0, 0, 0, 0, -35, 0, 0, 0, -35, 0, 0, 0, 35, 0, 17, 0, 0, 0, 0, 0, 0, -35, 0, 0, 0, 0, 0, 35}
 #define ZKV_FE_PROG_LEN 268
 #define ZKV_FE_PROG {0x10000u, 0x1u, 0x10102u, 0x1000003u, 0x800u, 0x2080105u, 0x800u, 0x8010203u, 0x20000u, 0x6u, 0x6u, 0x6u, 0x6u, 0x2000003u, 0x600u, 0x6u, 0x2000003u, 0x700u, 0x6u, 0x6u, 0x6u, 0x6u, 0x6u, 0x6u, 0x7000004u, 0x6u, 0x6u, 0x6u, 0x6u, 0x6u, 0x6u, 0x6u, 0x6000003u, 0x6u, 0x6u, 0x7000003u, 0x6u, 0x6u, 0x6u, 0x6u, 0x7000004u, 0x6u, 0x6u, 0x6u, 0x6u, 0x7000004u, 0x6u, 0x6u, 0x6u, 0x6u, 0x6u, 0x6u, 0x6u, 0x6u, 0x6u, 0x7000003u, 0x6u, 0x6u, 0x6u, 0x6u, 0x7000003u, 0x6u, 0x6u, 0x6u, 0x6u, 0x6u, 0x6u, 0x6000003u, 0x6u, 0x6u, 0x6u, 0x6u, 0x6u, 0x7000003u, 0x6u, 0x6u, 0x6u, 0x6u, 0x6u, 0x6000004u, 0x6u, 0x6u, 0x6u, 0x6u, 0x6u, 0x6000003u, 0x1u, 0x6u, 0x300u, 0x6u, 0x3000003u, 0x400u, 0x6u, 0x6u, 0x6u, 0x6u, 0x4000003u, 0x600u, 0x6u, 0x4000003u, 0x700u, 0x6u, 0x6u, 0x6u, 0x6u, 0x6u, 0x6u, 0x7000004u, 0x6u, 0x6u, 0x6u, 0x6u, 0x6u, 0x6u, 0x6u, 0x6000003u, 0x6u, 0x6u, 0x7000003u, 0x6u, 0x6u, 0x6u, 0x6u, 0x7000004u, 0x6u, 0x6u, 0x6u, 0x6u, 0x7000004u, 0x6u, 0x6u, 0x6u, 0x6u, 0x6u, 0x6u, 0x6u, 0x6u, 0x6u, 0x7000003u, 0x6u, 0x6u, 0x6u, 0x6u, 0x7000003u, 0x6u, 0x6u, 0x6u, 0x6u, 0x6u, 0x6u, 0x6000003u, 0x6u, 0x6u, 0x6u, 0x6u, 0x6u, 0x7000003u, 0x6u, 0x6u, 0x6u, 0x6u, 0x6u, 0x6000004u, 0x6u, 0x6u, 0x6u, 0x6u, 0x6u, 0x6000003u, 0x1u, 0x500u, 0x6u, 0x100u, 0x6u, 0x6u, 0x6u, 0x6u, 0x1000003u, 0x600u, 0x6u, 0x1000003u, 0x700u, 0x6u, 0x6u, 0x6u, 0x6u, 0x6u, 0x6u, 0x7000004u, 0x6u, 0x6u, 0x6u, 0x6u, 0x6u, 0x6u, 0x6u, 0x6000003u, 0x6u, 0x6u, 0x7000003u, 0x6u, 0x6u, 0x6u, 0x6u, 0x7000004u, 0x6u, 0x6u, 0x6u, 0x6u, 0x7000004u, 0x6u, 0x6u, 0x6u, 0x6u, 0x6u, 0x6u, 0x6u, 0x6u, 0x6u, 0x7000003u, 0x6u, 0x6u, 0x6u, 0x6u, 0x7000003u, 0x6u, 0x6u, 0x6u, 0x6u, 0x6u, 0x6u, 0x6000003u, 0x6u, 0x6u, 0x6u, 0x6u, 0x6u, 0x7000003u, 0x6u, 0x6u, 0x6u, 0x6u, 0x6u, 0x6000004u, 0x6u, 0x6u, 0x6u, 0x6u, 0x6u, 0x6000003u, 0x401u, 0x5000003u, 0x4000003u, 0x400u, 0x800u, 0x3080103u, 0x5000003u, 0x2000003u, 0x1010305u, 0x3000003u, 0x2040405u, 0x4000003u, 0x201u, 0x1020203u, 0x3020205u, 0x2000003u, 0x800u, 0x807u}
+#define ZKV_FE_PROG_PREP_LEN 271
+#define ZKV_FE_PROG_PREP {0x10000u, 0x1u, 0x10102u, 0x1000003u, 0x800u, 0x2080105u, 0x800u, 0x8010203u, 0x20000u, 0x8u, 0x6u, 0x6u, 0x6u, 0x6u, 0x9u, 0x108u, 0x6u, 0x9u, 0x208u, 0x6u, 0x6u, 0x6u, 0x6u, 0x6u, 0x6u, 0x200000au, 0x6u, 0x6u, 0x6u, 0x6u, 0x6u, 0x6u, 0x6u, 0x1000009u, 0x6u, 0x6u, 0x2000009u, 0x6u, 0x6u, 0x6u, 0x6u, 0x200000au, 0x6u, 0x6u, 0x6u, 0x6u, 0x200000au, 0x6u, 0x6u, 0x6u, 0x6u, 0x6u, 0x6u, 0x6u, 0x6u, 0x6u, 0x2000009u, 0x6u, 0x6u, 0x6u, 0x6u, 0x2000009u, 0x6u, 0x6u, 0x6u, 0x6u, 0x6u, 0x6u, 0x1000009u, 0x6u, 0x6u, 0x6u, 0x6u, 0x6u, 0x2000009u, 0x6u, 0x6u, 0x6u, 0x6u, 0x6u, 0x100000au, 0x6u, 0x6u, 0x6u, 0x6u, 0x6u, 0x1000009u, 0x1u, 0x6u, 0x300u, 0x6u, 0x3000003u, 0x400u, 0x8u, 0x6u, 0x6u, 0x6u, 0x6u, 0x9u, 0x108u, 0x6u, 0x9u, 0x208u, 0x6u, 0x6u, 0x6u, 0x6u, 0x6u, 0x6u, 0x200000au, 0x6u, 0x6u, 0x6u, 0x6u, 0x6u, 0x6u, 0x6u, 0x1000009u, 0x6u, 0x6u, 0x2000009u, 0x6u, 0x6u, 0x6u, 0x6u, 0x200000au, 0x6u, 0x6u, 0x6u, 0x6u, 0x200000au, 0x6u, 0x6u, 0x6u, 0x6u, 0x6u, 0x6u, 0x6u, 0x6u, 0x6u, 0x2000009u, 0x6u, 0x6u, 0x6u, 0x6u, 0x2000009u, 0x6u, 0x6u, 0x6u, 0x6u, 0x6u, 0x6u, 0x1000009u, 0x6u, 0x6u, 0x6u, 0x6u, 0x6u, 0x2000009u, 0x6u, 0x6u, 0x6u, 0x6u, 0x6u, 0x100000au, 0x6u, 0x6u, 0x6u, 0x6u, 0x6u, 0x1000009u, 0x1u, 0x500u, 0x6u, 0x100u, 0x8u, 0x6u, 0x6u, 0x6u, 0x6u, 0x9u, 0x108u, 0x6u, 0x9u, 0x208u, 0x6u, 0x6u, 0x6u, 0x6u, 0x6u, 0x6u, 0x200000au, 0x6u, 0x6u, 0x6u, 0x6u, 0x6u, 0x6u, 0x6u, 0x1000009u, 0x6u, 0x6u, 0x2000009u, 0x6u, 0x6u, 0x6u, 0x6u, 0x200000au, 0x6u, 0x6u, 0x6u, 0x6u, 0x200000au, 0x6u, 0x6u, 0x6u, 0x6u, 0x6u, 0x6u, 0x6u, 0x6u, 0x6u, 0x2000009u, 0x6u, 0x6u, 0x6u, 0x6u, 0x2000009u, 0x6u, 0x6u, 0x6u, 0x6u, 0x6u, 0x6u, 0x1000009u, 0x6u, 0x6u, 0x6u, 0x6u, 0x6u, 0x2000009u, 0x6u, 0x6u, 0x6u, 0x6u, 0x6u, 0x100000au, 0x6u, 0x6u, 0x6u, 0x6u, 0x6u, 0x1000009u, 0x401u, 0x5000003u, 0x4000003u, 0x400u, 0x800u, 0x3080103u, 0x5000003u, 0x2000003u, 0x1010305u, 0x3000003u, 0x2040405u, 0x4000003u, 0x201u, 0x1020203u, 0x3020205u, 0x2000003u, 0x800u, 0x807u}
 #define ZKV_FP_M30_LIMBS {0x187cfd47, 0x3082305b, 0x071ca8d3, 0x205aa45a, 0x01585d97, 0x0116da06, 0x1a029b85, 0x139cb84c, 0x00003064}
 #define ZKV_FP_MINV30 0x1b799c77u
 #define ZKV_FP_R3 {{0x4e2312b2u, 0x26d80b94u, 0x85af210eu, 0xfdde6f98u, 0xad1d1adau, 0xb923065cu, 0xa668ff5au, 0x26c2d286u}}
diff --git a/stylus_zkvm_verifiers_amd/csrc/gen_constants.py b/stylus_zkvm_verifiers_amd/csrc/gen_constants.py
--- a/stylus_zkvm_verifiers_amd/csrc/gen_constants.py
+++ b/stylus_zkvm_verifiers_amd/csrc/gen_constants.py
@@ -130,96 +130,126 @@
     w('// width-3 NAF digits of u (odd digits up to +-7), least significant first, top digit 1: %d non-zero digits' % sum(1 for d in u_w3 if d))
     w('#define ZKV_U_WNAF3_LEN %d' % len(u_w3))
     w('#define ZKV_U_WNAF3 {%s}' % ', '.join(str(d) for d in u_w3))
-    OPS = dict(COPY=0, CONJ=1, INV=2, MUL=3, MULC=4, FROB=5, CSQR=6, ISONE=7)
+    OPS = dict(COPY=0, CONJ=1, INV=2, MUL=3, MULC=4, FROB=5, CSQR=6, ISONE=7, PREP=8, MULP=9, MULPC=10, COPYP=11)
     ACC, F_, E_, Y1, Y3, Y4, X3, X5, X7 = range(9)
-    prog = []
-    acc_is = [None]
-    def op(name, d=0, a=0, b=0):
-        if name == 'COPY' and d == ACC and acc_is[0] == a:
-            return
-        if name == 'COPY' and a == ACC: acc_is[0] = d
-        elif name == 'COPY' and d == ACC: acc_is[0] = a
-        elif d == ACC or d == acc_is[0]: acc_is[0] = None
-        prog.append(OPS[name] | d << 8 | a << 16 | b << 24)
-    import functools, sys
-    sys.setrecursionlimit(10000)
-    DIG = (1, 17, 35)
-    @functools.lru_cache(None)
-    def recode(n):
-        if n == 0:
-            return (0, ())
-        if n % 2 == 0:
-            c, t = recode(n // 2)
-            return (c, (0,) + t)
-        best = None
-        for d in DIG:
-            for sd in (d, -d):
-                m = (n - sd) // 2
-                if abs(m) < abs(n) or (abs(n) <= max(DIG) and m == 0):
-                    c, t = recode(m)
-                    if best is None or c + 1 < best[0]:
-                        best = (c + 1, (sd,) + t)
-        return best
-    u_dig = recode(U)[1]
-    assert sum(d << i for i, d in enumerate(u_dig)) == U and u_dig[-1] > 0 and sum(1 for d in u_dig if d) == 12
-    w('// digits of u from {0, +-1, +-17, +-35}, least significant first, top digit positive: %d non-zero (final exponentiation, x^u)' % sum(1 for d in u_dig if d))
-    w('#define ZKV_U_DIG_LEN %d' % len(u_dig))
-    w('#define ZKV_U_DIG {%s}' % ', '.join(str(d) for d in u_dig))
-    def expu(x):
-        X17, X35 = X3, X5
-        op('COPY', ACC, x)
-        for _ in range(4): op('CSQR', ACC)
-        op('MUL', ACC, ACC, x); op('COPY', X17, ACC)
-        op('CSQR', ACC)
-        op('MUL', ACC, ACC, x); op('COPY', X35, ACC)
-        src = {1: x, 17: X17, 35: X35}
-        op('COPY', ACC, src[u_dig[-1]])
-        for i in range(len(u_dig) - 2, -1, -1):
-            op('CSQR', ACC)
-            d = u_dig[i]
-            if d:
-                op('MUL' if d > 0 else 'MULC', ACC, ACC, src[abs(d)])
-    op('COPY', ACC, F_); op('CONJ', ACC); op('INV', F_, F_); op('MUL', ACC, ACC, F_)
-    op('FROB', F_, ACC, 2); op('MUL', E_, F_, ACC)
-    expu(E_); op('CONJ', ACC)
-    op('CSQR', ACC); op('COPY', Y1, ACC)
-    op('CSQR', ACC)
-    op('MUL', ACC, ACC, Y1); op('COPY', Y3, ACC)
-    expu(Y3); op('CONJ', ACC); op('COPY', Y4, ACC)
-    op('CSQR', ACC); op('COPY', F_, ACC)
-    expu(F_)
-    op('CONJ', Y3)
-    op('MUL', ACC, ACC, Y4)
-    op('MUL', ACC, ACC, Y3); op('COPY', Y3, ACC)
-    op('MUL', F_, ACC, Y1)
-    op('MUL', ACC, ACC, Y4)
-    op('MUL', ACC, ACC, E_)
-    op('FROB', Y1, F_, 1); op('MUL', ACC, ACC, Y1)
-    op('FROB', Y3, Y3, 2); op('MUL', ACC, ACC, Y3)
-    op('CONJ', E_); op('MUL', E_, E_, F_); op('FROB', E_, E_, 3)
-    op('MUL', ACC, ACC, E_)
-    op('ISONE', ACC)
-    TMP = 8
-    out = []
-    for e in prog:
-        o, d, a, b = e & 255, (e >> 8) & 255, (e >> 16) & 255, e >> 24
-        native = (o == OPS['CSQR'] or o == OPS['COPY'] or (o == OPS['CONJ'] and d == ACC)
-                  or (o in (OPS['MUL'], OPS['MULC']) and d == ACC and a == ACC and b != ACC))
-        if not native:
-            assert d != ACC or o == OPS['ISONE']
-            uses = (a == ACC and o in (OPS['INV'], OPS['MUL'], OPS['MULC'], OPS['FROB'])) or (b == ACC and o in (OPS['MUL'], OPS['MULC'])) or (o == OPS['ISONE'] and d == ACC)
-            if uses:
-                out.append(OPS['COPY'] | TMP << 8 | ACC << 16)
-                if o == OPS['ISONE']: d = TMP
-                if a == ACC and o != OPS['ISONE']: a = TMP
-                if b == ACC and o in (OPS['MUL'], OPS['MULC']): b = TMP
-                e = o | d << 8 | a << 16 | b << 24
-        out.append(e)
-    prog = out
-    w('// final exponentiation (easy part, Fuentes-Castaneda hard part, x^u on the signed digit set {1, 17, 35}) as a flat program: op | dst << 8 | a << 16 | b << 24;')
-    w('// ops 0 COPY d<-a, 1 CONJ d, 2 INV d<-a, 3 MUL d<-a*b, 4 MULC d<-a*conj(b), 5 FROB d<-pi^b(a), 6 CSQR d (cyclotomic), 7 ISONE; slots 0 ACC 1 F 2 E 3 Y1 4 Y3 5 Y4 6 X17 7 X35 8 TMP')
-    w('#define ZKV_FE_PROG_LEN %d' % len(prog))
-    w('#define ZKV_FE_PROG {%s}' % ', '.join('0x%xu' % v for v in prog))
+    for prepared in (False, True):
+      prog = []
+      acc_is = [None]
+      def op(name, d=0, a=0, b=0):
+          if name == 'COPY' and d == ACC and acc_is[0] == a:
+              return
+          if name == 'COPY' and a == ACC: acc_is[0] = d
+          elif name == 'COPY' and d == ACC: acc_is[0] = a
+          elif d == ACC or d == acc_is[0]: acc_is[0] = None
+          prog.append(OPS[name] | d << 8 | a << 16 | b << 24)
+      import functools, sys
+      sys.setrecursionlimit(10000)
+      DIG = (1, 17, 35)
+      @functools.lru_cache(None)
+      def recode(n):
+          if n == 0:
+              return (0, ())
+          if n % 2 == 0:
+              c, t = recode(n // 2)
+              return (c, (0,) + t)
+          best = None
+          for d in DIG:
+              for sd in (d, -d):
+                  m = (n - sd) // 2
+                  if abs(m) < abs(n) or (abs(n) <= max(DIG) and m == 0):
+                      c, t = recode(m)
+                      if best is None or c + 1 < best[0]:
+                          best = (c + 1, (sd,) + t)
+          return best
+      u_dig = recode(U)[1]
+      assert sum(d << i for i, d in enumerate(u_dig)) == U and u_dig[-1] > 0 and sum(1 for d in u_dig if d) == 12
+      if not prepared:
+          w('// digits of u from {0, +-1, +-17, +-35}, least significant first, top digit positive: %d non-zero (final exponentiation, x^u)' % sum(1 for d in u_dig if d))
+          w('#define ZKV_U_DIG_LEN %d' % len(u_dig))
+          w('#define ZKV_U_DIG {%s}' % ', '.join(str(d) for d in u_dig))
+      def expu_prepared(x):
+          op('COPY', ACC, x); op('PREP', 0)
+          for _ in range(4): op('CSQR', ACC)
+          op('MULP', ACC, ACC, 0); op('PREP', 1)
+          op('CSQR', ACC)
+          op('MULP', ACC, ACC, 0); op('PREP', 2)
+          src = {1: 0, 17: 1, 35: 2}
+          if u_dig[-1] != 35: op('COPYP', ACC, src[u_dig[-1]])
+          for i in range(len(u_dig) - 2, -1, -1):
+              op('CSQR', ACC)
+              d = u_dig[i]
+              if d:
+                  op('MULP' if d > 0 else 'MULPC', ACC, ACC, src[abs(d)])
+      def expu(x):
+          if prepared:
+              return expu_prepared(x)
+          X17, X35 = X3, X5
+          op('COPY', ACC, x)
+          for _ in range(4): op('CSQR', ACC)
+          op('MUL', ACC, ACC, x); op('COPY', X17, ACC)
+          op('CSQR', ACC)
+          op('MUL', ACC, ACC, x); op('COPY', X35, ACC)
+          src = {1: x, 17: X17, 35: X35}
+          op('COPY', ACC, src[u_dig[-1]])
+          for i in range(len(u_dig) - 2, -1, -1):
+              op('CSQR', ACC)
+              d = u_dig[i]
+              if d:
+                  op('MUL' if d > 0 else 'MULC', ACC, ACC, src[abs(d)])
+      op('COPY', ACC, F_); op('CONJ', ACC); op('INV', F_, F_); op('MUL', ACC, ACC, F_)
+      op('FROB', F_, ACC, 2); op('MUL', E_, F_, ACC)
+      expu(E_); op('CONJ', ACC)
+      op('CSQR', ACC); op('COPY', Y1, ACC)
+      op('CSQR', ACC)
+      op('MUL', ACC, ACC, Y1); op('COPY', Y3, ACC)
+      expu(Y3); op('CONJ', ACC); op('COPY', Y4, ACC)
+      op('CSQR', ACC); op('COPY', F_, ACC)
+      expu(F_)
+      op('CONJ', Y3)
+      op('MUL', ACC, ACC, Y4)
+      op('MUL', ACC, ACC, Y3); op('COPY', Y3, ACC)
+      op('MUL', F_, ACC, Y1)
+      op('MUL', ACC, ACC, Y4)
+      op('MUL', ACC, ACC, E_)
+      op('FROB', Y1, F_, 1); op('MUL', ACC, ACC, Y1)
+      op('FROB', Y3, Y3, 2); op('MUL', ACC, ACC, Y3)
+      op('CONJ', E_); op('MUL', E_, E_, F_); op('FROB', E_, E_, 3)
+      op('MUL', ACC, ACC, E_)
+      op('ISONE', ACC)
+      TMP = 8
+      out = []
+      for e in prog:
+          o, d, a, b = e & 255, (e >> 8) & 255, (e >> 16) & 255, e >> 24
+          if o == OPS['CSQR']: assert d == ACC
+          if o in (OPS['MULP'], OPS['MULPC']): assert prepared and d == ACC and a == ACC and b < 3
+          if o == OPS['PREP']: assert prepared and d < 3
+          if o == OPS['COPYP']: assert prepared and d == ACC and a < 3
+          native = (o in (OPS['CSQR'], OPS['COPY'], OPS['PREP'], OPS['MULP'], OPS['MULPC'], OPS['COPYP']) or (o == OPS['CONJ'] and d == ACC)
+                    or (o in (OPS['MUL'], OPS['MULC']) and d == ACC and a == ACC and b != ACC))
+          if native and o in (OPS['MUL'], OPS['MULC']): assert a == ACC and b != ACC
+          if not native:
+              assert d != ACC or o == OPS['ISONE']
+              uses = (a == ACC and o in (OPS['INV'], OPS['MUL'], OPS['MULC'], OPS['FROB'])) or (b == ACC and o in (OPS['MUL'], OPS['MULC'])) or (o == OPS['ISONE'] and d == ACC)
+              if uses:
+                  out.append(OPS['COPY'] | TMP << 8 | ACC << 16)
+                  if o == OPS['ISONE']: d = TMP
+                  if a == ACC and o != OPS['ISONE']: a = TMP
+                  if b == ACC and o in (OPS['MUL'], OPS['MULC']): b = TMP
+                  e = o | d << 8 | a << 16 | b << 24
+          out.append(e)
+      prog = out
+      if not prepared:
+          w('// final exponentiation (easy part, Fuentes-Castaneda hard part, x^u on the signed digit set {1, 17, 35}) as a flat program: op | dst << 8 | a << 16 | b << 24;')
+          w('// ops 0 COPY d<-a, 1 CONJ d, 2 INV d<-a, 3 MUL d<-a*b, 4 MULC d<-a*conj(b), 5 FROB d<-pi^b(a), 6 CSQR d (cyclotomic), 7 ISONE; slots 0 ACC 1 F 2 E 3 Y1 4 Y3 5 Y4 6 X17 7 X35 8 TMP')
+          w('#define ZKV_FE_PROG_LEN %d' % len(prog))
+          w('#define ZKV_FE_PROG {%s}' % ', '.join('0x%xu' % v for v in prog))
+      else:
+          n = lambda *names: sum(1 for v in prog if (v & 255) in [OPS[k] for k in names])
+          assert n('MULP', 'MULPC') == 39 and n('MUL', 'MULC') == 12 and n('PREP') == 9 and n('CSQR') == 189
+          w('// the same program with the table values x, x^17, x^35 of every x^u kept as prepared multipliers in limb-form entries 0, 1, 2:')
+          w('// ops 8 PREP P[d]<-ACC, 9 MULP ACC<-ACC*P[b], 10 MULPC ACC<-ACC*conj(P[b]), 11 COPYP ACC<-P[a]; %d entries, %d on prepared multipliers' % (len(prog), n('MULP', 'MULPC')))
+          w('#define ZKV_FE_PROG_PREP_LEN %d' % len(prog))
+          w('#define ZKV_FE_PROG_PREP {%s}' % ', '.join('0x%xu' % v for v in prog))
     e = P - 2
     bits = bin(e)[2:]
     sched = []
diff --git a/stylus_zkvm_verifiers_amd/csrc/k_pair.hip b/stylus_zkvm_verifiers_amd/csrc/k_pair.hip
--- a/stylus_zkvm_verifiers_amd/csrc/k_pair.hip
+++ b/stylus_zkvm_verifiers_amd/csrc/k_pair.hip
@@ -74,7 +74,8 @@
     const uint32_t par = threadIdx.x & 1u;
     uint32_t* wl = lds + (threadIdx.x >> 6) * (54 * ZKV_BLOCK) + (threadIdx.x & 63u);
     L9Ref acc = l9_ref(wl);
-    bool one = final_exp_prog_p(ws.f, ws.fe, ws.cap, (uint32_t)(8 * par * ws.cap + i) * 4u, acc);
+    static_assert(WS_FE_WORDS == WS_FE_PACKED_WORDS + 3 * ZKV_PREP_WORDS, "ws.fe holds the packed slots and three prepared entries");
+    bool one = final_exp_prog_t<true>(ws.f, ws.fe, ws.cap, (uint32_t)(8 * par * ws.cap + i) * 4u, acc);
     if (!par) status[i] = one ? ST_OK : ST_VERIFICATION_FAILED;
     ZKV_STAMP(1, 1);
 }
diff --git a/stylus_zkvm_verifiers_amd/csrc/zkv_field.h b/stylus_zkvm_verifiers_amd/csrc/zkv_field.h
--- a/stylus_zkvm_verifiers_amd/csrc/zkv_field.h
+++ b/stylus_zkvm_verifiers_amd/csrc/zkv_field.h
@@ -556,6 +556,32 @@
 ZKV_HD L9 l9_mul(const L9& a, const L9& b) { return l9_mul_ni(ZKV_L9A(a), ZKV_L9A(b)); }
 #else
 ZKV_HD L9 l9_mul(const L9& a, const L9& b) { return l9_mul_core(a, b); }
+#endif
+ZKV_HD L9 l9_mul_uv_core(const L9& a, const L9& u, const L9& v) {
+#if defined(ZKV_COUNT_FP_MUL)
+    zkv_fp_mul_counter += 2;
+#endif
+    const uint32_t FAT[9] = ZKV_FP_FAT8P_LIMBS;
+    uint32_t xo[9], V[9];
+    uint64_t col[18];
+#pragma unroll
+    for (int k = 0; k < 18; k++) col[k] = 0;
+    fp_mac81(col, a.l, u.l);
+    const bool even = zkv_parity() == 0;
+#pragma unroll
+    for (int i = 0; i < 9; i++) { xo[i] = zkv_partner_u32(a.l[i]); V[i] = even ? FAT[i] - v.l[i] : v.l[i]; }
+    fp_mac81(col, xo, V);
+    L9 r; fp_reduce_cols_limbs(col, r.l);
+    return r;
+}
+#if defined(__HIP_DEVICE_COMPILE__) && defined(ZKV_FP_MUL_NOINLINE)
+__device__ __noinline__ inline L9 l9_mul_uv_ni(ZKV_L9P(pa), ZKV_L9P(pu), ZKV_L9P(pv)) {
+    ZKV_L9MK(a, pa); ZKV_L9MK(u, pu); ZKV_L9MK(v, pv);
+    return l9_mul_uv_core(a, u, v);
+}
+ZKV_HD L9 l9_mul_uv(const L9& a, const L9& u, const L9& v) { return l9_mul_uv_ni(ZKV_L9A(a), ZKV_L9A(u), ZKV_L9A(v)); }
+#else
+ZKV_HD L9 l9_mul_uv(const L9& a, const L9& u, const L9& v) { return l9_mul_uv_core(a, u, v); }
 #endif
 struct LTerm { const uint32_t* x; int32_t k; };
 #define ZKV_L9_G 256
diff --git a/stylus_zkvm_verifiers_amd/csrc/zkv_internal.h b/stylus_zkvm_verifiers_amd/csrc/zkv_internal.h
--- a/stylus_zkvm_verifiers_amd/csrc/zkv_internal.h
+++ b/stylus_zkvm_verifiers_amd/csrc/zkv_internal.h
@@ -7,7 +7,8 @@
 constexpr int WS_PREP_WORDS = 64 + 8 * MAX_VAR;
 constexpr int WS_NORM_WORDS = 48;
 constexpr int WS_F_WORDS = 96;
-constexpr int WS_FE_WORDS = 7 * 96;
+constexpr int WS_FE_PACKED_WORDS = 7 * 96;
+constexpr int WS_FE_WORDS = WS_FE_PACKED_WORDS + 3 * 18 * 18;
 struct Workspace {
     uint32_t* prep; uint32_t* norm; uint32_t* f; uint32_t* fe; uint32_t* flags;
     uint32_t* g2bad;
diff --git a/stylus_zkvm_verifiers_amd/csrc/zkv_tower_mem.h b/stylus_zkvm_verifiers_amd/csrc/zkv_tower_mem.h
--- a/stylus_zkvm_verifiers_amd/csrc/zkv_tower_mem.h
+++ b/stylus_zkvm_verifiers_amd/csrc/zkv_tower_mem.h
@@ -274,6 +274,154 @@
     }
     l9_st(acc, 3, h0); l9_st(acc, 4, h1); l9_st(acc, 5, h2);
 }
+constexpr int ZKV_PREP_WORDS = 18 * 18;
+struct PRef { uint32_t* p; size_t stride; uint32_t off; };
+ZKV_HD uint32_t zkv_parity_here() {
+    uint32_t par = zkv_parity();
+#if defined(__HIP_DEVICE_COMPILE__)
+    asm volatile("" : "+v"(par));
+#endif
+    return par;
+}
+ZKV_HD uint32_t p_own(PRef m) { return m.off + zkv_parity_here() * 36u * (uint32_t)m.stride; }
+ZKV_HD PRef m_fresh(PRef r) {
+#if defined(__HIP_DEVICE_COMPILE__)
+    asm volatile("" : "+v"(r.off));
+#endif
+    return r;
+}
+#if defined(__HIP_DEVICE_COMPILE__)
+typedef __attribute__((address_space(1))) uint32_t zkv_glb_u32;
+typedef __attribute__((address_space(1))) char zkv_glb_char;
+#else
+typedef uint32_t zkv_glb_u32;
+typedef char zkv_glb_char;
+#endif
+ZKV_HD L9 p_ld(PRef m, int row0, uint32_t lane_off) {
+    L9 r;
+#pragma unroll
+    for (int k = 0; k < 9; k++) r.l[k] = *(const zkv_glb_u32*)((const zkv_glb_char*)((const zkv_glb_u32*)m.p + (size_t)(row0 + k) * m.stride) + lane_off);
+    return r;
+}
+ZKV_HD void p_st_own(PRef m, uint32_t own, int j, const L9& a) {
+#pragma unroll
+    for (int k = 0; k < 9; k++) *(zkv_glb_u32*)((zkv_glb_char*)((zkv_glb_u32*)m.p + (size_t)(18 * j + k) * m.stride) + own) = a.l[k];
+}
+ZKV_HD L9 l9_mul_p(const L9& a, PRef S0, int j) {
+    PRef S = m_fresh(S0);
+    S.p += (size_t)(18 * j) * S.stride;
+#if defined(__HIP_DEVICE_COMPILE__)
+    asm volatile("" : "+s"(S.p));
+#endif
+    return l9_mul_uv(a, p_ld(S, 0, S.off), p_ld(S, 9, S.off));
+}
+ZKV_HD void l9_prep_f6(PRef P, int t, const L9& b0, const L9& b1, const L9& b2) {
+    const uint32_t own = p_own(P);
+    p_st_own(P, own, 6 * t, b0); p_st_own(P, own, 6 * t + 1, b1); p_st_own(P, own, 6 * t + 2, b2);
+    { const LTerm s[2] = {{b1.l, 1}, {b2.l, 1}}; p_st_own(P, own, 6 * t + 3, l9_lincomb(s, 1)); }
+    { const LTerm s[2] = {{b0.l, 1}, {b1.l, 1}}; p_st_own(P, own, 6 * t + 4, l9_lincomb(s, 1)); }
+    { const LTerm s[2] = {{b0.l, 1}, {b2.l, 1}}; p_st_own(P, own, 6 * t + 5, l9_lincomb(s, 1)); }
+}
+ZKV_HD void f12l9_prep(PRef P0, L9Ref acc) {
+    const PRef P = m_fresh(P0);
+    L9 z[3];
+#pragma unroll
+    for (int i = 0; i < 3; i++) {
+        const L9 g = l9_ld(acc, i), h = l9_ld(acc, 3 + i);
+        const LTerm s[2] = {{g.l, 1}, {h.l, 1}};
+        z[i] = l9_lincomb(s, 1);
+    }
+    l9_prep_f6(P, 2, z[0], z[1], z[2]);
+    l9_prep_f6(P, 0, l9_ld(acc, 0), l9_ld(acc, 1), l9_ld(acc, 2));
+    l9_prep_f6(P, 1, l9_ld(acc, 3), l9_ld(acc, 4), l9_ld(acc, 5));
+}
+ZKV_HD void f12l9_from_prep(L9Ref acc, PRef P0) {
+    const PRef P = m_fresh(P0);
+    const uint32_t own = p_own(P);
+#pragma unroll
+    for (int i = 0; i < 6; i++) l9_st(acc, i, p_ld(P, 18 * (6 * (i / 3) + i % 3), own));
+}
+template <class LDA> ZKV_HD void l9_f6_mul_raw_p(LDA lda, PRef S0, int t, L9F6Raw& r) {
+    const PRef S = S0;
+    r.v0 = l9_mul_p(lda(0), S, 6 * t);
+    const L9 v1 = l9_mul_p(lda(1), S, 6 * t + 1);
+    r.v2 = l9_mul_p(lda(2), S, 6 * t + 2);
+    L9 sa, m;
+    { const L9 a1 = lda(1), a2 = lda(2);
+#pragma unroll
+      for (int i = 0; i < 9; i++) sa.l[i] = a1.l[i] + a2.l[i]; }
+    m = l9_mul_p(sa, S, 6 * t + 3);
+#pragma unroll
+    for (int i = 0; i < 9; i++) r.wa[i] = (int32_t)m.l[i] - (int32_t)v1.l[i] - (int32_t)r.v2.l[i];
+    { const L9 a0 = lda(0), a1 = lda(1);
+#pragma unroll
+      for (int i = 0; i < 9; i++) sa.l[i] = a0.l[i] + a1.l[i]; }
+    m = l9_mul_p(sa, S, 6 * t + 4);
+#pragma unroll
+    for (int i = 0; i < 9; i++) r.wb[i] = (int32_t)m.l[i] - (int32_t)r.v0.l[i] - (int32_t)v1.l[i];
+    { const L9 a0 = lda(0), a2 = lda(2);
+#pragma unroll
+      for (int i = 0; i < 9; i++) sa.l[i] = a0.l[i] + a2.l[i]; }
+    m = l9_mul_p(sa, S, 6 * t + 5);
+#pragma unroll
+    for (int i = 0; i < 9; i++) r.wc[i] = (int32_t)m.l[i] - (int32_t)r.v0.l[i] - (int32_t)r.v2.l[i] + (int32_t)v1.l[i];
+}
+ZKV_HD void f12l9_mul_p(L9Ref acc, PRef S, const bool conj_b) {
+    const int32_t k1 = zkv_parity() != 0 ? 1 : -1;
+    const int32_t sg = conj_b ? -1 : 1;
+    L9F6Raw raw;
+    int32_t pw[9];
+    L9 xc0, xc1, xc2;
+    {
+        l9_f6_mul_raw_p([&](int i) { return l9_ld(acc, i); }, S, 0, raw);
+        l9_partner_i32(raw.wa, pw);
+        { const LTerm t[3] = {{raw.v0.l, 1}, {(const uint32_t*)raw.wa, 9}, {(const uint32_t*)pw, k1}}; xc0 = l9_lincomb(t, 48); }
+        const L9 pv2 = l9_partner(raw.v2);
+        { const LTerm t[3] = {{(const uint32_t*)raw.wb, 1}, {raw.v2.l, 9}, {pv2.l, k1}}; xc1 = l9_lincomb(t, 8); }
+        { const LTerm t[1] = {{(const uint32_t*)raw.wc, 1}}; xc2 = l9_lincomb(t, 8); }
+    }
+    uint32_t xy0[9], xy1[9], xy2[9];
+    {
+        L9 g0, g1, g2;
+        l9_f6_mul_raw_p([&](int i) { return l9_ld(acc, 3 + i); }, S, 1, raw);
+        L9 yc0, yc1, yc2;
+        l9_partner_i32(raw.wa, pw);
+        { const LTerm t[3] = {{raw.v0.l, 1}, {(const uint32_t*)raw.wa, 9}, {(const uint32_t*)pw, k1}}; yc0 = l9_lincomb(t, 48); }
+        const L9 pv2 = l9_partner(raw.v2);
+        { const LTerm t[3] = {{(const uint32_t*)raw.wb, 1}, {raw.v2.l, 9}, {pv2.l, k1}}; yc1 = l9_lincomb(t, 8); }
+        { const LTerm t[1] = {{(const uint32_t*)raw.wc, 1}}; yc2 = l9_lincomb(t, 8); }
+        const L9 pyc2 = l9_partner(yc2);
+        { const LTerm t[3] = {{xc0.l, 1}, {yc2.l, 9 * sg}, {pyc2.l, k1 * sg}}; g0 = l9_lincomb(t, 12); }
+        { const LTerm t[2] = {{xc1.l, 1}, {yc0.l, sg}}; g1 = l9_lincomb(t, 3); }
+        { const LTerm t[2] = {{xc2.l, 1}, {yc1.l, sg}}; g2 = l9_lincomb(t, 3); }
+#pragma unroll
+        for (int i = 0; i < 9; i++) {
+            xy0[i] = yc0.l[i] + (uint32_t)(sg * (int32_t)xc0.l[i]); xy1[i] = yc1.l[i] + (uint32_t)(sg * (int32_t)xc1.l[i]);
+            xy2[i] = yc2.l[i] + (uint32_t)(sg * (int32_t)xc2.l[i]);
+        }
+        const uint32_t FAT4[9] = ZKV_FP_FAT4P_LIMBS;
+#pragma unroll
+        for (int i = 0; i < 3; i++) {
+            const L9 g = l9_ld(acc, i), h = l9_ld(acc, 3 + i);
+            L9 sum;
+#pragma unroll
+            for (int k = 0; k < 9; k++) sum.l[k] = h.l[k] + (conj_b ? FAT4[k] - g.l[k] : g.l[k]);
+            l9_carry(sum.l);
+            l9_st(acc, 3 + i, sum);
+        }
+        l9_st(acc, 0, g0); l9_st(acc, 1, g1); l9_st(acc, 2, g2);
+    }
+    L9 h0, h1, h2;
+    {
+        l9_f6_mul_raw_p([&](int i) { return l9_ld(acc, 3 + i); }, S, 2, raw);
+        l9_partner_i32(raw.wa, pw);
+        { const LTerm t[4] = {{raw.v0.l, 1}, {(const uint32_t*)raw.wa, 9}, {(const uint32_t*)pw, k1}, {xy0, -1}}; h0 = l9_lincomb(t, 52); }
+        const L9 pv2 = l9_partner(raw.v2);
+        { const LTerm t[4] = {{(const uint32_t*)raw.wb, 1}, {raw.v2.l, 9}, {pv2.l, k1}, {xy1, -1}}; h1 = l9_lincomb(t, 12); }
+        { const LTerm t[2] = {{(const uint32_t*)raw.wc, 1}, {xy2, -1}}; h2 = l9_lincomb(t, 12); }
+    }
+    l9_st(acc, 3, h0); l9_st(acc, 4, h1); l9_st(acc, 5, h2);
+}
 #endif
 
 template <class RD, class RA, class RB> ZKV_HD void f12m_mul_body(RD d, RA a, RB b, bool conj_b) {
diff --git a/stylus_zkvm_verifiers_amd/csrc/zkv_verify.h b/stylus_zkvm_verifiers_amd/csrc/zkv_verify.h
--- a/stylus_zkvm_verifiers_amd/csrc/zkv_verify.h
+++ b/stylus_zkvm_verifiers_amd/csrc/zkv_verify.h
@@ -458,23 +458,32 @@
     SoaRW r; r.p = s == 1 ? fbase : ebase + (size_t)(96 * (s - 2)) * cap; r.stride = cap; r.off = off;
     return r;
 }
-ZKV_HD bool final_exp_prog_p(uint32_t* fbase, uint32_t* ebase, size_t cap, uint32_t off, L9Ref acc) {
-    const uint32_t PROG[ZKV_FE_PROG_LEN] = ZKV_FE_PROG;
+ZKV_HD PRef fe_prep(int q, uint32_t* ebase, size_t cap, uint32_t off) {
+    PRef r; r.p = ebase + (size_t)(7 * 96 + ZKV_PREP_WORDS * q) * cap; r.stride = cap; r.off = off - zkv_parity_here() * 32u * (uint32_t)cap;
+    return r;
+}
+template <bool PREPARED> ZKV_HD bool final_exp_prog_t(uint32_t* fbase, uint32_t* ebase, size_t cap, uint32_t off, L9Ref acc) {
+    constexpr int LEN = PREPARED ? ZKV_FE_PROG_PREP_LEN : ZKV_FE_PROG_LEN;
+    const uint32_t PROG_A[ZKV_FE_PROG_LEN] = ZKV_FE_PROG;
+    const uint32_t PROG_B[ZKV_FE_PROG_PREP_LEN] = ZKV_FE_PROG_PREP;
     bool one = false;
     const uint32_t slot = zkv_wave_slot_parity();
 #pragma unroll 1
-    for (int pc = 0; pc < ZKV_FE_PROG_LEN; pc++) {
-        const uint32_t e = PROG[pc];
+    for (int pc = 0; pc < LEN; pc++) {
+        const uint32_t e = PREPARED ? PROG_B[pc] : PROG_A[pc];
         const int op = (int)(e & 255u), d = (int)((e >> 8) & 255u), a = (int)((e >> 16) & 255u), b = (int)(e >> 24);
         if ((pc & 3) == 0) zkv_fair_share(slot);
 #if defined(__HIP_DEVICE_COMPILE__)
         asm volatile("" : "+v"(off));
 #endif
         if (op == 6) { ZKV_MARK("begin cyclo"); f12l9_cyclo_sqr(acc); ZKV_MARK("end cyclo"); }
+        else if (PREPARED && (op == 9 || op == 10)) { ZKV_MARK("begin prepmul"); f12l9_mul_p(acc, fe_prep(b, ebase, cap, off), op == 10); ZKV_MARK("end prepmul"); }
+        else if (PREPARED && op == 8) { ZKV_MARK("begin prep"); f12l9_prep(fe_prep(d, ebase, cap, off), acc); ZKV_MARK("end prep"); }
+        else if (PREPARED && op == 11) { ZKV_MARK("begin fromprep"); f12l9_from_prep(acc, fe_prep(a, ebase, cap, off)); ZKV_MARK("end fromprep"); }
         else if ((op == 3 || op == 4) && d == 0) { ZKV_MARK("begin accmul");  f12l9_mul(acc, fe_slot(b, fbase, ebase, cap, off), op == 4); ZKV_MARK("end accmul"); }
-        else if (op == 0 && d == 0) f12m_copy(acc, fe_slot(a, fbase, ebase, cap, off));
-        else if (op == 0 && a == 0) f12m_copy(fe_slot(d, fbase, ebase, cap, off), acc);
-        else if (op == 1 && d == 0) f12m_conj(acc);
+        else if (op == 0 && d == 0) { ZKV_MARK("begin copyin"); f12m_copy(acc, fe_slot(a, fbase, ebase, cap, off)); ZKV_MARK("end copyin"); }
+        else if (op == 0 && a == 0) { ZKV_MARK("begin copyout"); f12m_copy(fe_slot(d, fbase, ebase, cap, off), acc); ZKV_MARK("end copyout"); }
+        else if (op == 1 && d == 0) { ZKV_MARK("begin conjacc"); f12m_conj(acc); ZKV_MARK("end conjacc"); }
         else {
             const SoaRW D = fe_slot(d, fbase, ebase, cap, off), A = fe_slot(a, fbase, ebase, cap, off);
             if (op == 3 || op == 4) { ZKV_MARK("begin genmul"); f12m_mul_body(D, A, fe_slot(b, fbase, ebase, cap, off), op == 4); ZKV_MARK("end genmul"); }
@@ -486,6 +495,9 @@
         }
     }
     return one;
+}
+ZKV_HD bool final_exp_prog_p(uint32_t* fbase, uint32_t* ebase, size_t cap, uint32_t off, L9Ref acc) {
+    return final_exp_prog_t<false>(fbase, ebase, cap, off, acc);
 }
 #endif
 
```
